# GREAT-WHU/DBA-Fusion

Measured on AMD Instinct MI355X. Metric: DBA iterations/sec (25-KF, 96-edge, 512x512) [dba_update/s], higher is better.
Workload: dtype f32 (BA, f64 reduced system) / f16 (correlation)

## Files before the change

dba-fusion_amd/csrc/ba_host.hip:

```cpp
#include <hip/hip_runtime.h>

#include <algorithm>
#include <atomic>
#include <cstdio>
#include <cstdlib>
#include <cstring>
#include <mutex>
#include <unordered_map>
#include <vector>

#include "ba_kernels.h"

#ifndef GRAM_F32_DEFAULT
#define GRAM_F32_DEFAULT true
#endif

namespace dba {

static thread_local char g_last_error[512] = "";

void set_last_error(const char *what, hipError_t e) {
  snprintf(g_last_error, sizeof(g_last_error), "%s -> %s", what, hipGetErrorString(e));
}

struct BaEnv {
  static int num(const char *name) { const char *e = getenv(name); return e ? atoi(e) : 0; }
  static bool is(const char *name, const char *prefix) { const char *e = getenv(name); return e && !strncmp(e, prefix, strlen(prefix)); }
  int deterministic = is("DBA_DETERMINISTIC", "1");
  int solve_check = is("DBA_SOLVE_CHECK", "1");
  int schur_form = is("DBA_SCHUR_KERNEL", "r") ? 1 : (is("DBA_SCHUR_KERNEL", "f") || is("DBA_SCHUR_KERNEL", "g")) ? 2 : 0;
  int lin_ppl = num("DBA_LINEARIZE_PPL");
  bool lin_no_mfma = is("DBA_LINEARIZE_MFMA", "0");
  int lin_ew = num("DBA_LIN_EW");
  bool h_full = is("DBA_H_FULL", "1");
  int schur_nch = num("DBA_SCHUR_NCH");
  int gram_threads = num("DBA_SCHUR_WAVES") == 4 ? 256 : 512;
  bool gram_f32 = getenv("DBA_SCHUR_MFMA") ? is("DBA_SCHUR_MFMA", "f3") : GRAM_F32_DEFAULT;
  bool fuse_update = !is("DBA_BA_FUSE_UPDATE", "0");
};
static const BaEnv &ba_env() { static const BaEnv env; return env; }

static std::atomic<int> g_schur_form{ba_env().schur_form};
static std::atomic<int> g_deterministic{ba_env().deterministic};
static std::atomic<int> g_solve_check{ba_env().solve_check};

__global__ __launch_bounds__(256) void ba_solve_check_kernel(const double *__restrict__ H, const double *__restrict__ b, int n, double lm,
                                                             double ep, float *__restrict__ dx, int *__restrict__ meta) {
  __shared__ double s_res[256], s_mag[256];
  __shared__ int s_bad;
  if (meta[1] != 0) return;
  double res = 0.0, mag = 0.0;
  for (int i = threadIdx.x; i < n; i += blockDim.x) {
    double acc = -b[i], m = fabs(b[i]);
    for (int j = 0; j < n; j++) {
      double h = H[(size_t)max(i, j) * n + min(i, j)];
      if (i == j) h = fma(lm, h, h) + ep;
      const double t = h * (double)dx[j];
      acc += t, m += fabs(t);
    }
    res = fmax(res, fabs(acc)), mag = fmax(mag, m);
  }
  s_res[threadIdx.x] = res, s_mag[threadIdx.x] = mag;
  __syncthreads();
  if (threadIdx.x == 0) {
    double r = 0.0, m = 0.0;
    for (int k = 0; k < (int)blockDim.x; k++) r = fmax(r, s_res[k]), m = fmax(m, s_mag[k]);
    s_bad = !(r <= 1e-5 * m) ? 1 : 0;
    if (s_bad) meta[1] = 1;
  }
  __syncthreads();
  if (s_bad)
    for (int i = threadIdx.x; i < n; i += blockDim.x) dx[i] = 0.f;
}

static bool schur_auto_frame_form(int N, int P) {
  const int frames = P + 1;
  const int rows_est = 1 + (N + frames - 1) / frames;
  return rows_est > 6;
}

static std::atomic<int> g_schur_generation{0};
static thread_local int t_schur_form = 0;

bool ba_schur_frame_form(int N, int P) {
  const int forced = g_schur_form.load(std::memory_order_relaxed);
  if (N + 1 > GRAM_LIST_CAP) return false;
  if (forced) return forced == 2;
  if (t_schur_form) return t_schur_form == 2;
  return schur_auto_frame_form(N, P);
}

int ba_plan(int N, int B, int ht, int wd, int t0, int t1, void *ws, size_t ws_bytes, BaPlan *plan) {
  if (N < 0 || B <= 0 || ht <= 0 || wd <= 0 || t1 < t0 || t0 < 0 || t1 > B) return DBA_ERR_ARG;
  const int P = t1 - t0;
  const int HW = ht * wd;
  const int Mmax = (P + N < B) ? (P + N) : B;
  int ppl = 1;
  {
    const int env_ppl = ba_env().lin_ppl;
    const long waves1 = (long)Mmax * ((HW + 63) / 64);
    if (env_ppl == 1 || env_ppl == 2 || env_ppl == 4) ppl = env_ppl;
    else if (waves1 >= 16 * 1024) ppl = 4;
    else if (waves1 >= 8 * 1024) ppl = 2;
  }
  const int nchunks = (HW + 256 * ppl - 1) / (256 * ppl);
  const int nparts_max = ((HW + 255) / 256) * 4;
  const int nparts = nchunks * 4;
  const int n6 = 6 * P;
  size_t off = 0;
  auto take = [&](size_t bytes) {
    const size_t o = off;
    off = align_up(off + bytes, 256);
    return o;
  };
  dba_ba_layout L;
  memset(&L, 0, sizeof(L));
  L.meta = take(sizeof(int) * 32);
  const size_t o_gkey = take(sizeof(int) * (8 + 2 * (size_t)N));
  L.kx = take(sizeof(int) * (size_t)(Mmax > 0 ? Mmax : 1));
  const size_t o_fslot = take(sizeof(int) * (size_t)B);
  const size_t o_eoff = take(sizeof(int) * (size_t)(Mmax + 1));
  const size_t o_elist = take(sizeof(int) * (size_t)(N > 0 ? N : 1));
  const size_t o_erank = take(sizeof(int) * (size_t)(N > 0 ? N : 1));
  const size_t o_fpose = take(sizeof(int) * (size_t)(P > 0 ? P : 1));
  const size_t o_einfo = take(sizeof(int) * 2 * (size_t)(N > 0 ? N : 1));
  const size_t o_rowinfo = take(sizeof(int) * 8 * (size_t)(P + N > 0 ? P + N : 1));
  const size_t o_fhead = take(sizeof(int) * 4 * (size_t)(Mmax > 0 ? Mmax : 1));
  const size_t o_frow = take(sizeof(int) * 2 * (size_t)(P + N > 0 ? P + N : 1));
  L.E = take(sizeof(float) * (size_t)(P + N) * 6 * HW);
  L.Q = take(sizeof(float) * (size_t)Mmax * HW);
  L.w = take(sizeof(float) * (size_t)Mmax * HW);
  const size_t o_hparte = take(sizeof(float) * (size_t)(N > 0 ? N : 1) * nparts_max * HPE_STRIDE);
  const size_t o_aedge = take(sizeof(double) * 36 * (size_t)(N > 0 ? N : 1));
  L.dx = take(sizeof(float) * (size_t)(n6 > 0 ? n6 : 1));
  const size_t o_ptmp = take(sizeof(float) * 2 * 7 * (size_t)B);
  L.H = take(sizeof(double) * (size_t)(n6 > 0 ? n6 * (size_t)n6 : 1));
  L.b = take(sizeof(double) * (size_t)(n6 > 0 ? n6 : 1));
  size_t o_lscratch = 0;
  const bool lds_fits = ba_solve_fits_lds(n6);
  const bool want_scratch = !lds_fits || (ba_solve_band_supported(n6) && n6 >= 96);
  if (want_scratch) o_lscratch = take(sizeof(double) * ba_solve_scratch_doubles(n6));
  L.P = P;
  L.Mmax = Mmax;
  L.nchunks = nchunks;
  plan->layout = L;
  plan->bytes = off;
  plan->P = P;
  plan->N = N;
  plan->B = B;
  plan->HW = HW;
  plan->nchunks = nchunks;
  plan->ht = ht, plan->wd = wd, plan->t0 = t0, plan->t1 = t1;
  if (ws) {
    if (ws_bytes < off) return DBA_ERR_WORKSPACE;
    char *base = static_cast<char *>(ws);
    plan->T.meta = reinterpret_cast<int *>(base + L.meta);
    plan->T.kx = reinterpret_cast<int *>(base + L.kx);
    plan->T.frame_slot = reinterpret_cast<int *>(base + o_fslot);
    plan->T.eoff = reinterpret_cast<int *>(base + o_eoff);
    plan->T.elist = reinterpret_cast<int *>(base + o_elist);
    plan->T.elist_rank = reinterpret_cast<int *>(base + o_erank);
    plan->T.fpose = reinterpret_cast<int *>(base + o_fpose);
    plan->T.einfo = reinterpret_cast<int *>(base + o_einfo);
    plan->T.rowinfo = reinterpret_cast<int *>(base + o_rowinfo);
    plan->T.fhead = reinterpret_cast<int *>(base + o_fhead);
    plan->T.frow = reinterpret_cast<int *>(base + o_frow);
    plan->T.gkey = reinterpret_cast<int *>(base + o_gkey);
    plan->T.Mmax = Mmax;
    plan->T.B = B;
    plan->W.E = reinterpret_cast<float *>(base + L.E);
    plan->W.Q = reinterpret_cast<float *>(base + L.Q);
    plan->W.w = reinterpret_cast<float *>(base + L.w);
    plan->W.HpartE = reinterpret_cast<float *>(base + o_hparte);
    plan->W.Aedge = reinterpret_cast<double *>(base + o_aedge);
    plan->W.dx = reinterpret_cast<float *>(base + L.dx);
    plan->W.poses_tmp = reinterpret_cast<float *>(base + o_ptmp);
    plan->W.H = reinterpret_cast<double *>(base + L.H);
    plan->W.b = reinterpret_cast<double *>(base + L.b);
    plan->W.Lscratch = want_scratch ? reinterpret_cast<double *>(base + o_lscratch) : nullptr;
    plan->W.nparts = nparts;
    plan->W.ppl = ppl;
  }
  return DBA_OK;
}

static int ba_prepare_stage(const BaPlan &plan, const int64_t *ii, const int64_t *jj, int eta_rows, int check, bool judge_band,
                            hipStream_t stream) {
  const int N = plan.N, B = plan.B, P = plan.P;
  if (N > 0 && (!ii || !jj)) return DBA_ERR_ARG;
  const int want = std::max(std::max(N, B), P);
  const int threads = std::min(1024, std::max(64, (want + 63) / 64 * 64));
  const size_t scan_ints = std::max<size_t>(std::max(threads, P), N > threads ? 1024 : 0) + 32;
  const size_t lds = sizeof(int) * ((size_t)B + 2 * (size_t)plan.T.Mmax + 1 + scan_ints + plan.T.Mmax + 1);
  if (lds > 160 * 1024 || P > 16384) return DBA_ERR_UNSUPPORTED;
  if (lds > 64 * 1024) {
    DBA_HIP_CHECK(hipFuncSetAttribute(reinterpret_cast<const void *>(&ba_prepare_kernel),
                                      hipFuncAttributeMaxDynamicSharedMemorySize, 160 * 1024));
  }
  const int max_nt = judge_band ? ba_solve_wave_max_nt(6 * P) : 0;
  int *band_verdict = max_nt ? solver_verdict_slot(plan.T.meta) : nullptr;
  hipLaunchKernelGGL(ba_prepare_kernel, dim3(1), dim3(threads), lds, stream, ii, jj, N, B, plan.t0, plan.t1,
                     (int)scan_ints, ba_schur_frame_form(N, P) ? 1 : 0, check ? 1 : 0, eta_rows,
                     eta_rows > 1 ? ws_eta_status(plan.T.meta) : nullptr, plan.T, band_verdict, max_nt);
  DBA_LAUNCH_CHECK();
  return DBA_OK;
}

static int ba_linearize_stage(const BaPlan &plan, const BaProblem &g, const float *poses, const float *disps, float alpha,
                              int upd, float *poses_out, float *disps_w, hipStream_t stream) {
  if (!poses || !disps || !g.intrinsics || !g.disps_sens || !g.eta || g.eta_rows < 1) return DBA_ERR_ARG;
  if (g.eta_rows > 1 && g.eta_rows > plan.T.Mmax) return DBA_ERR_ARG;
  if (plan.N > 0 && (!g.targets || !g.weights || !g.jj)) return DBA_ERR_ARG;
#define LAUNCH_LIN(PPL, MF, EW)                                                                                          \
  hipLaunchKernelGGL((ba_linearize_kernel<PPL, MF, EW>), dim3(plan.nchunks * EW, plan.T.Mmax + 1), dim3(256), 0, stream, \
                     poses, disps, g.intrinsics, g.disps_sens, g.targets, g.weights, g.eta, g.eta_rows, g.jj,            \
                     g.frame_owned, plan.N, plan.HW, plan.wd, plan.t0, plan.P, alpha, upd, poses_out, disps_w, plan.T, plan.W)
  if (plan.W.ppl == 4) LAUNCH_LIN(4, false, 1);
  else if (plan.W.ppl == 2) LAUNCH_LIN(2, false, 1);
  else if (ba_env().lin_no_mfma) LAUNCH_LIN(1, false, 1);
  else {
    const int env_ew = ba_env().lin_ew;
    const long waves2 = (long)plan.nchunks * 2 * 4 * plan.T.Mmax;
    const bool one = env_ew ? env_ew == 1 : waves2 > 4096;
    if (one) LAUNCH_LIN(1, true, 1);
    else LAUNCH_LIN(1, true, 2);
  }
#undef LAUNCH_LIN
  DBA_LAUNCH_CHECK();
  return DBA_OK;
}

static int ba_reduce_stage(const BaPlan &plan, const int64_t *ii, const int64_t *jj, const uint8_t *frame_owned, int motion_only,
                           int lower, hipStream_t stream) {
  const int N = plan.N;
  const int ablocks = (N + 3) / 4;
  if (plan.P <= 0) return DBA_OK;
  if (ba_env().h_full) lower = 0;
  const bool fixed = g_deterministic.load(std::memory_order_relaxed) != 0;
  if (fixed) lower |= 2;
  if (!motion_only) {
    if (!ba_schur_frame_form(N, plan.P)) {
      hipLaunchKernelGGL(ba_schur_kernel, dim3(plan.P + N + ablocks, SCHUR_KP, SCHUR_CH), dim3(256), 0, stream, ii, jj,
                         frame_owned, N, plan.HW, plan.t0, plan.P, lower, plan.T, plan.W);
    } else {
      const int px = 1024;
      int nch = ba_env().schur_nch > 0 ? ba_env().schur_nch : (plan.HW + px - 1) / px;
      nch = std::max(1, std::min(nch, (plan.HW + 15) / 16));
      const dim3 grid((unsigned)(plan.T.Mmax * nch + ablocks));
      const int gram_threads = ba_env().gram_threads;
      const bool f32 = ba_env().gram_f32;
#define GRAM_LAUNCH(V, F)                                                                                     \
  hipLaunchKernelGGL((ba_schur_gram_kernel<V, F>), grid, dim3(gram_threads), 0, stream, ii, jj, frame_owned, \
                     N, plan.HW, plan.t0, plan.P, nch, lower, plan.T, plan.W)
      if (plan.HW % 4 == 0) { if (f32) GRAM_LAUNCH(true, true); else GRAM_LAUNCH(true, false); }
      else { if (f32) GRAM_LAUNCH(false, true); else GRAM_LAUNCH(false, false); }
#undef GRAM_LAUNCH
    }
    DBA_LAUNCH_CHECK();
  } else if (ablocks > 0) {
    hipLaunchKernelGGL(ba_assemble_kernel, dim3(ablocks), dim3(256), 0, stream, ii, jj, frame_owned, N, plan.t0, plan.P,
                       lower, plan.T, plan.W);
    DBA_LAUNCH_CHECK();
  }
  if (fixed) {
    const int n = 6 * plan.P;
    hipLaunchKernelGGL(ba_fixed_to_f64_kernel, dim3((n * n + n + 255) / 256), dim3(256), 0, stream, plan.W.H, plan.W.b, n);
    DBA_LAUNCH_CHECK();
  }
  return DBA_OK;
}

static int ba_symmetrize_launch(const BaPlan &plan, hipStream_t stream) {
  const int n = 6 * plan.P;
  if (n <= 0) return DBA_OK;
  hipLaunchKernelGGL(ba_symmetrize_kernel, dim3((n * n + 255) / 256), dim3(256), 0, stream, plan.W.H, n);
  DBA_LAUNCH_CHECK();
  return DBA_OK;
}

static int ba_solve_check_launch(const BaPlan &plan, float lm, float ep, hipStream_t stream) {
  if (plan.P <= 0) return DBA_OK;
  hipLaunchKernelGGL(ba_solve_check_kernel, dim3(1), dim3(256), 0, stream, plan.W.H, plan.W.b, 6 * plan.P, (double)lm, (double)ep,
                     plan.W.dx, plan.T.meta);
  DBA_LAUNCH_CHECK();
  return DBA_OK;
}

static int ba_solve_stage(const BaPlan &plan, float lm, float ep, const int *fpose, int hint, hipStream_t stream) {
  const int rc = launch_ba_solve(plan.W.H, plan.W.b, fpose, 6 * plan.P, (double)lm, (double)ep, plan.W.dx, plan.T.meta,
                                 plan.W.Lscratch, stream, nullptr, hint, (fpose && fpose == plan.T.fpose) ? plan.T.meta + 16 : nullptr);
  if (rc != DBA_OK) return rc;
  if (g_solve_check.load(std::memory_order_relaxed)) return ba_solve_check_launch(plan, lm, ep, stream);
  return DBA_OK;
}

static int ba_update_launch(const BaPlan &plan, float *poses, float *disps, const int64_t *jj, const uint8_t *frame_owned,
                            int update_poses, int update_disps, float *dz_out, float *dx_out, hipStream_t stream,
                            const float *poses_src = nullptr, float disp_floor = 0.f) {
  dim3 grid((plan.HW + 255) / 256, plan.T.Mmax + 1 + (disp_floor > 0.f ? plan.B : 0));
  hipLaunchKernelGGL(ba_update_kernel, grid, dim3(256), 0, stream, poses, poses_src, disps, jj, frame_owned, plan.HW, plan.t0,
                     plan.P, update_poses, update_disps, dz_out, dx_out, plan.T, plan.W, disp_floor);
  DBA_LAUNCH_CHECK();
  return DBA_OK;
}

int ba_run_loop(const BaPlan &plan, const BaProblem &g, float *poses, float *disps, const BaRun &run, hipStream_t stream) {
  const int *fpose = run.window_fpose ? run.window_fpose : plan.T.fpose;
  int rc;
  if (run.prepared != 1) {
    rc = ba_prepare_stage(plan, g.ii, g.jj, g.eta_rows, run.prepared == 2, run.window_fpose == nullptr, stream);
    if (rc != DBA_OK) return rc;
  }
  const bool fuse = ba_env().fuse_update;
  const float *pose_src = poses;
  bool pending = false;
  for (int itr = 0; itr < run.iterations; itr++) {
    float *pose_dst = plan.W.poses_tmp + (size_t)(itr & 1) * 7 * plan.B;
    const int upd = pending ? (run.motion_only ? 1 : 3) : 0;
    rc = ba_linearize_stage(plan, g, pose_src, disps, run.alpha, upd, pending ? pose_dst : nullptr, disps, stream);
    if (rc != DBA_OK) return rc;
    if (pending) pose_src = pose_dst;
    rc = ba_reduce_stage(plan, g.ii, g.jj, g.frame_owned, run.motion_only, 1, stream);
    if (rc != DBA_OK) return rc;
    if (run.exchange && run.exchange->fn && plan.P > 0) {
      const size_t n6 = (size_t)6 * plan.P;
      rc = run.exchange->fn(run.exchange->ctx, plan.W.H, (size_t)(plan.W.b - plan.W.H) + n6, stream);
      if (rc != DBA_OK) return rc;
    }
    rc = ba_solve_stage(plan, run.lm, run.ep, fpose, run.solver_hint, stream);
    if (rc != DBA_OK) return rc;
    const bool last = (itr == run.iterations - 1);
    if (fuse && !last) {
      pending = true;
      continue;
    }
    rc = ba_update_launch(plan, poses, disps, g.jj, g.frame_owned, 1, run.motion_only ? 0 : 1, last ? run.dz_out : nullptr,
                          last ? run.dx_out : nullptr, stream, pose_src == poses ? nullptr : pose_src,
                          last ? run.disp_floor : 0.f);
    if (rc != DBA_OK) return rc;
    pose_src = poses;
    pending = false;
  }
  return DBA_OK;
}

namespace {
struct BacoreStage {
  double *host = nullptr;
  size_t doubles = 0;
  unsigned *counter = nullptr;
  int seq = 0;
};
std::mutex g_stage_mu;
typedef std::unordered_map<const void *, BacoreStage> BacoreStageMap;
BacoreStageMap *stage_map_ptr() {
  static BacoreStageMap *m = new BacoreStageMap;
  return m;
}
#define stage_map() (*stage_map_ptr())
int *stage_flag(const BacoreStage &st) { return reinterpret_cast<int *>(st.host + st.doubles + 8); }
}

static int bacore_stage_for(const int *meta, size_t need, hipStream_t stream, BacoreStage **out) {
  std::lock_guard<std::mutex> lock(g_stage_mu);
  BacoreStage &st = stage_map()[meta];
  if (st.doubles < need) {
    if (st.host) {
      DBA_HIP_CHECK(hipStreamSynchronize(stream));
      (void)hipHostFree(st.host);
      st.host = nullptr, st.doubles = 0;
    }
    void *p = nullptr;
    DBA_HIP_CHECK(hipHostMalloc(&p, sizeof(double) * (need + 16), hipHostMallocCoherent | hipHostMallocMapped));
    st.host = static_cast<double *>(p), st.doubles = need;
    memset(p, 0, sizeof(double) * (need + 16));
    if (!st.counter) {
      DBA_HIP_CHECK(hipMalloc(reinterpret_cast<void **>(&st.counter), 64));
      DBA_HIP_CHECK(hipMemset(st.counter, 0, 64));
    }
  }
  *out = &st;
  return DBA_OK;
}

static int bacore_wait(int *flag, int seq, hipStream_t stream) {
  for (unsigned long spins = 1;; spins++) {
    if (__atomic_load_n(flag, __ATOMIC_ACQUIRE) == seq) return DBA_OK;
    if ((spins & 0x3fff) == 0) {
      const hipError_t q = hipStreamQuery(stream);
      if (q == hipSuccess) {
        if (__atomic_load_n(flag, __ATOMIC_ACQUIRE) == seq) return DBA_OK;
        set_last_error("BACore.hessian: the stream drained without the export kernel's completion word", hipErrorUnknown);
        return DBA_ERR_HIP;
      }
      if (q != hipErrorNotReady) {
        set_last_error("hipStreamQuery", q);
        return DBA_ERR_HIP;
      }
    }
    __builtin_ia32_pause();
  }
}

static int bacore_export(const BaPlan &plan, int layout, const double *A36, double stabilizer, double **out_host,
                         hipStream_t stream) {
  const int n = 6 * plan.P;
  BacoreStage *st = nullptr;
  const int rc = bacore_stage_for(plan.T.meta, (size_t)n * (n + 1), stream, &st);
  if (rc != DBA_OK) return rc;
  *out_host = st->host;
  if (n == 0) return DBA_OK;
  ExportArg arg;
  for (int i = 0; i < 36; i++) arg.A[i] = (layout == 1) ? A36[i] : 0.0;
  const int seq = ++st->seq;
  const int total = n * (n + 1);
  hipLaunchKernelGGL(ba_export_kernel, dim3((total + 255) / 256), dim3(256), 0, stream, plan.W.H, plan.W.b, n, st->host, layout,
                     arg, stabilizer, st->counter, stage_flag(*st), seq);
  DBA_LAUNCH_CHECK();
  return bacore_wait(stage_flag(*st), seq, stream);
}

}

using namespace dba;

extern "C" {

const char *dba_version(void) { return "dba_hip 0.1 (gfx950)"; }
const char *dba_last_error(void) { return g_last_error; }

size_t dba_ba_workspace_bytes(int N, int B, int ht, int wd, int t0, int t1) {
  BaPlan plan;
  if (ba_plan(N, B, ht, wd, t0, t1, nullptr, 0, &plan) != DBA_OK) return 0;
  return plan.bytes;
}

int dba_ba_get_layout(int N, int B, int ht, int wd, int t0, int t1, dba_ba_layout *out) {
  BaPlan plan;
  const int rc = ba_plan(N, B, ht, wd, t0, t1, nullptr, 0, &plan);
  if (rc != DBA_OK) return rc;
  *out = plan.layout;
  return DBA_OK;
}

int dba_ba_poll_eta_error(int *eta_rows, int *num_kx) { return ws_poll_eta(nullptr, eta_rows, num_kx); }

int dba_ba_poll_eta_error_ws(int N, int B, int ht, int wd, int t0, int t1, void *ws, size_t ws_bytes, int *eta_rows, int *num_kx) {
  DBA_PLAN_OR_RETURN(plan);
  return ws_poll_eta(plan.T.meta, eta_rows, num_kx);
}

int dba_ba_gather_edges(const float *target_inac, const float *weight_inac, const int64_t *ii_inac, const int64_t *jj_inac,
                        int n_inac, const int64_t *sel, int n_sel, const float *target_act, const float *weight_act,
                        const int64_t *ii_act, const int64_t *jj_act, int n_act, int ht, int wd, float *targets_out,
                        float *weights_out, int64_t *ii_out, int64_t *jj_out, dba_stream_t stream) {
  if (n_sel < 0 || n_act < 0 || n_inac < 0 || ht <= 0 || wd <= 0) return DBA_ERR_ARG;
  if (!sel && n_sel > n_inac) return DBA_ERR_ARG;
  const int n = n_sel + n_act;
  if (n == 0) return DBA_OK;
  if (!targets_out || !weights_out || !ii_out || !jj_out) return DBA_ERR_ARG;
  if (n_sel > 0 && (!target_inac || !weight_inac || !ii_inac || !jj_inac || n_inac == 0)) return DBA_ERR_ARG;
  if (n_act > 0 && (!target_act || !weight_act || !ii_act || !jj_act)) return DBA_ERR_ARG;
  const int HW = ht * wd;
  hipLaunchKernelGGL(ba_gather_edges_kernel, dim3((HW + 255) / 256, n, 2), dim3(256), 0, (hipStream_t)stream,
                     reinterpret_cast<const float2 *>(target_inac), reinterpret_cast<const float2 *>(weight_inac), ii_inac, jj_inac,
                     sel, n_sel, n_inac, reinterpret_cast<const float2 *>(target_act), reinterpret_cast<const float2 *>(weight_act),
                     ii_act, jj_act, HW, targets_out, weights_out, ii_out, jj_out);
  DBA_LAUNCH_CHECK();
  return DBA_OK;
}

int dba_ba_solver_verdict(int N, int B, int ht, int wd, int t0, int t1, void *ws, size_t ws_bytes) {
  DBA_PLAN_OR_RETURN(plan);
  if (!ba_solve_wave_supported(6 * plan.P)) return 2;
  const int *slot = solver_verdict_slot(plan.T.meta);
  return slot ? __atomic_load_n(slot, __ATOMIC_RELAXED) : 0;
}

int dba_ba_workspace_init(int N, int B, int ht, int wd, int t0, int t1, void *ws, size_t ws_bytes, dba_stream_t stream) {
  DBA_PLAN_OR_RETURN(plan);
  DBA_HIP_CHECK(hipMemsetAsync(plan.T.meta, 0, (size_t)((char *)(plan.T.gkey + 8) - (char *)plan.T.meta), (hipStream_t)stream));
  ws_words_reset(plan.T.meta);
  return DBA_OK;
}

int dba_ba_prepare(const int64_t *ii, const int64_t *jj, int N, int B, int ht, int wd, int t0, int t1,
                   void *ws, size_t ws_bytes, dba_stream_t stream) {
  return dba_ba_prepare_keyed(ii, jj, N, B, ht, wd, t0, t1, 0, 0, ws, ws_bytes, stream);
}

int dba_ba_prepare_keyed(const int64_t *ii, const int64_t *jj, int N, int B, int ht, int wd, int t0, int t1, int eta_rows,
                         int check, void *ws, size_t ws_bytes, dba_stream_t stream) {
  DBA_PLAN_OR_RETURN(plan);
  return ba_prepare_stage(plan, ii, jj, eta_rows, check, false, (hipStream_t)stream);
}

int dba_ba_linearize(const float *poses, const float *disps, const float *intrinsics,
                     const float *disps_sens, const float *targets, const float *weights,
                     const float *eta, int eta_rows, const int64_t *ii, const int64_t *jj,
                     const uint8_t *frame_owned, int N, int B, int ht, int wd, int t0, int t1,
                     float alpha, void *ws, size_t ws_bytes, dba_stream_t stream) {
  DBA_PLAN_OR_RETURN(plan);
  BaProblem g;
  g.intrinsics = intrinsics, g.disps_sens = disps_sens, g.targets = targets, g.weights = weights;
  g.eta = eta, g.eta_rows = eta_rows, g.ii = ii, g.jj = jj, g.frame_owned = frame_owned;
  return ba_linearize_stage(plan, g, poses, disps, alpha, 0, nullptr, nullptr, (hipStream_t)stream);
}

int dba_ba_reduce(const int64_t *ii, const int64_t *jj, const uint8_t *frame_owned, int N, int B, int ht,
                  int wd, int t0, int t1, int motion_only, void *ws, size_t ws_bytes, dba_stream_t stream) {
  DBA_PLAN_OR_RETURN(plan);
  const int rc = ba_reduce_stage(plan, ii, jj, frame_owned, motion_only, 1, (hipStream_t)stream);
  if (rc != DBA_OK) return rc;
  return ba_symmetrize_launch(plan, (hipStream_t)stream);
}

int dba_ba_schur_select(int form) {
  if (form < 0 || form > 2) return DBA_ERR_ARG;
  g_schur_form.store(form, std::memory_order_relaxed);
  g_schur_generation.fetch_add(1, std::memory_order_relaxed);
  return DBA_OK;
}

int dba_ba_schur_select_thread(int form) {
  if (form < 0 || form > 2) return DBA_ERR_ARG;
  t_schur_form = form;
  return DBA_OK;
}

int dba_ba_schur_thread_form(void) { return t_schur_form; }

int dba_ba_schur_auto_form(int N, int P) { return schur_auto_frame_form(N, P) ? 2 : 1; }

int dba_ba_schur_generation(void) { return g_schur_generation.load(std::memory_order_relaxed); }

int dba_ba_set_deterministic(int on) {
  g_deterministic.store(on ? 1 : 0, std::memory_order_relaxed);
  return DBA_OK;
}

int dba_ba_set_solve_check(int on) {
  g_solve_check.store(on ? 1 : 0, std::memory_order_relaxed);
  return DBA_OK;
}

int dba_ba_solve_check(int N, int B, int ht, int wd, int t0, int t1, float lm, float ep, void *ws, size_t ws_bytes,
                       dba_stream_t stream) {
  DBA_PLAN_OR_RETURN(plan);
  return ba_solve_check_launch(plan, lm, ep, (hipStream_t)stream);
}

int dba_ba_symmetrize(int N, int B, int ht, int wd, int t0, int t1, void *ws, size_t ws_bytes, dba_stream_t stream) {
  DBA_PLAN_OR_RETURN(plan);
  return ba_symmetrize_launch(plan, (hipStream_t)stream);
}

int dba_ba_solve(int N, int B, int ht, int wd, int t0, int t1, float lm, float ep, void *ws, size_t ws_bytes,
                 dba_stream_t stream) {
  return dba_ba_solve_skyline(N, B, ht, wd, t0, t1, lm, ep, nullptr, ws, ws_bytes, stream);
}

int dba_ba_solve_skyline(int N, int B, int ht, int wd, int t0, int t1, float lm, float ep, const int32_t *fpose, void *ws,
                         size_t ws_bytes, dba_stream_t stream) {
  DBA_PLAN_OR_RETURN(plan);
  return ba_solve_stage(plan, lm, ep, fpose, 0, (hipStream_t)stream);
}

int dba_ba_update(float *poses, float *disps, const int64_t *ii, const int64_t *jj,
                  const uint8_t *frame_owned, int N, int B, int ht, int wd, int t0, int t1, int update_poses,
                  int update_disps, float *dz_out, void *ws, size_t ws_bytes, dba_stream_t stream) {
  (void)ii;
  DBA_PLAN_OR_RETURN(plan);
  return ba_update_launch(plan, poses, disps, jj, frame_owned, update_poses, update_disps, dz_out, nullptr, (hipStream_t)stream);
}

int dba_ba_shard_front(const float *poses, const float *disps, const float *intrinsics, const float *disps_sens,
                       const float *targets, const float *weights, const float *eta, int eta_rows, const int64_t *ii,
                       const int64_t *jj, const uint8_t *frame_owned, int N, int B, int ht, int wd, int t0, int t1,
                       float alpha, int motion_only, void *ws, size_t ws_bytes, dba_stream_t stream) {
  DBA_PLAN_OR_RETURN(plan);
  BaProblem g;
  g.intrinsics = intrinsics, g.disps_sens = disps_sens, g.targets = targets, g.weights = weights;
  g.eta = eta, g.eta_rows = eta_rows, g.ii = ii, g.jj = jj, g.frame_owned = frame_owned;
  const int rc = ba_linearize_stage(plan, g, poses, disps, alpha, 0, nullptr, nullptr, (hipStream_t)stream);
  if (rc != DBA_OK) return rc;
  return ba_reduce_stage(plan, ii, jj, frame_owned, motion_only, 1, (hipStream_t)stream);
}

int dba_ba_shard_back(float *poses, float *disps, const int64_t *ii, const int64_t *jj, const uint8_t *frame_owned,
                      int N, int B, int ht, int wd, int t0, int t1, float lm, float ep, int update_disps,
                      const int32_t *window_fpose, int solver_hint, void *ws, size_t ws_bytes, dba_stream_t stream) {
  DBA_PLAN_OR_RETURN(plan);
  const int rc = ba_solve_stage(plan, lm, ep, window_fpose, solver_hint, (hipStream_t)stream);
  if (rc != DBA_OK) return rc;
  return ba_update_launch(plan, poses, disps, jj, frame_owned, 1, update_disps, nullptr, nullptr, (hipStream_t)stream);
}

int dba_ba(float *poses, float *disps, const float *intrinsics, const float *disps_sens,
           const float *targets, const float *weights, const float *eta, int eta_rows, const int64_t *ii,
           const int64_t *jj, int N, int B, int ht, int wd, int t0, int t1, int iterations, float lm,
           float ep, int motion_only, float *dx_out, float *dz_out, void *ws, size_t ws_bytes,
           dba_stream_t stream) {
  return dba_ba_run(poses, disps, intrinsics, disps_sens, targets, weights, eta, eta_rows, ii, jj, N, B, ht, wd, t0, t1,
                    iterations, lm, ep, motion_only, dx_out, dz_out, ws, ws_bytes, stream, 0, 0, 0.f);
}

int dba_ba_prepared(float *poses, float *disps, const float *intrinsics, const float *disps_sens,
                    const float *targets, const float *weights, const float *eta, int eta_rows, const int64_t *ii,
                    const int64_t *jj, int N, int B, int ht, int wd, int t0, int t1, int iterations, float lm,
                    float ep, int motion_only, float *dx_out, float *dz_out, void *ws, size_t ws_bytes,
                    dba_stream_t stream, int solver_hint) {
  return dba_ba_run(poses, disps, intrinsics, disps_sens, targets, weights, eta, eta_rows, ii, jj, N, B, ht, wd, t0, t1,
                    iterations, lm, ep, motion_only, dx_out, dz_out, ws, ws_bytes, stream, 1, solver_hint, 0.f);
}

int dba_ba_run(float *poses, float *disps, const float *intrinsics, const float *disps_sens, const float *targets,
               const float *weights, const float *eta, int eta_rows, const int64_t *ii, const int64_t *jj, int N, int B,
               int ht, int wd, int t0, int t1, int iterations, float lm, float ep, int motion_only, float *dx_out,
               float *dz_out, void *ws, size_t ws_bytes, dba_stream_t stream, int prepared, int solver_hint,
               float disp_floor) {
  if (!(disp_floor >= 0.f)) return DBA_ERR_ARG;
  DBA_PLAN_OR_RETURN(plan);
  BaProblem g;
  g.intrinsics = intrinsics, g.disps_sens = disps_sens, g.targets = targets, g.weights = weights;
  g.eta = eta, g.eta_rows = eta_rows, g.ii = ii, g.jj = jj, g.frame_owned = nullptr;
  BaRun run = {};
  run.iterations = iterations, run.lm = lm, run.ep = ep, run.alpha = 0.05f ;
  run.motion_only = motion_only, run.prepared = prepared, run.solver_hint = prepared == 1 ? solver_hint : 0;
  run.disp_floor = disp_floor, run.dx_out = dx_out, run.dz_out = dz_out;
  return ba_run_loop(plan, g, poses, disps, run, (hipStream_t)stream);
}

int dba_bacore_hessian(const float *poses, const float *disps, const float *intrinsics,
                       const float *disps_sens, const float *targets, const float *weights,
                       const float *eta, int eta_rows, const int64_t *ii, const int64_t *jj, int N, int B,
                       int ht, int wd, int t0, int t1, double *H_host, double *v_host, void *ws,
                       size_t ws_bytes, dba_stream_t stream) {
  return dba_bacore_hessian_run(poses, disps, intrinsics, disps_sens, targets, weights, eta, eta_rows, ii, jj, N, B, ht, wd,
                                t0, t1, H_host, v_host, ws, ws_bytes, stream, 0);
}

int dba_bacore_hessian_host(const float *poses, const float *disps, const float *intrinsics,
                            const float *disps_sens, const float *targets, const float *weights,
                            const float *eta, int eta_rows, const int64_t *ii, const int64_t *jj, int N, int B,
                            int ht, int wd, int t0, int t1, void *ws, size_t ws_bytes, dba_stream_t stream, int prepared,
                            int layout, const double *A36, double stabilizer, double **out_host) {
  DBA_PLAN_OR_RETURN(plan);
  int rc;
  if (!out_host || (layout != 0 && layout != 1) || (layout == 1 && !A36)) return DBA_ERR_ARG;
  hipStream_t s = (hipStream_t)stream;
  if (prepared != 1) {
    rc = ba_prepare_stage(plan, ii, jj, eta_rows, prepared == 2, false, s);
    if (rc != DBA_OK) return rc;
  }
  BaProblem g;
  g.intrinsics = intrinsics, g.disps_sens = disps_sens, g.targets = targets, g.weights = weights;
  g.eta = eta, g.eta_rows = eta_rows, g.ii = ii, g.jj = jj, g.frame_owned = nullptr;
  rc = ba_linearize_stage(plan, g, poses, disps, 0.001f , 0, nullptr, nullptr, s);
  if (rc != DBA_OK) return rc;
  rc = ba_reduce_stage(plan, ii, jj, nullptr, 0, 1, s);
  if (rc != DBA_OK) return rc;
  return bacore_export(plan, layout, A36, stabilizer, out_host, s);
}

int dba_bacore_export_host(int N, int B, int ht, int wd, int t0, int t1, void *ws, size_t ws_bytes, dba_stream_t stream, int layout,
                           const double *A36, double stabilizer, double **out_host) {
  DBA_PLAN_OR_RETURN(plan);
  if (!out_host || (layout != 0 && layout != 1) || (layout == 1 && !A36)) return DBA_ERR_ARG;
  return bacore_export(plan, layout, A36, stabilizer, out_host, (hipStream_t)stream);
}

int dba_bacore_staging(int N, int B, int ht, int wd, int t0, int t1, void *ws, size_t ws_bytes, double **out_host) {
  DBA_PLAN_OR_RETURN(plan);
  if (!out_host) return DBA_ERR_ARG;
  std::lock_guard<std::mutex> lock(g_stage_mu);
  auto it = stage_map().find(plan.T.meta);
  *out_host = (it == stage_map().end()) ? nullptr : it->second.host;
  return *out_host ? DBA_OK : DBA_ERR_ARG;
}

int dba_bacore_hessian_run(const float *poses, const float *disps, const float *intrinsics,
                           const float *disps_sens, const float *targets, const float *weights,
                           const float *eta, int eta_rows, const int64_t *ii, const int64_t *jj, int N, int B,
                           int ht, int wd, int t0, int t1, double *H_host, double *v_host, void *ws,
                           size_t ws_bytes, dba_stream_t stream, int prepared) {
  double *stage = nullptr;
  const int rc = dba_bacore_hessian_host(poses, disps, intrinsics, disps_sens, targets, weights, eta, eta_rows, ii, jj, N, B, ht, wd,
                                         t0, t1, ws, ws_bytes, stream, prepared, 0, nullptr, 0.0, &stage);
  if (rc != DBA_OK) return rc;
  const size_t n = (size_t)6 * std::max(t1 - t0, 0);
  if (n && H_host && H_host != stage) memcpy(H_host, stage, sizeof(double) * n * n);
  if (n && v_host && v_host != stage + n * n) memcpy(v_host, stage + n * n, sizeof(double) * n);
  return DBA_OK;
}

struct DxArg {
  float v[384];
};
__global__ void ba_dx_from_arg_kernel(DxArg a, float *__restrict__ dx, float *__restrict__ dx_out, int n) {
  const int i = blockIdx.x * blockDim.x + threadIdx.x;
  if (i < n) {
    dx[i] = a.v[i];
    if (dx_out) dx_out[i] = a.v[i];
  }
}

int dba_bacore_retract(float *poses, float *disps, const int64_t *ii, const int64_t *jj, int N, int B, int ht,
                       int wd, int t0, int t1, const double *dx_host, float *dx_out, float *dz_out, void *ws,
                       size_t ws_bytes, dba_stream_t stream) {
  (void)ii;
  DBA_PLAN_OR_RETURN(plan);
  const int n = 6 * plan.P;
  if (n > 0 && n <= 384) {
    if (!dx_host) return DBA_ERR_ARG;
    DxArg a;
    for (int i = 0; i < n; i++) a.v[i] = (float)dx_host[i];
    hipLaunchKernelGGL(ba_dx_from_arg_kernel, dim3((n + 127) / 128), dim3(128), 0, (hipStream_t)stream, a, plan.W.dx, dx_out, n);
    DBA_LAUNCH_CHECK();
  } else if (n > 0) {
    if (!dx_host) return DBA_ERR_ARG;
    std::vector<float> dxf((size_t)n);
    for (int i = 0; i < n; i++) dxf[i] = (float)dx_host[i];
    DBA_HIP_CHECK(hipMemcpyAsync(plan.W.dx, dxf.data(), sizeof(float) * n, hipMemcpyHostToDevice,
                                 (hipStream_t)stream));
    DBA_HIP_CHECK(hipStreamSynchronize((hipStream_t)stream));
  }
  const int rc = ba_update_launch(plan, poses, disps, jj, nullptr, 1, 1, dz_out, nullptr, (hipStream_t)stream);
  if (rc != DBA_OK) return rc;
  if (dx_out && n > 384) {
    hipLaunchKernelGGL(ba_copy_f32_kernel, dim3((n + 255) / 256), dim3(256), 0, (hipStream_t)stream, plan.W.dx,
                       dx_out, n);
    DBA_LAUNCH_CHECK();
  }
  return DBA_OK;
}

int dba_bacore_optimize(const double *H_host, const double *v_host, int N, int B, int ht, int wd, int t0,
                        int t1, float lm, float ep, float *dx_out, void *ws, size_t ws_bytes,
                        dba_stream_t stream) {
  DBA_PLAN_OR_RETURN(plan);
  const size_t n = (size_t)6 * plan.P;
  if (n == 0) return DBA_OK;
  if (!H_host || !v_host) return DBA_ERR_ARG;
  DBA_HIP_CHECK(hipMemcpyAsync(plan.W.H, H_host, sizeof(double) * n * n, hipMemcpyHostToDevice,
                               (hipStream_t)stream));
  DBA_HIP_CHECK(hipMemcpyAsync(plan.W.b, v_host, sizeof(double) * n, hipMemcpyHostToDevice,
                               (hipStream_t)stream));
  const int rc = ba_solve_stage(plan, lm, ep, nullptr, 0, (hipStream_t)stream);
  if (rc != DBA_OK) return rc;
  if (dx_out) {
    hipLaunchKernelGGL(ba_copy_f32_kernel, dim3(((int)n + 255) / 256), dim3(256), 0, (hipStream_t)stream,
                       plan.W.dx, dx_out, (int)n);
    DBA_LAUNCH_CHECK();
  }
  DBA_HIP_CHECK(hipStreamSynchronize((hipStream_t)stream));
  return DBA_OK;
}

}
```

dba-fusion_amd/csrc/ba_kernels.h:

```cpp
#pragma once
#include "common.h"

namespace dba {

constexpr int HPE_STRIDE = 32;
#ifndef SCHUR_KP_CFG
#define SCHUR_KP_CFG 8
#endif
#ifndef SCHUR_CH_CFG
#define SCHUR_CH_CFG 2
#endif
constexpr int SCHUR_KP = SCHUR_KP_CFG;
constexpr int SCHUR_CH = SCHUR_CH_CFG;

struct BaTables {
  int *meta;
  int *kx;
  int *frame_slot;
  int *eoff;
  int *elist;
  int *elist_rank;
  int *fpose;
  int *einfo;
  int *rowinfo;
  int *fhead;
  int *frow;
  int *gkey;
  int Mmax, B;
};

struct BaBuffers {
  float *E;
  float *Q;
  float *w;
  float *HpartE;
  double *Aedge;
  double *H;
  double *b;
  float *dx;
  double *Lscratch;
  float *poses_tmp;
  int nparts;
  int ppl;
};

struct BaPlan {
  BaTables T;
  BaBuffers W;
  dba_ba_layout layout;
  size_t bytes;
  int P, N, B, HW, nchunks;
  int ht, wd, t0, t1;
};

int ba_plan(int N, int B, int ht, int wd, int t0, int t1, void *ws, size_t ws_bytes, BaPlan *plan);
#define DBA_PLAN_OR_RETURN(plan) \
  BaPlan plan;                   \
  if (const int plan_rc_ = ::dba::ba_plan(N, B, ht, wd, t0, t1, ws, ws_bytes, &plan)) return plan_rc_

constexpr int GKEY_MAGIC = 0x6b657935;
__global__ void ba_prepare_kernel(const int64_t *ii, const int64_t *jj, int N, int B, int t0, int t1, int scan_ints,
                                  int ftable, int check, int eta_rows, int *status, BaTables T, int *band_verdict, int max_nt);
bool ba_schur_frame_form(int N, int P);
template <int PPL, bool MF, int EW>
__global__ void ba_linearize_kernel(const float *poses, const float *disps, const float *intrinsics,
                                    const float *disps_sens, const float *targets, const float *weights,
                                    const float *eta, int eta_rows, const int64_t *jj,
                                    const uint8_t *frame_owned, int N, int HW, int wd, int t0, int P,
                                    float alpha, int upd, float *poses_out, float *disps_w, BaTables T, BaBuffers W);
__global__ void ba_assemble_kernel(const int64_t *ii, const int64_t *jj, const uint8_t *frame_owned, int N,
                                   int t0, int P, int lower, BaTables T, BaBuffers W);
__global__ void ba_schur_kernel(const int64_t *ii, const int64_t *jj, const uint8_t *frame_owned, int N, int HW,
                                int t0, int P, int lower, BaTables T, BaBuffers W);
__global__ void ba_symmetrize_kernel(double *H, int n);
struct ExportArg {
  double A[36];
};
__global__ void ba_export_kernel(const double *H, const double *b, int n, double *out, int gtsam, ExportArg arg, double stab,
                                 unsigned *counter, int *host_flag, int seq);
__global__ void ba_fixed_to_f64_kernel(double *H, double *b, int n);
constexpr int GRAM_LIST_CAP = 1024;
template <bool VEC, bool F32>
__global__ void ba_schur_gram_kernel(const int64_t *ii, const int64_t *jj, const uint8_t *frame_owned, int N, int HW,
                                     int t0, int P, int nch, int lower, BaTables T, BaBuffers W);
__global__ void ba_update_kernel(float *poses, const float *poses_src, float *disps, const int64_t *jj, const uint8_t *frame_owned,
                                 int HW, int t0, int P, int update_poses, int update_disps, float *dz_out,
                                 float *dx_out, BaTables T, BaBuffers W, float disp_floor);
__global__ void ba_copy_f32_kernel(const float *src, float *dst, int n);
__global__ void ba_gather_edges_kernel(const float2 *tgt_inac, const float2 *wgt_inac, const int64_t *ii_inac, const int64_t *jj_inac,
                                       const int64_t *sel, int n_sel, int n_inac, const float2 *tgt_act, const float2 *wgt_act,
                                       const int64_t *ii_act, const int64_t *jj_act, int HW, float *tgt_out, float *wgt_out,
                                       int64_t *ii_out, int64_t *jj_out);

struct BaProblem {
  const float *intrinsics, *disps_sens, *targets, *weights, *eta;
  int eta_rows;
  const int64_t *ii, *jj;
  const uint8_t *frame_owned;
};
struct BaExchange {
  int (*fn)(void *ctx, double *hb, size_t hb_len, hipStream_t stream);
  void *ctx;
};
struct BaRun {
  int iterations;
  float lm, ep, alpha;
  int motion_only;
  int prepared, solver_hint;
  float disp_floor;
  const int32_t *window_fpose;
  const BaExchange *exchange;
  float *dx_out, *dz_out;
};
int ba_run_loop(const BaPlan &plan, const BaProblem &g, float *poses, float *disps, const BaRun &run, hipStream_t stream);

int launch_ba_solve(const double *H, const double *b, const int *fpose, int n, double lm, double ep, float *dx, int *meta,
                    double *Lscratch, hipStream_t stream, long long *prof = nullptr, int hint = 0, int *splan = nullptr);
bool ba_solve_fits_lds(int n);
bool ba_solve_tile_supported(int n);
bool ba_solve_band_supported(int n);
int launch_ba_solve_band(const double *H, const double *b, const int *fpose, int n, double lm, double ep, float *dx,
                         int *meta, double *scratch, size_t scratch_doubles, bool big, hipStream_t stream,
                         bool last = false);
int launch_ba_solve_tile(const double *H, const double *b, int n, double lm, double ep, float *dx, int *meta,
                         hipStream_t stream);
bool ba_solve_wave_supported(int n);
int ba_solve_wave_max_nt(int n);
int *solver_verdict_slot(const int *meta);
void ws_words_reset(const int *meta);
int *ws_eta_status(const int *meta);
int ws_poll_eta(const int *meta, int *eta_rows, int *num_kx);
int launch_ba_solve_wave(const double *H, const double *b, const int *fpose, int n, double lm, double ep, float *dx, int *meta,
                         double *Lscratch, int *verdict, hipStream_t stream, long long *prof = nullptr, int *splan = nullptr);
size_t ba_solve_scratch_doubles(int n);
constexpr int SOLVE_MAX_LDS_BYTES = 160 * 1024;

}
```

dba-fusion_amd/csrc/ba_kernels.hip:

```cpp
#include "ba_kernels.h"
#include "ba_solve_admit.h"

#include <cstdio>
#include <cstring>

namespace dba {

__device__ __forceinline__ int wave_incl_scan(int v, int lane) {
#pragma unroll
  for (int off = 1; off < 64; off <<= 1) {
    const int o = __shfl_up(v, off, 64);
    if (lane >= off) v += o;
  }
  return v;
}

__global__ __launch_bounds__(1024) void ba_prepare_kernel(const int64_t *__restrict__ ii,
                                                          const int64_t *__restrict__ jj, int N, int B,
                                                          int t0, int t1, int scan_ints, int ftable, int check,
                                                          int eta_rows, int *__restrict__ status, BaTables T,
                                                          int *__restrict__ band_verdict, int max_nt) {
  extern __shared__ int sm[];
  int *flag = sm;
  int *cnt = sm + B;
  int *kxs = cnt + T.Mmax + 1;
  int *scan = kxs + T.Mmax;
  int *vcnt = scan + scan_ints;
  const int tid = threadIdx.x, nt = blockDim.x, lane = tid & 63, wave = tid >> 6, nw = nt >> 6;
  const int P = t1 - t0;
  const int my_i = (tid < N) ? (int)ii[tid] : -1, my_j = (tid < N) ? (int)jj[tid] : -1;
  auto src = [&](int n) { return (n == tid) ? my_i : (int)ii[n]; };
  auto dst = [&](int n) { return (n == tid) ? my_j : (int)jj[n]; };
  auto check_eta = [&](int nk) {
    if (tid == 0) {
      const bool bad = eta_rows > 1 && eta_rows != nk;
      T.gkey[7] = bad ? 1 : 0;
      if (bad && status) {
        status[1] = eta_rows, status[2] = nk;
        __hip_atomic_store(status, 1, __ATOMIC_RELEASE, __HIP_MEMORY_SCOPE_SYSTEM);
      }
    }
  };

  {
    const int *key = T.gkey;
    bool same = check && key[0] == GKEY_MAGIC && key[1] == N && key[2] == B && key[3] == t0 && key[4] == t1 &&
                key[5] == ftable && key[6] == T.Mmax;
    if (same) {
      for (int n = tid; n < N; n += nt) {
        const long long a = (long long)ii[n], b = (long long)jj[n];
        same = same && (long long)key[8 + n] == a && (long long)key[8 + N + n] == b;
      }
    }
    if (__syncthreads_and(same)) {
      check_eta(T.meta[0]);
      return;
    }
  }

  for (int f = tid; f < B; f += nt) flag[f] = 0;
  for (int m = tid; m <= T.Mmax; m += nt) cnt[m] = 0;
  __syncthreads();
  for (int p = tid; p < P; p += nt) {
    const int f = t0 + p;
    if (f >= 0 && f < B) flag[f] = 1;
  }
  for (int n = tid; n < N; n += nt) {
    const int f = src(n);
    if (f >= 0 && f < B) flag[f] = 1;
  }
  __syncthreads();

  const int per = (B + nt - 1) / nt;
  const int lo = min(tid * per, B), hi = min(lo + per, B);
  int c = 0;
  for (int f = lo; f < hi; f++) c += flag[f];
  const int incl = wave_incl_scan(c, lane);
  if (lane == 63) scan[wave] = incl;
  __syncthreads();
  if (wave == 0) {
    const int v = (lane < nw) ? scan[lane] : 0;
    const int w = wave_incl_scan(v, lane);
    if (lane < nw) scan[16 + lane] = w;
  }
  __syncthreads();
  int slot = incl - c + (wave > 0 ? scan[16 + wave - 1] : 0);
  const int M = scan[16 + nw - 1];
  for (int f = lo; f < hi; f++) {
    if (flag[f]) {
      if (slot < T.Mmax) T.kx[slot] = f, kxs[slot] = f;
      T.frame_slot[f] = (slot < T.Mmax) ? slot : -1;
      flag[f] = slot + 1;
      slot++;
    } else {
      T.frame_slot[f] = -1;
    }
  }
  if (tid == 0) {
    T.meta[0] = min(M, T.Mmax);
    T.meta[1] = 0;
    T.meta[2] = (M > T.Mmax) ? 1 : 0;
    T.meta[7] = 0;
    T.meta[16] = 0;
  }
  check_eta(min(M, T.Mmax));
  __syncthreads();
  auto slot_of = [&](int f) { return (f >= 0 && f < B && flag[f] > 0 && flag[f] <= T.Mmax) ? flag[f] - 1 : -1; };
  auto emit_edge = [&](int n, int m, int pos, int jx) {
    const int tg = jx - t0;
    int *ri = T.rowinfo + 8 * (P + n);
    const bool ok = m >= 0 && tg >= 0 && tg < P;
    ri[0] = ok ? m : -1, ri[1] = tg, ri[2] = pos + 1, ri[3] = (m >= 0) ? cnt[m + 1] : 0, ri[4] = (m >= 0) ? kxs[m] : -1;
    if (pos >= 0) T.einfo[2 * pos] = n, T.einfo[2 * pos + 1] = jx;
  };

  for (int n = tid; n < N; n += nt) {
    const int m = slot_of(src(n));
    if (m >= 0) atomicAdd(&cnt[m], 1);
  }
  __syncthreads();
  if (wave == 0) {
    int carry = 0;
    for (int base = 0; base <= T.Mmax; base += 64) {
      const int m = base + lane;
      const int v = (m < T.Mmax) ? cnt[m] : 0;
      const int w = wave_incl_scan(v, lane);
      if (m <= T.Mmax) {
        cnt[m] = carry + w - v;
        T.eoff[m] = carry + w - v;
      }
      carry += __shfl(w, 63, 64);
    }
  }
  __syncthreads();
  int *sii = scan;
  const int Mv0 = min(M, T.Mmax);
  if (N <= nt) {
    const bool myvalid = (tid < N) && (slot_of(my_i) >= 0) && (my_j - t0 >= 0) && (my_j - t0 < P);
    constexpr int VBIT = 1 << 30;
    if (tid < N) sii[tid] = (my_i & (VBIT - 1)) | (myvalid ? VBIT : 0);
    if (ftable)
      for (int m = tid; m <= T.Mmax; m += nt) {
        const int pp = (m < Mv0) ? kxs[m] - t0 : -1;
        vcnt[m] = (pp >= 0 && pp < P) ? 1 : 0;
      }
    __syncthreads();
    int vrank = 0;
    if (tid < N) {
      const int f = my_i & (VBIT - 1), m = slot_of(my_i);
      int pos = -1;
      if (m >= 0) {
        int rank = 0;
        for (int q = 0; q < tid; q++) {
          const int x = sii[q];
          const bool same = ((x & (VBIT - 1)) == f);
          rank += same;
          vrank += same ? (x >> 30) : 0;
        }
        pos = cnt[m] + rank;
        T.elist[pos] = tid;
        if (myvalid && ftable) atomicAdd(&vcnt[m], 1);
      }
      emit_edge(tid, m, pos, my_j);
    }
    if (!ftable) {
      for (int m = tid; m < T.Mmax; m += nt) T.fhead[4 * m] = -1, T.fhead[4 * m + 2] = 0;
    } else {
    __syncthreads();
    if (wave == 0) {
      int carry = 0;
      for (int base = 0; base < T.Mmax; base += 64) {
        const int m = base + lane;
        const int v = (m < T.Mmax) ? vcnt[m] : 0;
        const int w = wave_incl_scan(v, lane);
        if (m < T.Mmax) {
          const int pp = (m < Mv0) ? kxs[m] - t0 : -1;
          const bool own = (pp >= 0 && pp < P);
          const int off = carry + w - v;
          int *fh = T.fhead + 4 * m;
          fh[0] = (m < Mv0) ? kxs[m] : -1, fh[1] = off, fh[2] = v, fh[3] = 0;
          if (own) T.frow[2 * off] = pp, T.frow[2 * off + 1] = pp;
          vcnt[m] = off + (own ? 1 : 0);
        }
        carry += __shfl(w, 63, 64);
      }
    }
    __syncthreads();
    if (myvalid) {
      const int o = vcnt[slot_of(my_i)] + vrank;
      T.frow[2 * o] = P + tid, T.frow[2 * o + 1] = my_j - t0;
    }
    }
  } else {
    for (int m = tid; m < T.Mmax; m += nt) T.fhead[4 * m] = -1, T.fhead[4 * m + 2] = 0;
    for (int n = tid; n < N; n += nt) T.elist_rank[n] = 0;
    for (int base = 0; base < N; base += 1024) {
      __syncthreads();
      for (int q = tid; q < 1024 && base + q < N; q += nt) sii[q] = (int)ii[base + q];
      __syncthreads();
      const int lim = min(1024, N - base);
      for (int n = tid; n < N; n += nt) {
        if (n <= base) continue;
        const int f = (int)ii[n];
        if (slot_of(f) < 0) continue;
        int rank = 0;
        const int qend = min(lim, n - base);
        for (int q = 0; q < qend; q++) rank += (sii[q] == f);
        T.elist_rank[n] += rank;
      }
    }
    __syncthreads();
    for (int n = tid; n < N; n += nt) {
      const int m = slot_of((int)ii[n]);
      const int pos = (m >= 0) ? cnt[m] + T.elist_rank[n] : -1;
      if (m >= 0) T.elist[pos] = n;
      emit_edge(n, m, pos, (int)jj[n]);
    }
  }
  for (int p = tid; p < P; p += nt) {
    const int m = slot_of(t0 + p);
    int *ri = T.rowinfo + 8 * p;
    ri[0] = m, ri[1] = p, ri[2] = (m >= 0) ? cnt[m] : 0, ri[3] = (m >= 0) ? cnt[m + 1] : 0, ri[4] = t0 + p;
  }
  __syncthreads();
  const int Mv = min(M, T.Mmax);
  int *minS = cnt;
  int *fps = scan;
  for (int m = tid; m < Mv; m += nt) {
    const int pp = kxs[m] - t0;
    minS[m] = (pp >= 0 && pp < P) ? pp : 0x7fffffff;
  }
  for (int pp = tid; pp < P; pp += nt) fps[pp] = pp;
  __syncthreads();
  for (int n = tid; n < N; n += nt) {
    const int m = slot_of(src(n)), tg = dst(n) - t0;
    if (m >= 0 && tg >= 0 && tg < P) atomicMin(&minS[m], tg);
  }
  __syncthreads();
  for (int n = tid; n < N; n += nt) {
    const int m = slot_of(src(n)), tg = dst(n) - t0;
    if (m >= 0 && tg >= 0 && tg < P) atomicMin(&fps[tg], minS[m]);
  }
  for (int m = tid; m < Mv; m += nt) {
    const int pp = kxs[m] - t0;
    if (pp >= 0 && pp < P) atomicMin(&fps[pp], minS[m]);
  }
  __syncthreads();
  for (int pp = tid; pp < P; pp += nt) T.fpose[pp] = fps[pp];
  if (band_verdict && wave == 0) {
    const int admitted = ba_solve_wave_admits(fps, 6 * P, lane, max_nt);
    if (lane == 0) __hip_atomic_store(band_verdict, admitted ? 1 : 2, __ATOMIC_RELAXED, __HIP_MEMORY_SCOPE_SYSTEM);
  }
  for (int n = tid; n < N; n += nt) T.gkey[8 + n] = (int)ii[n], T.gkey[8 + N + n] = (int)jj[n];
  if (tid == 0) {
    int *key = T.gkey;
    key[0] = GKEY_MAGIC, key[1] = N, key[2] = B, key[3] = t0, key[4] = t1, key[5] = ftable, key[6] = T.Mmax;
  }
}

__device__ void retract_pose(float *pose, const float *xi) {
  const float *tau = xi, *phi = xi + 3;
  const float th2 = phi[0] * phi[0] + phi[1] * phi[1] + phi[2] * phi[2];
  const float th4 = th2 * th2;
  const float th = sqrtf(th2);
  float imag, real;
  if (th2 < 1e-8f) {
    imag = 0.5f - (1.0f / 48.0f) * th2 + (1.0f / 3840.0f) * th4;
    real = 1.0f - (1.0f / 8.0f) * th2 + (1.0f / 384.0f) * th4;
  } else {
    imag = sinf(0.5f * th) / th;
    real = cosf(0.5f * th);
  }
  const float dq[4] = {imag * phi[0], imag * phi[1], imag * phi[2], real};
  float dt[3] = {tau[0], tau[1], tau[2]};
  if (th > 1e-4f) {
    const float a = (1.f - cosf(th)) / th2;
    const float b = (th - sinf(th)) / (th * th2);
    const float c1[3] = {phi[1] * tau[2] - phi[2] * tau[1], phi[2] * tau[0] - phi[0] * tau[2],
                         phi[0] * tau[1] - phi[1] * tau[0]};
    const float c2[3] = {phi[1] * c1[2] - phi[2] * c1[1], phi[2] * c1[0] - phi[0] * c1[2],
                         phi[0] * c1[1] - phi[1] * c1[0]};
#pragma unroll
    for (int c = 0; c < 3; c++) dt[c] += a * c1[c] + b * c2[c];
  }
  const float t[3] = {pose[0], pose[1], pose[2]};
  const float q[4] = {pose[3], pose[4], pose[5], pose[6]};
  float q1[4], t1[3];
  q1[0] = dq[3] * q[0] + dq[0] * q[3] + dq[1] * q[2] - dq[2] * q[1];
  q1[1] = dq[3] * q[1] + dq[1] * q[3] + dq[2] * q[0] - dq[0] * q[2];
  q1[2] = dq[3] * q[2] + dq[2] * q[3] + dq[0] * q[1] - dq[1] * q[0];
  q1[3] = dq[3] * q[3] - dq[0] * q[0] - dq[1] * q[1] - dq[2] * q[2];
  quat_rotate(dq, t, t1);
  pose[0] = t1[0] + dt[0];
  pose[1] = t1[1] + dt[1];
  pose[2] = t1[2] + dt[2];
  pose[3] = q1[0];
  pose[4] = q1[1];
  pose[5] = q1[2];
  pose[6] = q1[3];
}


__device__ __forceinline__ void load_pose(const float *__restrict__ poses, const float *__restrict__ dx, int f, int t0, int P,
                                          bool upd, float *out) {
#pragma unroll
  for (int c = 0; c < 7; c++) out[c] = poses[7 * f + c];
  const int p = f - t0;
  if (upd && p >= 0 && p < P) retract_pose(out, dx + 6 * p);
}

__device__ __forceinline__ void edge_pose64(const float *__restrict__ poses, const float *__restrict__ dx, int ix, int jx,
                                            int t0, int P, bool upd, double *t, double *R) {
  double q[4];
  if (ix == jx) {
    t[0] = -0.1; t[1] = 0.0; t[2] = 0.0;
    q[0] = 0.0; q[1] = 0.0; q[2] = 0.0; q[3] = 1.0;
  } else {
    float Pi[7], Pj[7];
    load_pose(poses, dx, ix, t0, P, upd, Pi);
    load_pose(poses, dx, jx, t0, P, upd, Pj);
    const double ti[3] = {Pi[0], Pi[1], Pi[2]}, qi[4] = {Pi[3], Pi[4], Pi[5], Pi[6]};
    const double tj[3] = {Pj[0], Pj[1], Pj[2]}, qj[4] = {Pj[3], Pj[4], Pj[5], Pj[6]};
    q[0] = -qj[3] * qi[0] + qj[0] * qi[3] - qj[1] * qi[2] + qj[2] * qi[1];
    q[1] = -qj[3] * qi[1] + qj[1] * qi[3] - qj[2] * qi[0] + qj[0] * qi[2];
    q[2] = -qj[3] * qi[2] + qj[2] * qi[3] - qj[0] * qi[1] + qj[1] * qi[0];
    q[3] = qj[3] * qi[3] + qj[0] * qi[0] + qj[1] * qi[1] + qj[2] * qi[2];
    const double uv0 = 2.0 * (q[1] * ti[2] - q[2] * ti[1]);
    const double uv1 = 2.0 * (q[2] * ti[0] - q[0] * ti[2]);
    const double uv2 = 2.0 * (q[0] * ti[1] - q[1] * ti[0]);
    t[0] = tj[0] - (ti[0] + q[3] * uv0 + (q[1] * uv2 - q[2] * uv1));
    t[1] = tj[1] - (ti[1] + q[3] * uv1 + (q[2] * uv0 - q[0] * uv2));
    t[2] = tj[2] - (ti[2] + q[3] * uv2 + (q[0] * uv1 - q[1] * uv0));
  }
  const double x = q[0], y = q[1], z = q[2], w = q[3];
  R[0] = 1.0 - 2.0 * (y * y + z * z);
  R[1] = 2.0 * (x * y - w * z);
  R[2] = 2.0 * (x * z + w * y);
  R[3] = 2.0 * (x * y + w * z);
  R[4] = 1.0 - 2.0 * (x * x + z * z);
  R[5] = 2.0 * (y * z - w * x);
  R[6] = 2.0 * (x * z - w * y);
  R[7] = 2.0 * (y * z + w * x);
  R[8] = 1.0 - 2.0 * (x * x + y * y);
}

__device__ __forceinline__ float backsub_pixel(const BaTables &T, const BaBuffers &W, int m, int frame, int k, int HW, int t0,
                                               int P) {
  float acc = 0.f;
  const int p = frame - t0;
  if (p > 0 && p < P) {
    const float *Er = W.E + ((size_t)p * 6) * HW + k;
    const float *x = W.dx + 6 * p;
    float dw = 0.f;
#pragma unroll
    for (int c = 0; c < 6; c++) dw += Er[(size_t)c * HW] * x[c];
    acc += dw;
  }
  const int e0 = T.eoff[m], e1 = T.eoff[m + 1];
  for (int e = e0; e < e1; e++) {
    const int2 ei = *reinterpret_cast<const int2 *>(T.einfo + 2 * e);
    const int n = ei.x;
    const int tgt = ei.y - t0;
    if (tgt <= 0 || tgt >= P) continue;
    const float *Er = W.E + ((size_t)(P + n) * 6) * HW + k;
    const float *x = W.dx + 6 * tgt;
    float dw = 0.f;
#pragma unroll
    for (int c = 0; c < 6; c++) dw += Er[(size_t)c * HW] * x[c];
    acc += dw;
  }
  const size_t mk = (size_t)m * HW + k;
  return W.Q[mk] * (W.w[mk] - acc);
}


struct PixelLin {
  float Ju[6], Jv[6];
  float Jzu, Jzv;
  float ru, rv, wu, wv;
};

template <typename T>
__device__ __forceinline__ void edge_adjoint(const T *t, const T *R, T *A) {
#pragma unroll
  for (int k = 0; k < 3; k++)
#pragma unroll
    for (int c = 0; c < 3; c++) {
      A[6 * k + c] = -R[3 * k + c];
      A[6 * (3 + k) + 3 + c] = -R[3 * k + c];
      A[6 * (3 + k) + c] = (T)0;
    }
#pragma unroll
  for (int c = 0; c < 3; c++) {
    A[6 * 0 + 3 + c] = t[2] * R[3 + c] - t[1] * R[6 + c];
    A[6 * 1 + 3 + c] = t[0] * R[6 + c] - t[2] * R[c];
    A[6 * 2 + 3 + c] = t[1] * R[c] - t[0] * R[3 + c];
  }
}

__device__ __forceinline__ void linearize_pixel(float u, float v, float disp, float tu, float tv,
                                                float wgt_u, float wgt_v, const float *intr,
                                                const float *tij, const Rot3 &R, bool stereo,
                                                PixelLin &L, float &Cii, float &bz) {
  const float fx = intr[0], fy = intr[1], cx = intr[2], cy = intr[3];
  const float X0 = (u - cx) / fx, X1 = (v - cy) / fy;
  const float x = fmaf(disp, tij[0], fmaf(R.r[0], X0, fmaf(R.r[1], X1, R.r[2])));
  const float y = fmaf(disp, tij[1], fmaf(R.r[3], X0, fmaf(R.r[4], X1, R.r[5])));
  const float z = fmaf(disp, tij[2], fmaf(R.r[6], X0, fmaf(R.r[7], X1, R.r[8])));
  const float h = disp;
  const bool close = z < 0.25f;
  const float d = close ? 0.f : 1.f / z;
  const float d2 = d * d;
  float wu = close ? 0.f : 0.001f * wgt_u;
  float wv = close ? 0.f : 0.001f * wgt_v;
  L.ru = tu - fmaf(fx * d, x, cx);
  L.rv = tv - fmaf(fy * d, y, cy);

  float *Jju = L.Ju, *Jjv = L.Jv;
  Jju[0] = fx * (h * d);
  Jju[1] = 0.f;
  Jju[2] = fx * (-x * h * d2);
  Jju[3] = fx * (-x * y * d2);
  Jju[4] = fx * fmaf(x * x, d2, 1.f);
  Jju[5] = fx * (-y * d);
  Jjv[0] = 0.f;
  Jjv[1] = fy * (h * d);
  Jjv[2] = fy * (-y * h * d2);
  Jjv[3] = fy * (-fmaf(y * y, d2, 1.f));
  Jjv[4] = fy * (x * y * d2);
  Jjv[5] = fy * (x * d);
  L.Jzu = fx * (tij[0] * d - tij[2] * (x * d2));
  L.Jzv = fy * (tij[1] * d - tij[2] * (y * d2));

  Cii = wu * L.Jzu * L.Jzu + wv * L.Jzv * L.Jzv;
  bz = wu * L.ru * L.Jzu + wv * L.rv * L.Jzv;
  if (stereo) { wu = 0.f; wv = 0.f; }
  L.wu = wu;
  L.wv = wv;
}


constexpr int RED_PITCH = 68;

template <int L>
__device__ __forceinline__ void reduce_deposit(float val, float *red_lane) {
  red_lane[L * RED_PITCH] = val;
}

__device__ __forceinline__ float reduce_row(const float *red_wave, int lane) {
  const float4 *row = reinterpret_cast<const float4 *>(red_wave + lane * RED_PITCH);
  float4 s = row[0];
#pragma unroll
  for (int q = 1; q < 16; q++) {
    const float4 v = row[q];
    s.x += v.x;
    s.y += v.y;
    s.z += v.z;
    s.w += v.w;
  }
  return (s.x + s.y) + (s.z + s.w);
}

__device__ __forceinline__ void wave_lds_fence() {
  __builtin_amdgcn_wave_barrier();
  __builtin_amdgcn_s_waitcnt(0xc07f);
  __builtin_amdgcn_wave_barrier();
}

template <int PPL, int A, int B_>
struct HjjLoop {
  __device__ __forceinline__ static void run(const PixelLin (&L)[PPL], float *acc) {
    float val = 0.f;
#pragma unroll
    for (int q = 0; q < PPL; q++)
      val += L[q].wu * L[q].Ju[A] * L[q].Ju[B_] + L[q].wv * L[q].Jv[A] * L[q].Jv[B_];
    reduce_deposit<A * (A + 1) / 2 + B_>(val, acc);
    if constexpr (B_ < A)
      HjjLoop<PPL, A, B_ + 1>::run(L, acc);
    else if constexpr (A < 5)
      HjjLoop<PPL, A + 1, 0>::run(L, acc);
  }
};

template <int PPL, int A>
struct VjLoop {
  __device__ __forceinline__ static void run(const PixelLin (&L)[PPL], float *acc) {
    float val = 0.f;
#pragma unroll
    for (int q = 0; q < PPL; q++) val += L[q].wu * L[q].ru * L[q].Ju[A] + L[q].wv * L[q].rv * L[q].Jv[A];
    reduce_deposit<21 + A>(val, acc);
    if constexpr (A < 5) VjLoop<PPL, A + 1>::run(L, acc);
  }
};

typedef float lin_f4 __attribute__((ext_vector_type(4)));
constexpr int MFS_T = 16;
constexpr int MFS_P = 20;
constexpr int MFS_VALS = 4 * 16 * MFS_P;
constexpr int MFS_WTS = 4 * 2 * MFS_P;
constexpr int MFS_FLOATS = (MFS_VALS + MFS_WTS) > (64 + 8 * 64) ? (MFS_VALS + MFS_WTS) : (64 + 8 * 64);

#ifdef LIN_PROF
__device__ unsigned long long g_lin_prof[16];
__device__ unsigned long long g_lin_span[2 * 8192];
#define LP(k) do { if (threadIdx.x == 0 && blockIdx.x == 3) { const unsigned long long t_ = wall_clock64(); atomicAdd(&g_lin_prof[k], t_ - lp_); lp_ = t_; } } while (0)
#else
#define LP(k) (void)0
#endif
template <int PPL, bool MF, int EW>
__global__ __launch_bounds__(256, (PPL == 1 ? (MF ? 4 : 2) : 1)) void ba_linearize_kernel(
    const float *__restrict__ poses, const float *__restrict__ disps, const float *__restrict__ intrinsics,
    const float *__restrict__ disps_sens, const float *__restrict__ targets,
    const float *__restrict__ weights, const float *__restrict__ eta, int eta_rows,
    const int64_t *__restrict__ jj, const uint8_t *__restrict__ frame_owned, int N, int HW, int wd,
    int t0, int P, float alpha, int upd_arg, float *__restrict__ poses_out, float *__restrict__ disps_w, BaTables T,
    BaBuffers W) {
  const int upd = T.gkey[7] ? 0 : upd_arg;
#ifdef LIN_PROF
  unsigned long long lp_ = wall_clock64();
  const unsigned long long lp_start_ = lp_;
#endif
  const int m = blockIdx.y;
  if (m == T.Mmax) {
    const int n6 = 6 * P;
    const size_t total = (size_t)n6 * n6;
    for (size_t i = (size_t)blockIdx.x * blockDim.x + threadIdx.x; i < total; i += (size_t)gridDim.x * blockDim.x)
      W.H[i] = 0.0;
    if (blockIdx.x == 0) {
      for (int i = threadIdx.x; i < n6; i += blockDim.x) W.b[i] = 0.0;
      if (upd && poses_out)
        for (int f = threadIdx.x; f < T.B; f += blockDim.x) {
          float pr[7];
          load_pose(poses, W.dx, f, t0, P, true, pr);
#pragma unroll
          for (int c = 0; c < 7; c++) poses_out[7 * f + c] = pr[c];
        }
    }
    return;
  }
  const int M = T.meta[0];
  if (m >= M) return;
  const int frame = T.kx[m];
  if (frame_owned && !frame_owned[frame]) return;

  const int lane = lane_id();
  const int wv = threadIdx.x >> 6, ew = wv % EW;
  const int wave_global = blockIdx.x * (4 / EW) + wv / EW;
  const int kbase = wave_global * (WAVE * PPL) + lane;
  const int nparts = W.nparts;

  float intr[4] = {intrinsics[0], intrinsics[1], intrinsics[2], intrinsics[3]};
  int kc[PPL];
  bool active[PPL];
  float u[PPL], v[PPL], disp[PPL];
#pragma unroll
  for (int q = 0; q < PPL; q++) {
    const int k = kbase + WAVE * q;
    active[q] = k < HW;
    kc[q] = active[q] ? k : 0;
    u[q] = (float)(kc[q] % wd);
    v[q] = (float)(kc[q] / wd);
    disp[q] = disps[(size_t)frame * HW + kc[q]];
    if ((upd & 2) && active[q])
      disp[q] = disp[q] + backsub_pixel(T, W, m, frame, kc[q], HW, t0, P);
  }
  if (upd & 2) {
    __syncthreads();
    if ((threadIdx.x >> 6) % EW == 0) {
#pragma unroll
      for (int q = 0; q < PPL; q++)
        if (active[q]) disps_w[(size_t)frame * HW + kc[q]] = disp[q];
    }
  }

  float Csum[PPL], wsum[PPL], Ei[PPL][6];
#pragma unroll
  for (int q = 0; q < PPL; q++) {
    Csum[q] = 0.f;
    wsum[q] = 0.f;
#pragma unroll
    for (int c = 0; c < 6; c++) Ei[q][c] = 0.f;
  }
  constexpr int EB = 16;
  __shared__ float s_pose[EB][12];
  __shared__ __attribute__((aligned(16))) float s_adj[EB][28];
  __shared__ int s_edge[EB][2];
  constexpr int RED_FLOATS = MF ? MFS_FLOATS : 64 * RED_PITCH;
  __shared__ __attribute__((aligned(16))) float s_red[4][RED_FLOATS];
  float *red_wave = s_red[wv];
  float *red_lane = red_wave + lane;
  const int e0 = T.eoff[m], e1 = T.eoff[m + 1];
  LP(0);
  for (int batch = e0; batch < e1; batch += EB) {
    const int cnt = min(EB, e1 - batch);
    __syncthreads();
    LP(1);
    if ((int)threadIdx.x < cnt) {
      const int2 ei = *reinterpret_cast<const int2 *>(T.einfo + 2 * (batch + threadIdx.x));
      const int n = ei.x, jx = ei.y;
      double t64[3], R64[9];
      edge_pose64(poses, W.dx, frame, jx, t0, P, upd != 0, t64, R64);
      s_edge[threadIdx.x][0] = n;
      s_edge[threadIdx.x][1] = jx;
#pragma unroll
      for (int c = 0; c < 3; c++) s_pose[threadIdx.x][c] = (float)t64[c];
#pragma unroll
      for (int c = 0; c < 9; c++) s_pose[threadIdx.x][3 + c] = (float)R64[c];
      double *Aw = (blockIdx.x == 0) ? W.Aedge + (size_t)n * 36 : nullptr;
      float *As = s_adj[threadIdx.x];
#pragma unroll
      for (int k = 0; k < 3; k++) {
#pragma unroll
        for (int c = 0; c < 3; c++) {
          const double rkc = -R64[3 * k + c];
          const int k1 = (k + 1) % 3, k2 = (k + 2) % 3;
          const double x = t64[k2] * R64[3 * k1 + c] - t64[k1] * R64[3 * k2 + c];
          As[6 * k + c] = (float)rkc, As[6 * k + 3 + c] = (float)x, As[18 + 3 * k + c] = (float)rkc;
          if (Aw) Aw[6 * k + c] = rkc, Aw[6 * k + 3 + c] = x, Aw[6 * (3 + k) + c] = 0.0, Aw[6 * (3 + k) + 3 + c] = rkc;
        }
      }
    }
    __syncthreads();
    LP(2);
    float nx_t[PPL][2], nx_w[PPL][2];
    {
      const int n = s_edge[min(ew, cnt - 1)][0];
#pragma unroll
      for (int q = 0; q < PPL; q++) {
        const size_t tb = (size_t)n * 2 * HW + kc[q];
        nx_t[q][0] = targets[tb];
        nx_t[q][1] = targets[tb + HW];
        nx_w[q][0] = weights[tb];
        nx_w[q][1] = weights[tb + HW];
      }
    }
    for (int i = ew; i < cnt; i += EW) {
      const int n = s_edge[i][0];
      const int jx = s_edge[i][1];
      float tij[3];
      Rot3 R;
#pragma unroll
      for (int c = 0; c < 3; c++) tij[c] = s_pose[i][c];
#pragma unroll
      for (int c = 0; c < 9; c++) R.r[c] = s_pose[i][3 + c];
      float cu_t[PPL][2], cu_w[PPL][2];
#pragma unroll
      for (int q = 0; q < PPL; q++) {
        cu_t[q][0] = nx_t[q][0]; cu_t[q][1] = nx_t[q][1];
        cu_w[q][0] = nx_w[q][0]; cu_w[q][1] = nx_w[q][1];
      }
      if (i + EW < cnt) {
        const int nn = s_edge[i + EW][0];
#pragma unroll
        for (int q = 0; q < PPL; q++) {
          const size_t tb = (size_t)nn * 2 * HW + kc[q];
          nx_t[q][0] = targets[tb];
          nx_t[q][1] = targets[tb + HW];
          nx_w[q][0] = weights[tb];
          nx_w[q][1] = weights[tb + HW];
        }
      }

      PixelLin L[PPL];
#pragma unroll
      for (int q = 0; q < PPL; q++) {
        const float wgu = active[q] ? cu_w[q][0] : 0.f, wgv = active[q] ? cu_w[q][1] : 0.f;
        float Cii, bz;
        linearize_pixel(u[q], v[q], disp[q], cu_t[q][0], cu_t[q][1], wgu, wgv, intr, tij, R, frame == jx, L[q],
                        Cii, bz);
        Csum[q] += Cii;
        wsum[q] += bz;
        float *Eij = W.E + ((size_t)(P + n) * 6) * HW + kc[q];
        const float wJzu = L[q].wu * L[q].Jzu, wJzv = L[q].wv * L[q].Jzv;
        float ej[6];
#pragma unroll
        for (int c = 0; c < 6; c++) {
          ej[c] = wJzu * L[q].Ju[c] + wJzv * L[q].Jv[c];
#ifndef LIN_ABLATE_ESTORE
          if (active[q]) Eij[(size_t)c * HW] = ej[c];
#endif
        }
        const float *Ae = s_adj[i];
#pragma unroll
        for (int c = 0; c < 3; c++)
          Ei[q][c] += fmaf(ej[2], Ae[12 + c], fmaf(ej[1], Ae[6 + c], ej[0] * Ae[c]));
#pragma unroll
        for (int c = 0; c < 3; c++)
          Ei[q][3 + c] += fmaf(ej[5], Ae[24 + c], fmaf(ej[4], Ae[21 + c], fmaf(ej[3], Ae[18 + c],
                          fmaf(ej[2], Ae[15 + c], fmaf(ej[1], Ae[9 + c], ej[0] * Ae[3 + c])))));
      }
      float acc;
      if constexpr (MF) {
        static_assert(!MF || PPL == 1, "the matrix-core reduction is written for one pixel per lane");
        {
          const int t_ = lane >> 2, k0 = lane & 3;
          float *su = red_wave + (k0 * 16) * MFS_P + t_, *sv = su + 8 * MFS_P;
#pragma unroll
          for (int i = 0; i < 6; i++) {
            su[i * MFS_P] = L[0].Ju[i];
            sv[i * MFS_P] = L[0].Jv[i];
          }
          su[6 * MFS_P] = L[0].ru;
          sv[6 * MFS_P] = L[0].rv;
          su[7 * MFS_P] = 0.f;
          sv[7 * MFS_P] = 0.f;
          red_wave[MFS_VALS + (k0 * 2) * MFS_P + t_] = L[0].wu;
          red_wave[MFS_VALS + (k0 * 2 + 1) * MFS_P + t_] = L[0].wv;
        }
        wave_lds_fence();
        lin_f4 c4 = {0.f, 0.f, 0.f, 0.f};
        {
          const lin_f4 *xs = reinterpret_cast<const lin_f4 *>(red_wave + ((lane >> 4) * 16 + (lane & 15)) * MFS_P);
          const lin_f4 *ws = reinterpret_cast<const lin_f4 *>(red_wave + MFS_VALS + ((lane >> 4) * 2 + ((lane >> 3) & 1)) * MFS_P);
          lin_f4 c4b = {0.f, 0.f, 0.f, 0.f};
#pragma unroll
          for (int t4 = 0; t4 < MFS_T / 4; t4 += 2) {
            const lin_f4 x = xs[t4], w4 = ws[t4], y = xs[t4 + 1], v4 = ws[t4 + 1];
#pragma unroll
            for (int e = 0; e < 4; e++) {
              c4 = __builtin_amdgcn_mfma_f32_16x16x4f32(x[e] * w4[e], x[e], c4, 0, 0, 0);
              c4b = __builtin_amdgcn_mfma_f32_16x16x4f32(y[e] * v4[e], y[e], c4b, 0, 0, 0);
            }
          }
#pragma unroll
          for (int r = 0; r < 4; r++) c4[r] += c4b[r];
        }
        wave_lds_fence();
        {
          const int g = lane >> 4, col = lane & 15;
#pragma unroll
          for (int r = 0; r < 4; r++) {
            const int row = 4 * g + r;
            const int a = row & 7, b = col & 7;
            int slot = -1;
            if (((row >> 3) == (col >> 3)) && a < 6) {
              if (b <= a) slot = a * (a + 1) / 2 + b;
              else if (b == 6) slot = 21 + a;
            }
            if (slot >= 0) red_wave[32 * (row >> 3) + slot] = c4[r];
          }
        }
        wave_lds_fence();
        acc = red_wave[lane & 31] + red_wave[32 + (lane & 31)];
        wave_lds_fence();
      } else {
#ifndef LIN_ABLATE_REDUCE
      HjjLoop<PPL, 0, 0>::run(L, red_lane);
      VjLoop<PPL, 0>::run(L, red_lane);
      wave_lds_fence();
      acc = reduce_row(red_wave, lane);
      wave_lds_fence();
#else
      acc = L[0].Ju[0] + L[0].Jv[7];
#endif
      }
      if (lane < HPE_STRIDE) W.HpartE[((size_t)n * nparts + wave_global) * HPE_STRIDE + lane] = acc;
      LP(3);
    }
  }
  LP(4);
  if constexpr (EW > 1) {
    constexpr int NV = 8 * PPL;
    __syncthreads();
    if (ew != 0) {
#pragma unroll
      for (int q = 0; q < PPL; q++) {
        red_lane[(8 * q + 0) * 64] = Csum[q];
        red_lane[(8 * q + 1) * 64] = wsum[q];
#pragma unroll
        for (int c = 0; c < 6; c++) red_lane[(8 * q + 2 + c) * 64] = Ei[q][c];
      }
    }
    __syncthreads();
    if (ew != 0) return;
    static_assert(NV * 64 <= RED_FLOATS, "hand-over does not fit the staging tile");
#pragma unroll
    for (int o = 1; o < EW; o++) {
      const float *src = s_red[wv + o] + lane;
#pragma unroll
      for (int q = 0; q < PPL; q++) {
        Csum[q] += src[(8 * q + 0) * 64];
        wsum[q] += src[(8 * q + 1) * 64];
#pragma unroll
        for (int c = 0; c < 6; c++) Ei[q][c] += src[(8 * q + 2 + c) * 64];
      }
    }
  }
#pragma unroll
  for (int q = 0; q < PPL; q++) {
    if (!active[q]) continue;
    const int k = kc[q];
    const size_t fk = (size_t)frame * HW + k;
    const float ds = disps_sens[fk];
    const float mm = (ds > 0.f) ? 1.f : 0.f;
    const float et = eta[(size_t)min(m, eta_rows - 1) * HW + k];
    const float C = (Csum[q] + mm * alpha) + (1.f - mm) * et;
    const float w = wsum[q] - (mm * alpha) * (disp[q] - ds);
    W.Q[(size_t)m * HW + k] = 1.f / C;
    W.w[(size_t)m * HW + k] = w;
    const int p = frame - t0;
    if (p >= 0 && p < P) {
      float *Er = W.E + ((size_t)p * 6) * HW + k;
#pragma unroll
      for (int c = 0; c < 6; c++) Er[(size_t)c * HW] = Ei[q][c];
    }
  }
  LP(5);
#ifdef LIN_PROF
  if ((threadIdx.x & 63) == 0) {
    const int slot = ((blockIdx.y * gridDim.x + blockIdx.x) * 4 + (threadIdx.x >> 6)) & 8191;
    g_lin_span[2 * slot] = lp_start_;
    g_lin_span[2 * slot + 1] = wall_clock64();
  }
#endif
}

#ifdef LIN_PROF
extern "C" void dba_lin_prof_dump() {
  unsigned long long h[16];
  (void)hipDeviceSynchronize();
  (void)hipMemcpyFromSymbol(h, HIP_SYMBOL(g_lin_prof), sizeof(h));
  static unsigned long long sp[2 * 8192];
  (void)hipMemcpyFromSymbol(sp, HIP_SYMBOL(g_lin_span), sizeof(sp));
  unsigned long long lo = ~0ull, hi = 0, sum = 0, cnt = 0, maxlife = 0, laststart = 0;
  for (int i = 0; i < 8192; i++)
    if (sp[2 * i]) {
      lo = sp[2 * i] < lo ? sp[2 * i] : lo, hi = sp[2 * i + 1] > hi ? sp[2 * i + 1] : hi;
      laststart = sp[2 * i] > laststart ? sp[2 * i] : laststart;
      const unsigned long long life = sp[2 * i + 1] - sp[2 * i];
      sum += life, cnt++, maxlife = life > maxlife ? life : maxlife;
    }
  fprintf(stderr, "LIN_PROF (10 ns ticks, wave 0 of slice-block 3, summed over frames): prologue %llu, sync %llu, resolve %llu, edges %llu, tail-of-loop %llu, epilogue %llu | last launch: %llu waves, first start -> last end %llu ticks, last start at +%llu, mean life %.1f, longest %llu\n",
          h[0], h[1], h[2], h[3], h[4], h[5], cnt, hi - lo, laststart - lo, cnt ? (double)sum / cnt : 0.0, maxlife);
  {
    fprintf(stderr, "LIN_PROF residency (t in ticks: alive / started):");
    for (int d = 0; d <= 10; d++) {
      const unsigned long long t = lo + (hi - lo) * d / 10;
      int alive = 0, started = 0;
      for (int i = 0; i < 8192; i++)
        if (sp[2 * i]) started += sp[2 * i] <= t, alive += (sp[2 * i] <= t && sp[2 * i + 1] > t);
      fprintf(stderr, " %llu: %d / %d;", t - lo, alive, started);
    }
    fprintf(stderr, "\n");
  }
  memset(h, 0, sizeof(h));
  memset(sp, 0, sizeof(sp));
  (void)hipMemcpyToSymbol(HIP_SYMBOL(g_lin_span), sp, sizeof(sp));
  (void)hipMemcpyToSymbol(HIP_SYMBOL(g_lin_prof), h, sizeof(h));
}
#endif

template __global__ void ba_linearize_kernel<1, true, 2>(const float *, const float *, const float *, const float *,
                                                const float *, const float *, const float *, int, const int64_t *,
                                                const uint8_t *, int, int, int, int, int, float, int, float *, float *,
                                                BaTables, BaBuffers);
template __global__ void ba_linearize_kernel<1, true, 1>(const float *, const float *, const float *, const float *,
                                                const float *, const float *, const float *, int, const int64_t *,
                                                const uint8_t *, int, int, int, int, int, float, int, float *, float *,
                                                BaTables, BaBuffers);
template __global__ void ba_linearize_kernel<1, false, 1>(const float *, const float *, const float *, const float *,
                                                const float *, const float *, const float *, int, const int64_t *,
                                                const uint8_t *, int, int, int, int, int, float, int, float *, float *,
                                                BaTables, BaBuffers);
template __global__ void ba_linearize_kernel<2, false, 1>(const float *, const float *, const float *, const float *,
                                                const float *, const float *, const float *, int, const int64_t *,
                                                const uint8_t *, int, int, int, int, int, float, int, float *, float *,
                                                BaTables, BaBuffers);
template __global__ void ba_linearize_kernel<4, false, 1>(const float *, const float *, const float *, const float *,
                                                const float *, const float *, const float *, int, const int64_t *,
                                                const uint8_t *, int, int, int, int, int, float, int, float *, float *,
                                                BaTables, BaBuffers);

__device__ __forceinline__ void atomic_add_f64(double *p, double v) {
  __hip_atomic_fetch_add(p, v, __ATOMIC_RELAXED, __HIP_MEMORY_SCOPE_AGENT);
}

constexpr double ACC_FIX_SCALE = 1073741824.0;
__device__ __forceinline__ void acc_add(double *p, double v, bool fixed) {
  if (fixed)
    atomicAdd(reinterpret_cast<unsigned long long *>(p), (unsigned long long)__double2ll_rn(v * ACC_FIX_SCALE));
  else
    atomic_add_f64(p, v);
}

__device__ __forceinline__ void h_add_pair(const BaBuffers &W, int n6, int hr, int hc, double s, bool lower, bool fixed) {
  if (lower) {
    if (hr == hc) acc_add(&W.H[(size_t)hr * n6 + hc], 2.0 * s, fixed);
    else acc_add(&W.H[(size_t)max(hr, hc) * n6 + min(hr, hc)], s, fixed);
  } else {
    acc_add(&W.H[(size_t)hr * n6 + hc], s, fixed);
    acc_add(&W.H[(size_t)hc * n6 + hr], s, fixed);
  }
}


__device__ __forceinline__ void ba_assemble_block(int block, const int64_t *__restrict__ ii,
                                                  const int64_t *__restrict__ jj,
                                                  const uint8_t *__restrict__ frame_owned, int N, int t0, int P,
                                                  int hflags, const BaTables &T, const BaBuffers &W) {
  const bool lower = (hflags & 1) != 0, fixed = (hflags & 2) != 0;
  const int tid = threadIdx.x;
  const int n6 = 6 * P;
  const int edge_blocks = (N + 3) / 4;
  if (block < edge_blocks) {
    const int n = 4 * block + (tid >> 6);
    const int l = tid & 63;
    if (n >= N) return;
    const int src = (int)ii[n];
    if (frame_owned && !frame_owned[src]) return;
    int ta = 0;
    while ((ta + 1) * (ta + 2) / 2 <= min(l, 20)) ta++;
    const int tb = min(l, 20) - ta * (ta + 1) / 2;
    const int ja = min(l, 35) / 6, jb = min(l, 35) % 6;
    const int va = (l >= 21 && l < 27) ? l - 21 : 0;
    double Ajb[6], Atb[6], Ata[6], Ava[6];
    {
      const double *A = W.Aedge + (size_t)n * 36;
#pragma unroll
      for (int k = 0; k < 6; k++) Ajb[k] = A[6 * k + jb], Atb[k] = A[6 * k + tb], Ata[k] = A[6 * k + ta], Ava[k] = A[6 * k + va];
    }
    double s = 0.0;
    if (l < 27) {
      const float *hp = W.HpartE + (size_t)n * W.nparts * HPE_STRIDE + l;
      int part = 0;
      for (; part + 32 <= W.nparts; part += 32) {
        float v[32];
#pragma unroll
        for (int q = 0; q < 32; q++) v[q] = hp[(size_t)(part + q) * HPE_STRIDE];
#pragma unroll
        for (int q = 0; q < 32; q++) s += (double)v[q];
      }
      for (; part + 8 <= W.nparts; part += 8) {
        float v[8];
#pragma unroll
        for (int q = 0; q < 8; q++) v[q] = hp[(size_t)(part + q) * HPE_STRIDE];
#pragma unroll
        for (int q = 0; q < 8; q++) s += (double)v[q];
      }
      for (; part < W.nparts; part++) s += (double)hp[(size_t)part * HPE_STRIDE];
    }
    const int i = src - t0, j = (int)jj[n] - t0;
    const bool iv = (i >= 0 && i < P), jv = (j >= 0 && j < P);
    if (!iv && !jv) return;
    auto tri = [](int a, int b) { return a >= b ? a * (a + 1) / 2 + b : b * (b + 1) / 2 + a; };
    if (jv) {
      if (l < 21) {
        acc_add(&W.H[(size_t)(6 * j + ta) * n6 + 6 * j + tb], s, fixed);
        if (ta != tb && !lower) acc_add(&W.H[(size_t)(6 * j + tb) * n6 + 6 * j + ta], s, fixed);
      } else if (l < 27) {
        acc_add(&W.b[6 * j + (l - 21)], s, fixed);
      }
    }
    if (!iv) return;
    double hji = 0.0;
#pragma unroll
    for (int k = 0; k < 6; k++) hji = fma(__shfl(s, tri(ja, k), 64), Ajb[k], hji);
    double hii = 0.0, vi = 0.0;
#pragma unroll
    for (int k = 0; k < 6; k++) {
      double u = 0.0;
#pragma unroll
      for (int m = 0; m < 6; m++) u = fma(__shfl(s, k >= m ? k * (k + 1) / 2 + m : m * (m + 1) / 2 + k, 64), Atb[m], u);
      hii = fma(Ata[k], u, hii);
      vi = fma(Ava[k], __shfl(s, 21 + k, 64), vi);
    }
    if (jv && l < 36) h_add_pair(W, n6, 6 * j + ja, 6 * i + jb, hji, lower, fixed);
    if (l < 21) {
      acc_add(&W.H[(size_t)(6 * i + ta) * n6 + 6 * i + tb], hii, fixed);
      if (ta != tb && !lower) acc_add(&W.H[(size_t)(6 * i + tb) * n6 + 6 * i + ta], hii, fixed);
    } else if (l < 27) {
      acc_add(&W.b[6 * i + va], vi, fixed);
    }
    return;
  }
}

__global__ __launch_bounds__(256) void ba_assemble_kernel(const int64_t *__restrict__ ii,
                                                          const int64_t *__restrict__ jj,
                                                          const uint8_t *__restrict__ frame_owned, int N,
                                                          int t0, int P, int lower, BaTables T, BaBuffers W) {
  ba_assemble_block((int)blockIdx.x, ii, jj, frame_owned, N, t0, P, lower, T, W);
}

__global__ __launch_bounds__(256) void ba_schur_kernel(const int64_t *__restrict__ ii,
                                                       const int64_t *__restrict__ jj,
                                                       const uint8_t *__restrict__ frame_owned, int N, int HW,
                                                       int t0, int P, int lower, BaTables T, BaBuffers W) {
  __shared__ float red[4][44];
  const int tid = threadIdx.x, lane = tid & 63, wv = tid >> 6;
  const int n6 = 6 * P;
  const int ablk = (N + 3) / 4;
  if ((int)blockIdx.x < ablk) {
    if (blockIdx.y == 0 && blockIdx.z == 0)
      ba_assemble_block((int)blockIdx.x, ii, jj, frame_owned, N, t0, P, lower, T, W);
    return;
  }
  const int r1 = (int)blockIdx.x - ablk;
  const int4 ri = *reinterpret_cast<const int4 *>(T.rowinfo + 8 * r1);
  const int m = ri.x, tgt1 = ri.y, first_partner = ri.z, e1 = ri.w;
  if (m < 0) return;
  if (frame_owned && !frame_owned[T.rowinfo[8 * r1 + 4]]) return;
  const int chunk = (HW + gridDim.z - 1) / gridDim.z;
  const int k0 = blockIdx.z * chunk, k1 = min(HW, k0 + chunk);

  const float *E1 = W.E + (size_t)r1 * 6 * HW;
  const float *Qm = W.Q + (size_t)m * HW;
  const float *wm = W.w + (size_t)m * HW;

  for (int pe = first_partner - 1 + (int)blockIdx.y; pe < e1; pe += gridDim.y) {
    const bool self = (pe == first_partner - 1);
    const int2 ei = self ? make_int2(0, 0) : *reinterpret_cast<const int2 *>(T.einfo + 2 * pe);
    const int r2 = self ? r1 : P + ei.x;
    const int tgt2 = self ? tgt1 : ei.y - t0;
    if (tgt2 < 0 || tgt2 >= P) continue;
    const float *E2 = W.E + (size_t)r2 * 6 * HW;

    float acc[36];
    float sv[6];
#pragma unroll
    for (int c = 0; c < 36; c++) acc[c] = 0.f;
#pragma unroll
    for (int c = 0; c < 6; c++) sv[c] = 0.f;
    for (int k = k0 + tid; k < k1; k += 256) {
      const float q = Qm[k];
      float e1v[6], e2v[6];
#pragma unroll
      for (int c = 0; c < 6; c++) {
        e1v[c] = E1[(size_t)c * HW + k] * q;
        e2v[c] = E2[(size_t)c * HW + k];
      }
#pragma unroll
      for (int a = 0; a < 6; a++)
#pragma unroll
        for (int b = 0; b < 6; b++) acc[a * 6 + b] = fmaf(e1v[a], e2v[b], acc[a * 6 + b]);
      if (self) {
        const float wk = wm[k];
#pragma unroll
        for (int c = 0; c < 6; c++) sv[c] = fmaf(e1v[c], wk, sv[c]);
      }
    }
    __syncthreads();
#pragma unroll
    for (int c = 0; c < 36; c++) {
      const float r = wave_sum_to_lane63(acc[c]);
      if (lane == 63) red[wv][c] = r;
    }
    if (self) {
#pragma unroll
      for (int c = 0; c < 6; c++) {
        const float r = wave_sum_to_lane63(sv[c]);
        if (lane == 63) red[wv][36 + c] = r;
      }
    }
    __syncthreads();
    if (tid < 36) {
      const double s = (double)red[0][tid] + (double)red[1][tid] + (double)red[2][tid] + (double)red[3][tid];
      const int a = tid / 6, b = tid % 6;
      if (!self) h_add_pair(W, n6, 6 * tgt1 + a, 6 * tgt2 + b, -s, (lower & 1) != 0, (lower & 2) != 0);
      else if (!(lower & 1) || a >= b) acc_add(&W.H[(size_t)(6 * tgt1 + a) * n6 + 6 * tgt2 + b], -s, (lower & 2) != 0);
    } else if (self && tid < 42) {
      const double s = (double)red[0][tid] + (double)red[1][tid] + (double)red[2][tid] + (double)red[3][tid];
      acc_add(&W.b[6 * tgt1 + (tid - 36)], -s, (lower & 2) != 0);
    }
  }
}

constexpr int GRAM_MAX_T = 5;
constexpr int GRAM_MAX_ROWS = (16 * GRAM_MAX_T - 1) / 6;
constexpr int GRAM_MAX_TILES = GRAM_MAX_T * (GRAM_MAX_T + 1) / 2;
typedef double gram_d4 __attribute__((ext_vector_type(4)));

template <int T>
struct GramStage {
  lin_f4 q;
  lin_f4 e[T];
};

template <int T, bool VEC>
__device__ __forceinline__ void gram_load(GramStage<T> &S, const float *const (&bp)[T], const float *qm, int g, int gend,
                                          int c0, int c1, int lk) {
  const int p4 = c0 + 16 * g + 4 * lk;
  if (g < gend && p4 + 3 < c1) {
    if constexpr (VEC) {
      S.q = *reinterpret_cast<const lin_f4 *>(qm + p4);
#pragma unroll
      for (int t = 0; t < T; t++) S.e[t] = *reinterpret_cast<const lin_f4 *>(bp[t] + p4);
    } else {
#pragma unroll
      for (int s = 0; s < 4; s++) S.q[s] = qm[p4 + s];
#pragma unroll
      for (int t = 0; t < T; t++)
#pragma unroll
        for (int s = 0; s < 4; s++) S.e[t][s] = bp[t][p4 + s];
    }
  } else {
#pragma unroll
    for (int s = 0; s < 4; s++) {
      const bool ok = (g < gend) && (p4 + s < c1);
      const int pi = ok ? p4 + s : c0;
      const float qv = qm[pi];
      S.q[s] = ok ? qv : 0.f;
#pragma unroll
      for (int t = 0; t < T; t++) {
        const float ev = bp[t][pi];
        S.e[t][s] = ok ? ev : 0.f;
      }
    }
  }
}

template <int T>
__device__ __forceinline__ void gram_mac(const GramStage<T> &S, gram_d4 (&acc)[T * (T + 1) / 2]) {
#pragma unroll
  for (int s = 0; s < 4; s++) {
    double a[T], b[T];
    const double qs = (double)S.q[s];
#pragma unroll
    for (int t = 0; t < T; t++) {
      b[t] = (double)S.e[t][s];
      a[t] = b[t] * qs;
    }
#pragma unroll
    for (int ti = 0; ti < T; ti++)
#pragma unroll
      for (int tj = 0; tj <= ti; tj++)
        acc[ti * (ti + 1) / 2 + tj] =
            __builtin_amdgcn_mfma_f64_16x16x4f64(a[ti], b[tj], acc[ti * (ti + 1) / 2 + tj], 0, 0, 0);
  }
}

template <int T>
__device__ __forceinline__ void gram_mac_f32(const GramStage<T> &S, gram_d4 (&acc)[T * (T + 1) / 2]) {
#pragma unroll
  for (int ti = 0; ti < T; ti++) {
    float a[4];
#pragma unroll
    for (int s = 0; s < 4; s++) a[s] = S.e[ti][s] * S.q[s];
#pragma unroll
    for (int tj = 0; tj <= ti; tj++) {
      lin_f4 c = {0.f, 0.f, 0.f, 0.f};
#pragma unroll
      for (int s = 0; s < 4; s++) c = __builtin_amdgcn_mfma_f32_16x16x4f32(a[s], S.e[tj][s], c, 0, 0, 0);
#pragma unroll
      for (int r = 0; r < 4; r++) acc[ti * (ti + 1) / 2 + tj][r] += (double)c[r];
    }
  }
}

template <int T, bool VEC, bool F32>
__device__ __forceinline__ void gram_frame(const BaBuffers &W, const float *wm, const float *qm, int my_row, int nrows,
                                           int c0, int c1, int HW, double *red) {
  constexpr int NT = T * (T + 1) / 2;
  constexpr int UNR = (T <= 2) ? 4 : (T == 3 ? 2 : 1);
  const int lane = threadIdx.x & 63, wv = threadIdx.x >> 6, li = lane & 15, lk = lane >> 4;
  const float *bp[T];
#pragma unroll
  for (int t = 0; t < T; t++) {
    const int c = 16 * t + li;
    const int a = (c > 0) ? (c - 1) / 6 : 0;
    const int comp = (c > 0) ? (c - 1) - 6 * a : 0;
    const int erow = __shfl(my_row, a, 64);
    bp[t] = (c == 0 || a >= nrows) ? wm : W.E + ((size_t)erow * 6 + comp) * HW;
  }
  gram_d4 acc[NT];
#pragma unroll
  for (int i = 0; i < NT; i++) acc[i] = gram_d4{0.0, 0.0, 0.0, 0.0};

  const int ngroups = (c1 - c0 + 15) / 16;
  const int nw = (int)(blockDim.x >> 6);
  const int per = (ngroups + nw - 1) / nw;
  const int gbeg = wv * per, gend = min(ngroups, gbeg + per);
  GramStage<T> A[UNR], B[UNR];
#pragma unroll
  for (int u = 0; u < UNR; u++) gram_load<T, VEC>(A[u], bp, qm, gbeg + u, gend, c0, c1, lk);
  for (int g = gbeg; g < gend; g += 2 * UNR) {
#pragma unroll
    for (int u = 0; u < UNR; u++) gram_load<T, VEC>(B[u], bp, qm, g + UNR + u, gend, c0, c1, lk);
#pragma unroll
    for (int u = 0; u < UNR; u++)
      if (g + u < gend) {
        if constexpr (F32) gram_mac_f32<T>(A[u], acc);
        else gram_mac<T>(A[u], acc);
      }
#pragma unroll
    for (int u = 0; u < UNR; u++) gram_load<T, VEC>(A[u], bp, qm, g + 2 * UNR + u, gend, c0, c1, lk);
#pragma unroll
    for (int u = 0; u < UNR; u++)
      if (g + UNR + u < gend) {
        if constexpr (F32) gram_mac_f32<T>(B[u], acc);
        else gram_mac<T>(B[u], acc);
      }
  }
  for (int w = 0; w < nw; w++) {
    if (wv == w) {
#pragma unroll
      for (int i = 0; i < NT; i++)
#pragma unroll
        for (int r = 0; r < 4; r++) {
          double *p = red + (i * 4 + r) * 64 + lane;
          *p = (w == 0) ? acc[i][r] : *p + acc[i][r];
        }
    }
    __syncthreads();
  }
}

__device__ void gram_frame_pairs(const BaBuffers &W, const float *wm, const float *qm, const int *frow, int nrows, int c0,
                                 int c1, int HW, int n6, bool lower, bool fixed, float *red) {
  const int tid = threadIdx.x, lane = tid & 63, wv = tid >> 6;
  for (int a = 0; a < nrows; a++) {
    const float *E1 = W.E + (size_t)frow[2 * a] * 6 * HW;
    const int tgt1 = frow[2 * a + 1];
    for (int b = a; b < nrows; b++) {
      const bool self = (a == b);
      const float *E2 = W.E + (size_t)frow[2 * b] * 6 * HW;
      const int tgt2 = frow[2 * b + 1];
      float acc[36], sv[6];
#pragma unroll
      for (int c = 0; c < 36; c++) acc[c] = 0.f;
#pragma unroll
      for (int c = 0; c < 6; c++) sv[c] = 0.f;
      for (int k = c0 + tid; k < c1; k += (int)blockDim.x) {
        const float q = qm[k];
        float e1v[6], e2v[6];
#pragma unroll
        for (int c = 0; c < 6; c++) {
          e1v[c] = E1[(size_t)c * HW + k] * q;
          e2v[c] = E2[(size_t)c * HW + k];
        }
#pragma unroll
        for (int x = 0; x < 6; x++)
#pragma unroll
          for (int y = 0; y < 6; y++) acc[x * 6 + y] = fmaf(e1v[x], e2v[y], acc[x * 6 + y]);
        if (self) {
          const float wk = wm[k];
#pragma unroll
          for (int c = 0; c < 6; c++) sv[c] = fmaf(e1v[c], wk, sv[c]);
        }
      }
      __syncthreads();
#pragma unroll
      for (int c = 0; c < 36; c++) {
        const float r = wave_sum_to_lane63(acc[c]);
        if (lane == 63) red[wv * 44 + c] = r;
      }
      if (self) {
#pragma unroll
        for (int c = 0; c < 6; c++) {
          const float r = wave_sum_to_lane63(sv[c]);
          if (lane == 63) red[wv * 44 + 36 + c] = r;
        }
      }
      __syncthreads();
      const int nw = (int)(blockDim.x >> 6);
      if (tid < 36) {
        double s = 0.0;
        for (int w = 0; w < nw; w++) s += (double)red[w * 44 + tid];
        const int x = tid / 6, y = tid % 6;
        if (!self) h_add_pair(W, n6, 6 * tgt1 + x, 6 * tgt2 + y, -s, lower, fixed);
        else if (!lower || x >= y) acc_add(&W.H[(size_t)(6 * tgt1 + x) * n6 + 6 * tgt2 + y], -s, fixed);
      } else if (self && tid < 42) {
        double s = 0.0;
        for (int w = 0; w < nw; w++) s += (double)red[w * 44 + tid];
        acc_add(&W.b[6 * tgt1 + (tid - 36)], -s, fixed);
      }
    }
  }
}

template <bool VEC, bool F32>
__global__ __launch_bounds__(512, 2) void ba_schur_gram_kernel(const int64_t *__restrict__ ii, const int64_t *__restrict__ jj,
                                                               const uint8_t *__restrict__ frame_owned, int N, int HW,
                                                               int t0, int P, int nch, int lower, BaTables T, BaBuffers W) {
  __shared__ double red[GRAM_MAX_TILES * 256];
  __shared__ int s_tgt[64];
  const int tid = threadIdx.x, lane = tid & 63;
  const int ablk = (N + 3) / 4;
  if ((int)blockIdx.x < ablk) {
    if (tid < 256) ba_assemble_block((int)blockIdx.x, ii, jj, frame_owned, N, t0, P, lower, T, W);
    return;
  }
  const int fblk = (int)blockIdx.x - ablk;
  const int m = fblk / nch, ch = fblk - m * nch;
  const int4 fh = *reinterpret_cast<const int4 *>(T.fhead + 4 * m);
  const int frame = fh.x, nrows = fh.z;
  if (frame < 0 || nrows == 0) return;
  if (frame_owned && !frame_owned[frame]) return;
  const int cpx = ((HW + nch - 1) / nch + 15) / 16 * 16;
  const int c0 = ch * cpx, c1 = min(HW, c0 + cpx);
  if (c0 >= c1) return;
  const float *wm = W.w + (size_t)m * HW, *qm = W.Q + (size_t)m * HW;
  const int n6 = 6 * P;
  const int *frow = T.frow + 2 * fh.y;
  if (nrows > GRAM_MAX_ROWS) {
    gram_frame_pairs(W, wm, qm, frow, nrows, c0, c1, HW, n6, (lower & 1) != 0, (lower & 2) != 0, reinterpret_cast<float *>(red));
    return;
  }
  int my_row = 0, my_tgt = 0;
  if (lane < nrows) {
    const int2 rt = *reinterpret_cast<const int2 *>(frow + 2 * lane);
    my_row = rt.x, my_tgt = rt.y;
  }
  if (tid < 64) s_tgt[lane] = my_tgt;
  const int R = 1 + 6 * nrows, Tn = (R + 15) / 16;
  switch (Tn) {
    case 1: gram_frame<1, VEC, F32>(W, wm, qm, my_row, nrows, c0, c1, HW, red); break;
    case 2: gram_frame<2, VEC, F32>(W, wm, qm, my_row, nrows, c0, c1, HW, red); break;
    case 3: gram_frame<3, VEC, F32>(W, wm, qm, my_row, nrows, c0, c1, HW, red); break;
    case 4: gram_frame<4, VEC, F32>(W, wm, qm, my_row, nrows, c0, c1, HW, red); break;
    default: gram_frame<5, VEC, F32>(W, wm, qm, my_row, nrows, c0, c1, HW, red); break;
  }
  const int ntiles = Tn * (Tn + 1) / 2;
  const int r = (tid >> 6) & 3, li = lane & 15, lk = lane >> 4;
  const int tgroups = (int)(blockDim.x >> 8);
  int ti = 0, tj = 0;
  for (int idx = 0; idx < ntiles; idx++) {
    if (idx % tgroups != (tid >> 8)) {
      if (++tj > ti) ti++, tj = 0;
      continue;
    }
    const int i = 16 * ti + (F32 ? 4 * lk + r : lk + 4 * r), j = 16 * tj + li;
    if (i < R && j <= i && i >= 1) {
      const double s = -red[(idx * 4 + r) * 64 + lane];
      const int a = (i - 1) / 6, ca = (i - 1) - 6 * a;
      const int hr = 6 * s_tgt[a] + ca;
      if (j == 0) {
        acc_add(&W.b[hr], s, (lower & 2) != 0);
      } else {
        const int b = (j - 1) / 6, cb = (j - 1) - 6 * b;
        const int hc = 6 * s_tgt[b] + cb;
        if (i == j) acc_add(&W.H[(size_t)hr * n6 + hc], s, (lower & 2) != 0);
        else h_add_pair(W, n6, hr, hc, s, (lower & 1) != 0, (lower & 2) != 0);
      }
    }
    if (++tj > ti) ti++, tj = 0;
  }
}
#define GRAM_INST(V, F)                                                                                                  \
  template __global__ void ba_schur_gram_kernel<V, F>(const int64_t *, const int64_t *, const uint8_t *, int, int, int, int, \
                                                      int, int, BaTables, BaBuffers);
GRAM_INST(true, true)
GRAM_INST(true, false)
GRAM_INST(false, true)
GRAM_INST(false, false)
#undef GRAM_INST

__global__ __launch_bounds__(256) void ba_fixed_to_f64_kernel(double *__restrict__ H, double *__restrict__ b, int n) {
  const int idx = blockIdx.x * blockDim.x + threadIdx.x;
  double *p = (idx < n * n) ? H + idx : ((idx < n * n + n) ? b + (idx - n * n) : nullptr);
  if (!p) return;
  const long long v = *reinterpret_cast<const long long *>(p);
  *p = (double)v * (1.0 / ACC_FIX_SCALE);
}

__global__ __launch_bounds__(256) void ba_symmetrize_kernel(double *__restrict__ H, int n) {
  const int idx = blockIdx.x * blockDim.x + threadIdx.x;
  if (idx >= n * n) return;
  const int i = idx / n, j = idx - i * n;
  if (j > i) H[idx] = H[(size_t)j * n + i];
}

__global__ __launch_bounds__(256) void ba_export_kernel(const double *__restrict__ H, const double *__restrict__ b, int n,
                                                        double *__restrict__ out, int gtsam, ExportArg arg, double stab,
                                                        unsigned *__restrict__ counter, int *__restrict__ host_flag, int seq) {
  const int ld = gtsam ? n + 1 : n;
  const int total = n * ld + (gtsam ? 0 : n);
  const int idx = blockIdx.x * blockDim.x + threadIdx.x;
  auto h = [&](int i, int j) {
    const double x = H[(size_t)max(i, j) * n + min(i, j)];
    return (gtsam && i == j && i < 6) ? x + stab : x;
  };
  if (idx < total) {
    double r;
    if (!gtsam) {
      if (idx < n * n) {
        const int i = idx / n, j = idx - i * n;
        r = H[(size_t)max(i, j) * n + min(i, j)];
      } else {
        r = b[idx - n * n];
      }
    } else {
      const int i = idx / ld, j = idx - i * ld;
      const int p = i / 6, a = i - 6 * p;
      if (j == n) {
        r = 0.0;
#pragma unroll
        for (int k = 0; k < 6; k++) r = fma(arg.A[6 * k + a], b[6 * p + k], r);
      } else {
        const int q = j / 6, c = j - 6 * q;
        r = 0.0;
#pragma unroll
        for (int k = 0; k < 6; k++) {
          double t = 0.0;
#pragma unroll
          for (int l = 0; l < 6; l++) t = fma(h(6 * p + k, 6 * q + l), arg.A[6 * l + c], t);
          r = fma(arg.A[6 * k + a], t, r);
        }
      }
    }
    out[idx] = r;
  }
  __threadfence_system();
  __syncthreads();
  if (threadIdx.x == 0) {
    const unsigned done = atomicAdd(counter, 1u);
    if (done == gridDim.x - 1) {
      *counter = 0;
      __threadfence_system();
      __hip_atomic_store(host_flag, seq, __ATOMIC_RELEASE, __HIP_MEMORY_SCOPE_SYSTEM);
    }
  }
}

__global__ __launch_bounds__(256) void ba_update_kernel(float *__restrict__ poses, const float *__restrict__ poses_src,
                                                        float *__restrict__ disps,
                                                        const int64_t *__restrict__ jj,
                                                        const uint8_t *__restrict__ frame_owned, int HW,
                                                        int t0, int P, int update_poses, int update_disps,
                                                        float *__restrict__ dz_out,
                                                        float *__restrict__ dx_out, BaTables T, BaBuffers W,
                                                        float disp_floor) {
  const int m = blockIdx.y;
  if (T.gkey[7]) {
    if (m == T.Mmax && blockIdx.x == 0 && dx_out)
      for (int i = threadIdx.x; i < 6 * P; i += blockDim.x) dx_out[i] = 0.f;
    const int k = blockIdx.x * blockDim.x + threadIdx.x;
    if (m < T.Mmax && k < HW && dz_out && update_disps) dz_out[(size_t)m * HW + k] = 0.f;
    return;
  }
  if (m > T.Mmax) {
    const int frame = m - T.Mmax - 1;
    const int slot = T.frame_slot[frame];
    if (update_disps && slot >= 0 && slot < T.meta[0] && (!frame_owned || frame_owned[frame])) return;
    const int k = blockIdx.x * blockDim.x + threadIdx.x;
    if (k >= HW) return;
    const size_t fk = (size_t)frame * HW + k;
    if (disps[fk] < disp_floor) disps[fk] = disp_floor;
    return;
  }
  if (m == T.Mmax) {
    if (blockIdx.x != 0) return;
    if (dx_out)
      for (int i = threadIdx.x; i < 6 * P; i += blockDim.x) dx_out[i] = W.dx[i];
    if (!update_poses) return;
    for (int p = threadIdx.x; p < P; p += blockDim.x) {
      float pr[7];
      load_pose(poses_src ? poses_src : poses, W.dx, t0 + p, t0, P, true, pr);
#pragma unroll
      for (int c = 0; c < 7; c++) poses[7 * (t0 + p) + c] = pr[c];
    }
    return;
  }
  if (!update_disps) return;
  const int M = T.meta[0];
  if (m >= M) return;
  const int frame = T.kx[m];
  if (frame_owned && !frame_owned[frame]) return;
  const int k = blockIdx.x * blockDim.x + threadIdx.x;
  if (k >= HW) return;

  const float dz = backsub_pixel(T, W, m, frame, k, HW, t0, P);
  const size_t mk = (size_t)m * HW + k;
  const size_t fk = (size_t)frame * HW + k;
  float d = disps[fk] + dz;
  if (disp_floor > 0.f) d = (d < disp_floor) ? disp_floor : d;
  disps[fk] = d;
  if (dz_out) dz_out[mk] = dz;
}

__global__ __launch_bounds__(256) void ba_gather_edges_kernel(const float2 *__restrict__ tgt_inac, const float2 *__restrict__ wgt_inac,
                                                              const int64_t *__restrict__ ii_inac, const int64_t *__restrict__ jj_inac,
                                                              const int64_t *__restrict__ sel, int n_sel, int n_inac,
                                                              const float2 *__restrict__ tgt_act, const float2 *__restrict__ wgt_act,
                                                              const int64_t *__restrict__ ii_act, const int64_t *__restrict__ jj_act,
                                                              int HW, float *__restrict__ tgt_out, float *__restrict__ wgt_out,
                                                              int64_t *__restrict__ ii_out, int64_t *__restrict__ jj_out) {
  const int o = blockIdx.y, k = blockIdx.x * 256 + threadIdx.x;
  const bool inac = o < n_sel;
  int64_t src = inac ? (sel ? sel[o] : (int64_t)o) : (int64_t)(o - n_sel);
  if (inac) src = (src < 0) ? src + n_inac : src;
  const bool bad = inac && (src < 0 || src >= n_inac);
  if (bad) src = 0;
  if (blockIdx.x == 0 && blockIdx.z == 0 && threadIdx.x == 0) {
    ii_out[o] = inac ? ii_inac[src] : ii_act[src];
    jj_out[o] = inac ? jj_inac[src] : jj_act[src];
  }
  if (k >= HW) return;
  const float2 *in = blockIdx.z ? (inac ? wgt_inac : wgt_act) : (inac ? tgt_inac : tgt_act);
  float *out = blockIdx.z ? wgt_out : tgt_out;
  float2 v = in[(size_t)src * HW + k];
  if (bad) v = make_float2(0.f, 0.f);
  out[((size_t)o * 2 + 0) * HW + k] = v.x;
  out[((size_t)o * 2 + 1) * HW + k] = v.y;
}

__global__ void ba_copy_f32_kernel(const float *__restrict__ src, float *__restrict__ dst, int n) {
  const int i = blockIdx.x * blockDim.x + threadIdx.x;
  if (i < n) dst[i] = src[i];
}

}
```

dba-fusion_amd/dbaf_amd/_lib.py:

```python
import ctypes
import os
import weakref

import torch

_HERE = os.path.dirname(os.path.abspath(__file__))
LIB_PATH = os.environ.get("DBA_HIP_LIB") or os.path.join(os.path.dirname(_HERE), "lib", "libdba_hip.so")

DBA_F32, DBA_F16, DBA_F64 = 0, 1, 2
_ERR = {-1: "DBA_ERR_ARG", -2: "DBA_ERR_WORKSPACE", -3: "DBA_ERR_HIP", -4: "DBA_ERR_UNSUPPORTED"}

c_int, c_float, c_size_t, c_void_p = ctypes.c_int, ctypes.c_float, ctypes.c_size_t, ctypes.c_void_p


class BaLayout(ctypes.Structure):
    _fields_ = [(n, c_size_t) for n in ("H", "b", "dx", "meta", "E", "Q", "w", "kx")] + \
               [("P", c_int), ("Mmax", c_int), ("nchunks", c_int)]


class ShardExchange(ctypes.Structure):
    _fields_ = [("world", c_int), ("rank", c_int), ("comm", c_void_p), ("peer_regions", c_void_p),
                ("peer_epoch", ctypes.POINTER(ctypes.c_uint)), ("peer_max_doubles", c_size_t), ("peer_status", c_void_p),
                ("band_idx", c_void_p), ("band_len", c_size_t), ("band_buf", c_void_p),
                ("my_rows", c_void_p), ("n_mine", c_int), ("kmax", c_int), ("all_rows", c_void_p), ("all_slots", c_void_p),
                ("n_all", c_int), ("send", c_void_p), ("recv", c_void_p)]


class RowJob(ctypes.Structure):
    _fields_ = [("src", c_void_p), ("dst", c_void_p), ("pos", c_void_p), ("row_bytes", ctypes.c_int64),
                ("count", c_int), ("dst_row0", c_int), ("src_rows", c_int), ("dst_rows", c_int)]


class AfJob(ctypes.Structure):
    _fields_ = [("kind", c_int), ("reserved", c_int), ("rows", RowJob)]


class AfGeometry(ctypes.Structure):
    _fields_ = [("poses", c_void_p), ("disps", c_void_p), ("intrinsics_b4", c_void_p), ("ii", c_void_p), ("jj", c_void_p),
                ("n_frames", c_int), ("ht", c_int), ("wd", c_int), ("reserved", c_int)]


_P = c_void_p
SYMBOLS = {
    "dba_version": (ctypes.c_char_p, []),
    "dba_last_error": (ctypes.c_char_p, []),
    "dba_ba_workspace_bytes": (c_size_t, [c_int] * 6),
    "dba_ba_get_layout": (c_int, [c_int] * 6 + [ctypes.POINTER(BaLayout)]),
    "dba_ba_prepare": (c_int, [_P, _P] + [c_int] * 6 + [_P, c_size_t, _P]),
    "dba_ba_prepare_keyed": (c_int, [_P, _P] + [c_int] * 8 + [_P, c_size_t, _P]),
    "dba_ba_workspace_init": (c_int, [c_int] * 6 + [_P, c_size_t, _P]),
    "dba_ba_solver_verdict": (c_int, [c_int] * 6 + [_P, c_size_t]),
    "dba_ba_poll_eta_error": (c_int, [ctypes.POINTER(c_int), ctypes.POINTER(c_int)]),
    "dba_ba_poll_eta_error_ws": (c_int, [c_int] * 6 + [_P, c_size_t, ctypes.POINTER(c_int), ctypes.POINTER(c_int)]),
    "dba_ba_gather_edges": (c_int, [_P] * 4 + [c_int, _P, c_int] + [_P] * 4 + [c_int] * 3 + [_P] * 5),
    "dba_ba_linearize": (c_int, [_P] * 7 + [c_int] + [_P] * 3 + [c_int] * 6 + [c_float, _P, c_size_t, _P]),
    "dba_ba_reduce": (c_int, [_P] * 3 + [c_int] * 7 + [_P, c_size_t, _P]),
    "dba_ba_schur_select": (c_int, [c_int]),
    "dba_ba_schur_select_thread": (c_int, [c_int]),
    "dba_ba_schur_auto_form": (c_int, [c_int, c_int]),
    "dba_ba_schur_thread_form": (c_int, []),
    "dba_ba_schur_generation": (c_int, []),
    "dba_ba_set_deterministic": (c_int, [c_int]),
    "dba_ba_set_solve_check": (c_int, [c_int]),
    "dba_ba_solve_check": (c_int, [c_int] * 6 + [c_float, c_float, _P, c_size_t, _P]),
    "dba_ba_symmetrize": (c_int, [c_int] * 6 + [_P, c_size_t, _P]),
    "dba_ba_solve": (c_int, [c_int] * 6 + [c_float, c_float, _P, c_size_t, _P]),
    "dba_ba_solve_skyline": (c_int, [c_int] * 6 + [c_float, c_float, _P, _P, c_size_t, _P]),
    "dba_ba_update": (c_int, [_P] * 5 + [c_int] * 8 + [_P, _P, c_size_t, _P]),
    "dba_ba_shard_front": (c_int, [_P] * 7 + [c_int] + [_P] * 3 + [c_int] * 6 + [c_float, c_int, _P, c_size_t, _P]),
    "dba_ba_shard_back": (c_int, [_P] * 5 + [c_int] * 6 + [c_float, c_float, c_int, _P, c_int, _P, c_size_t, _P]),
    "dba_comm_unique_id": (c_int, [_P]),
    "dba_comm_create": (c_int, [_P, c_int, c_int, ctypes.POINTER(_P)]),
    "dba_comm_destroy": (c_int, [_P]),
    "dba_comm_info": (c_int, [_P, ctypes.POINTER(c_int), ctypes.POINTER(c_int)]),
    "dba_comm_allreduce_f64": (c_int, [_P, c_size_t, _P]),
    "dba_ba_sharded_run": (c_int, [_P] * 7 + [c_int] + [_P] * 3 + [c_int] * 7 + [c_float, c_float, c_float, c_int, _P, c_int,
                                                                                  c_int, ctypes.POINTER(ShardExchange), _P,
                                                                                  c_size_t, _P]),
    "dba_ba": (c_int, [_P] * 7 + [c_int] + [_P, _P] + [c_int] * 7 + [c_float, c_float, c_int, _P, _P, _P,
                                                                     c_size_t, _P]),
    "dba_ba_prepared": (c_int, [_P] * 7 + [c_int] + [_P, _P] + [c_int] * 7 + [c_float, c_float, c_int, _P, _P, _P,
                                                                              c_size_t, _P, c_int]),
    "dba_ba_run": (c_int, [_P] * 7 + [c_int] + [_P, _P] + [c_int] * 7 + [c_float, c_float, c_int, _P, _P, _P,
                                                                         c_size_t, _P, c_int, c_int, c_float]),
    "dba_bacore_hessian": (c_int, [_P] * 7 + [c_int] + [_P, _P] + [c_int] * 6 + [_P, _P, _P, c_size_t, _P]),
    "dba_bacore_hessian_run": (c_int, [_P] * 7 + [c_int] + [_P, _P] + [c_int] * 6 + [_P, _P, _P, c_size_t, _P, c_int]),
    "dba_bacore_staging": (c_int, [c_int] * 6 + [_P, c_size_t, ctypes.POINTER(ctypes.c_void_p)]),
    "dba_bacore_export_host": (c_int, [c_int] * 6 + [_P, c_size_t, _P, c_int, _P, ctypes.c_double, ctypes.POINTER(ctypes.c_void_p)]),
    "dba_bacore_hessian_host": (c_int, [_P] * 7 + [c_int] + [_P, _P] + [c_int] * 6 + [_P, c_size_t, _P, c_int, c_int, _P,
                                        ctypes.c_double, ctypes.POINTER(ctypes.c_void_p)]),
    "dba_bacore_retract": (c_int, [_P] * 4 + [c_int] * 6 + [_P, _P, _P, _P, c_size_t, _P]),
    "dba_bacore_optimize": (c_int, [_P, _P] + [c_int] * 6 + [c_float, c_float, _P, _P, c_size_t, _P]),
    "dba_corr_index_forward": (c_int, [_P, _P, _P] + [c_int] * 7 + [_P]),
    "dba_corr_lookup_pyramid": (c_int, [_P, _P, _P] + [c_int] * 8 + [_P]),
    "dba_corr_volume_build_sheared_supported": (c_int, [c_int] * 6),
    "dba_corr_volume_build_sheared": (c_int, [_P, _P, _P] + [c_int] * 7 + [_P, c_size_t, _P]),
    "dba_corr_sheared_plane_elems": (c_int, [c_int, c_int]),
    "dba_corr_sheared_tiled": (c_int, [c_int, c_int]),
    "dba_corr_sheared_grid": (c_int, [c_int, c_int, _P, _P]),
    "dba_corr_lookup_select": (c_int, [c_int]),
    "dba_corr_lookup_arm_timing": (c_int, [_P, _P]),
    "dba_corr_shear_level": (c_int, [_P, _P] + [c_int] * 6 + [_P]),
    "dba_corr_lookup_pyramid_sheared": (c_int, [_P, _P, _P] + [c_int] * 7 + [_P]),
    "dba_corr_lookup_level_sheared": (c_int, [_P, _P, _P] + [c_int] * 7 + [_P]),
    "dba_corr_lookup_level_sheared_slots": (c_int, [_P, _P, _P, _P] + [c_int] * 7 + [_P]),
    "dba_corr_shear_level_slots": (c_int, [_P, _P, _P, _P] + [c_int] * 6 + [_P]),
    "dba_corr_volume_build_sheared_slots": (c_int, [_P, _P, _P, _P] + [c_int] * 7 + [_P, c_size_t, _P]),
    "dba_corr_lookup_pyramid_sheared_slots": (c_int, [_P, _P, _P, _P] + [c_int] * 7 + [_P]),
    "dba_corr_lookup_pyramid_slots": (c_int, [_P, _P, _P, _P] + [c_int] * 8 + [_P]),
    "dba_corr_lookup_reproject_sheared": (c_int, [_P] * 10 + [c_int] * 7 + [_P]),
    "dba_corr_lookup_reproject_motion_sheared": (c_int, [_P] * 12 + [c_int] * 7 + [_P]),
    "dba_corr_index_backward": (c_int, [_P, _P, _P] + [c_int] * 6 + [_P]),
    "dba_corr_volume_scratch_bytes": (c_size_t, [c_int] * 6),
    "dba_corr_once_pyramid_bytes": (c_size_t, [c_int] * 6),
    "dba_corr_build_lookup_once_sheared": (c_int, [_P, _P, _P, _P, _P, c_size_t, _P, c_size_t] + [c_int] * 8 + [_P]),
    "dba_corr_volume_build": (c_int, [_P, _P, _P] + [c_int] * 7 + [_P, c_size_t, _P]),
    "dba_altcorr_forward": (c_int, [_P] * 4 + [c_int] * 8 + [_P]),
    "dba_altcorr_forward_t": (c_int, [_P] * 4 + [c_int] * 9 + [_P]),
    "dba_altcorr_pyramid_forward": (c_int, [_P] * 6 + [c_int] * 8 + [_P]),
    "dba_altcorr_pyramid_forward_f16maps": (c_int, [_P] * 6 + [c_int] * 7 + [_P]),
    "dba_altcorr_backward": (c_int, [_P] * 6 + [c_int] * 8 + [_P]),
    "dba_reproject": (c_int, [_P] * 5 + [c_int] * 3 + [_P, _P, _P]),
    "dba_frame_distance": (c_int, [_P] * 5 + [c_int] * 3 + [c_float, _P, _P]),
    "dba_projmap": (c_int, [_P] * 5 + [c_int] * 3 + [_P, _P, _P]),
    "dba_iproj": (c_int, [_P] * 3 + [c_int] * 3 + [_P, _P]),
    "dba_depth_filter": (c_int, [_P] * 5 + [c_int] * 4 + [_P, _P]),
    "dba_peer_exchange_bytes": (c_size_t, [c_size_t]),
    "dba_peer_exchange_create": (c_int, [c_size_t, ctypes.POINTER(_P), _P]),
    "dba_peer_exchange_open": (c_int, [_P, ctypes.POINTER(_P)]),
    "dba_peer_exchange_close": (c_int, [_P, c_int]),
    "dba_peer_allreduce_f64": (c_int, [_P, c_size_t, _P, c_int, c_int, ctypes.c_uint, c_size_t, _P, _P]),
    "dba_cvx_upsample_disp": (c_int, [_P, c_int, _P, _P] + [c_int] * 4 + [_P, c_int, _P, _P]),
    "dba_segment_reduce": (c_int, [_P, c_int, _P, c_int, ctypes.c_int64, ctypes.c_int64, c_int, c_int, _P, _P]),
    "dba_frame_distance_bidir": (c_int, [_P] * 5 + [c_int] * 4 + [c_float, _P, _P]),
    "dba_proximity_edges_capacity": (c_int, [c_int] * 5),
    "dba_proximity_edges": (c_int, [_P] * 3 + [c_int] * 7 + [c_float, ctypes.c_double, c_int, c_int, _P, c_int, c_int]
                            + [_P, _P, c_int, _P, _P, c_int, _P, _P]),
    "dba_filter_repeated_edges": (c_int, [_P, _P, c_int, _P, _P, c_int, _P, _P, _P, _P]),
    "dba_select_edges": (c_int, [_P, _P, _P, c_int, c_int, _P, ctypes.c_int64, ctypes.c_int64, _P, _P, c_int, _P, _P, _P,
                                 _P]),
    "dba_move_rows": (c_int, [ctypes.POINTER(RowJob), c_int, _P]),
    "dba_shift_rows": (c_int, [ctypes.POINTER(_P), ctypes.POINTER(ctypes.c_int64), ctypes.POINTER(ctypes.c_int64), c_int,
                               ctypes.c_int64, _P]),
    "dba_add_factors_plan": (c_int, [_P, _P, _P, c_int, _P, _P, c_int, _P, _P, c_int] + [c_int] * 4 + [_P, _P, _P, _P]),
    "dba_add_factors_payload": (c_int, [ctypes.POINTER(AfJob), c_int, ctypes.POINTER(AfGeometry), _P]),
    "dba_update_inputs_edges": (c_int, [_P, _P, c_int, _P, _P, c_int, _P, c_int, c_int, ctypes.c_int64, ctypes.c_int64,
                                        c_float, c_int] + [_P] * 7),
    "dba_update_inputs_payload": (c_int, [_P, _P, c_int, _P, _P, c_int, _P, _P, c_int, c_int, c_int, c_float, c_int,
                                          c_float] + [_P] * 5 + [c_int] * 3 + [_P] * 4),
    "dba_update_inputs_payload_op": (c_int, [_P, _P, c_int, _P, _P, _P, c_int, c_int, _P, _P, c_int, c_int, c_int, c_float,
                                             c_int, c_float] + [_P] * 5 + [c_int] * 3 + [_P] * 6),
    "dba_update_inputs_poll": (c_int, [ctypes.POINTER(c_int)]),
    "dba_vio_window_plan": (c_int, [_P, _P, c_int] + [ctypes.c_int64] * 3 + [_P, _P, c_int, ctypes.c_int64] + [_P] * 8),
    "dba_vio_window_payload": (c_int, [ctypes.POINTER(RowJob), c_int, _P, ctypes.POINTER(c_int), _P]),
    "dba_vio_window_poll": (c_int, [ctypes.POINTER(c_int)]),
    "dba_keyframe_report_words": (c_int, []),
    "dba_keyframe_report": (c_int, [_P, ctypes.POINTER(_P), ctypes.POINTER(c_int)]),
    "dba_keyframe_check": (c_int, [_P] * 3 + [c_int] * 4 + [c_float, _P, c_int, _P]),
    "dba_keyframe_flow_magnitude": (c_int, [_P, c_int, c_int, _P, c_int, _P]),
    "dba_keyframe_wait": (c_int, [_P, c_int]),
}

_lib = None


def load():
    global _lib
    if _lib is None:
        if not os.path.exists(LIB_PATH):
            raise RuntimeError(
                "dba_hip: %s not found -- build it with `make lib` (hipcc --offload-arch=gfx950); "
                "there is no CPU fallback for the DBA hot path" % LIB_PATH)
        lib = ctypes.CDLL(LIB_PATH)
        for name, (res, args) in SYMBOLS.items():
            fn = getattr(lib, name)
            fn.restype = res
            fn.argtypes = args
        _lib = lib
    return _lib


def schur_generation():
    lib = load()
    return (lib.dba_ba_schur_generation(), lib.dba_ba_schur_thread_form())


def check(rc, what):
    if rc != 0:
        msg = _ERR.get(rc, str(rc))
        detail = load().dba_last_error().decode() if rc == -3 else ""
        raise RuntimeError("dba_hip: %s failed with %s %s" % (what, msg, detail))



def ptr(x):
    return ctypes.c_void_p(x.data_ptr()) if x is not None and x.numel() else None


def require(cond, op, msg):
    if not cond:
        raise ValueError("%s (MI355X): %s" % (op, msg))


def stream(dev):
    return ctypes.c_void_p(torch.cuda.current_stream(dev).cuda_stream)


def check_edge_list(op, dev, x, nm):
    require(isinstance(x, torch.Tensor) and x.is_cuda and (dev is None or x.device == dev), op,
            "%s must be a HIP device tensor%s; no CPU path" % (nm, "" if dev is None else " on %s" % dev))
    require(x.dtype == torch.int64 and x.dim() == 1 and x.is_contiguous(), op,
            "%s must be a contiguous 1-D int64 tensor" % nm)


def dev_tensor(op, x, nm, dev, dtype, aligned=False):
    require(isinstance(x, torch.Tensor) and x.is_cuda and (dev is None or x.device == dev), op,
            "%s must be a HIP device tensor%s; no CPU path" % (nm, "" if dev is None else " on %s" % dev))
    require(x.dtype == dtype, op, "%s must be %s, got %s" % (nm, dtype, x.dtype))
    require(x.is_contiguous(), op, "%s must be contiguous" % nm)
    require(not aligned or x.data_ptr() % 16 == 0, op, "%s must be 16-byte aligned" % nm)


def edge_list(op, x, nm, dev, max_edges, aligned=False):
    dev_tensor(op, x, nm, dev, torch.int64, aligned)
    require(x.dim() == 1, op, "%s must be 1-D, got %s" % (nm, tuple(x.shape)))
    require(x.shape[0] <= max_edges, op, "%s: %d edges exceed the supported %d" % (nm, x.shape[0], max_edges))


class EdgeSetMemo:

    def __init__(self, capacity=8):
        self.capacity = capacity
        self._entries = []

    def __len__(self):
        return len(self._entries)

    def lookup(self, lists, key):
        for refs, k, value in reversed(self._entries):
            if k == key and len(refs) == len(lists) and all(r() is x and v == x._version for (r, v), x in zip(refs, lists)):
                return value
        return None

    def remember(self, lists, key, value):
        live = [e for e in self._entries if all(r() is not None for r, _ in e[0])]
        self._entries = live[max(0, len(live) - (self.capacity - 1)):]
        self._entries.append((tuple((weakref.ref(x), x._version) for x in lists), key, value))

    def clear(self):
        del self._entries[:]
```

include/dba_hip.h:

```cpp
#ifndef DBA_HIP_H
#define DBA_HIP_H

#include <stddef.h>
#include <stdint.h>

#ifdef __cplusplus
extern "C" {
#endif

enum {
  DBA_OK = 0,
  DBA_ERR_ARG = -1,
  DBA_ERR_WORKSPACE = -2,
  DBA_ERR_HIP = -3,
  DBA_ERR_UNSUPPORTED = -4
};

enum { DBA_F32 = 0, DBA_F16 = 1, DBA_F64 = 2 };

typedef void *dba_stream_t;

const char *dba_version(void);
const char *dba_last_error(void);


size_t dba_ba_workspace_bytes(int N, int B, int ht, int wd, int t0, int t1);

typedef struct {
  size_t H, b, dx, meta, E, Q, w, kx;
  int P, Mmax, nchunks;
} dba_ba_layout;
int dba_ba_get_layout(int N, int B, int ht, int wd, int t0, int t1, dba_ba_layout *out);

int dba_ba_prepare(const int64_t *ii, const int64_t *jj, int N, int B, int ht, int wd, int t0, int t1,
                   void *ws, size_t ws_bytes, dba_stream_t stream);
int dba_ba_prepare_keyed(const int64_t *ii, const int64_t *jj, int N, int B, int ht, int wd, int t0, int t1, int eta_rows,
                         int check, void *ws, size_t ws_bytes, dba_stream_t stream);
int dba_ba_solver_verdict(int N, int B, int ht, int wd, int t0, int t1, void *ws, size_t ws_bytes);
int dba_ba_workspace_init(int N, int B, int ht, int wd, int t0, int t1, void *ws, size_t ws_bytes, dba_stream_t stream);
int dba_ba_poll_eta_error(int *eta_rows, int *num_kx);
int dba_ba_poll_eta_error_ws(int N, int B, int ht, int wd, int t0, int t1, void *ws, size_t ws_bytes, int *eta_rows, int *num_kx);

int dba_ba_gather_edges(const float *target_inac, const float *weight_inac, const int64_t *ii_inac, const int64_t *jj_inac,
                        int n_inac, const int64_t *sel, int n_sel, const float *target_act, const float *weight_act,
                        const int64_t *ii_act, const int64_t *jj_act, int n_act, int ht, int wd, float *targets_out,
                        float *weights_out, int64_t *ii_out, int64_t *jj_out, dba_stream_t stream);

int dba_ba_linearize(const float *poses, const float *disps, const float *intrinsics,
                     const float *disps_sens, const float *targets, const float *weights,
                     const float *eta, int eta_rows, const int64_t *ii, const int64_t *jj,
                     const uint8_t *frame_owned, int N, int B, int ht, int wd, int t0, int t1,
                     float alpha, void *ws, size_t ws_bytes, dba_stream_t stream);

int dba_ba_reduce(const int64_t *ii, const int64_t *jj, const uint8_t *frame_owned, int N, int B,
                  int ht, int wd, int t0, int t1, int motion_only, void *ws, size_t ws_bytes,
                  dba_stream_t stream);

int dba_ba_schur_select(int form);
int dba_ba_schur_select_thread(int form);
int dba_ba_schur_thread_form(void);
int dba_ba_schur_auto_form(int N, int P);
int dba_ba_schur_generation(void);

int dba_ba_set_deterministic(int on);

int dba_ba_set_solve_check(int on);
int dba_ba_solve_check(int N, int B, int ht, int wd, int t0, int t1, float lm, float ep, void *ws, size_t ws_bytes,
                       dba_stream_t stream);

int dba_ba_symmetrize(int N, int B, int ht, int wd, int t0, int t1, void *ws, size_t ws_bytes, dba_stream_t stream);

int dba_ba_solve(int N, int B, int ht, int wd, int t0, int t1, float lm, float ep, void *ws,
                 size_t ws_bytes, dba_stream_t stream);
int dba_ba_solve_skyline(int N, int B, int ht, int wd, int t0, int t1, float lm, float ep, const int32_t *fpose, void *ws,
                         size_t ws_bytes, dba_stream_t stream);

int dba_ba_update(float *poses, float *disps, const int64_t *ii, const int64_t *jj,
                  const uint8_t *frame_owned, int N, int B, int ht, int wd, int t0, int t1,
                  int update_poses, int update_disps, float *dz_out, void *ws, size_t ws_bytes,
                  dba_stream_t stream);

int dba_ba_shard_front(const float *poses, const float *disps, const float *intrinsics, const float *disps_sens,
                       const float *targets, const float *weights, const float *eta, int eta_rows, const int64_t *ii,
                       const int64_t *jj, const uint8_t *frame_owned, int N, int B, int ht, int wd, int t0, int t1,
                       float alpha, int motion_only, void *ws, size_t ws_bytes, dba_stream_t stream);
int dba_ba_shard_back(float *poses, float *disps, const int64_t *ii, const int64_t *jj, const uint8_t *frame_owned,
                      int N, int B, int ht, int wd, int t0, int t1, float lm, float ep, int update_disps,
                      const int32_t *window_fpose, int solver_hint, void *ws, size_t ws_bytes, dba_stream_t stream);

typedef struct dba_comm dba_comm;
int dba_comm_unique_id(void *id128);
int dba_comm_create(const void *id128, int world, int rank, dba_comm **out);
int dba_comm_destroy(dba_comm *c);
int dba_comm_info(dba_comm *c, int *world, int *rank);
int dba_comm_allreduce_f64(dba_comm *c, double *buf, size_t count, dba_stream_t stream);

typedef struct {
  int world, rank;
  dba_comm *comm;
  void *const *peer_regions;
  unsigned *peer_epoch;
  size_t peer_max_doubles;
  int *peer_status;
  const int64_t *band_idx;
  size_t band_len;
  double *band_buf;
  const int64_t *my_rows;
  int n_mine, kmax;
  const int64_t *all_rows, *all_slots;
  int n_all;
  float *send, *recv;
} dba_shard_exchange;

int dba_ba_sharded_run(float *poses, float *disps, const float *intrinsics, const float *disps_sens, const float *targets,
                       const float *weights, const float *eta, int eta_rows, const int64_t *ii, const int64_t *jj,
                       const uint8_t *frame_owned, int N, int B, int ht, int wd, int t0, int t1, int iterations, float lm,
                       float ep, float alpha, int motion_only, const int32_t *window_fpose, int solver_hint, int prepared,
                       const dba_shard_exchange *x, void *ws, size_t ws_bytes, dba_stream_t stream);

int dba_ba(float *poses, float *disps, const float *intrinsics, const float *disps_sens,
           const float *targets, const float *weights, const float *eta, int eta_rows,
           const int64_t *ii, const int64_t *jj, int N, int B, int ht, int wd, int t0, int t1,
           int iterations, float lm, float ep, int motion_only, float *dx_out, float *dz_out,
           void *ws, size_t ws_bytes, dba_stream_t stream);

int dba_ba_prepared(float *poses, float *disps, const float *intrinsics, const float *disps_sens,
                    const float *targets, const float *weights, const float *eta, int eta_rows,
                    const int64_t *ii, const int64_t *jj, int N, int B, int ht, int wd, int t0, int t1,
                    int iterations, float lm, float ep, int motion_only, float *dx_out, float *dz_out,
                    void *ws, size_t ws_bytes, dba_stream_t stream, int solver_hint);

int dba_ba_run(float *poses, float *disps, const float *intrinsics, const float *disps_sens,
               const float *targets, const float *weights, const float *eta, int eta_rows,
               const int64_t *ii, const int64_t *jj, int N, int B, int ht, int wd, int t0, int t1,
               int iterations, float lm, float ep, int motion_only, float *dx_out, float *dz_out,
               void *ws, size_t ws_bytes, dba_stream_t stream, int prepared, int solver_hint, float disp_floor);

int dba_bacore_hessian_run(const float *poses, const float *disps, const float *intrinsics,
                           const float *disps_sens, const float *targets, const float *weights,
                           const float *eta, int eta_rows, const int64_t *ii, const int64_t *jj, int N,
                           int B, int ht, int wd, int t0, int t1, double *H_host, double *v_host,
                           void *ws, size_t ws_bytes, dba_stream_t stream, int prepared);

int dba_bacore_hessian_host(const float *poses, const float *disps, const float *intrinsics,
                            const float *disps_sens, const float *targets, const float *weights,
                            const float *eta, int eta_rows, const int64_t *ii, const int64_t *jj, int N,
                            int B, int ht, int wd, int t0, int t1, void *ws, size_t ws_bytes, dba_stream_t stream,
                            int prepared, int layout, const double *A36, double stabilizer, double **out_host);

int dba_bacore_staging(int N, int B, int ht, int wd, int t0, int t1, void *ws, size_t ws_bytes, double **out_host);

int dba_bacore_export_host(int N, int B, int ht, int wd, int t0, int t1, void *ws, size_t ws_bytes, dba_stream_t stream, int layout,
                           const double *A36, double stabilizer, double **out_host);

int dba_bacore_hessian(const float *poses, const float *disps, const float *intrinsics,
                       const float *disps_sens, const float *targets, const float *weights,
                       const float *eta, int eta_rows, const int64_t *ii, const int64_t *jj, int N,
                       int B, int ht, int wd, int t0, int t1, double *H_host, double *v_host, void *ws,
                       size_t ws_bytes, dba_stream_t stream);

int dba_bacore_retract(float *poses, float *disps, const int64_t *ii, const int64_t *jj, int N, int B,
                       int ht, int wd, int t0, int t1, const double *dx_host, float *dx_out,
                       float *dz_out, void *ws, size_t ws_bytes, dba_stream_t stream);

int dba_bacore_optimize(const double *H_host, const double *v_host, int N, int B, int ht, int wd,
                        int t0, int t1, float lm, float ep, float *dx_out, void *ws, size_t ws_bytes,
                        dba_stream_t stream);


int dba_corr_index_forward(const void *volume, const float *coords, void *corr, int n, int h1, int w1,
                           int h2, int w2, int radius, int dtype, dba_stream_t stream);

int dba_corr_lookup_pyramid(const void *const *volumes ,
                            const float *coords_nhw2, void *corr, int n, int h1, int w1, int h2,
                            int w2, int num_levels, int radius, int dtype, dba_stream_t stream);

int dba_corr_sheared_plane_elems(int h1, int w1);
int dba_corr_sheared_tiled(int h1, int w1);
int dba_corr_sheared_grid(int h1, int w1, int *h1g, int *w1g);
int dba_corr_lookup_select(int kernel);
int dba_corr_lookup_arm_timing(void *start_event, void *stop_event);
int dba_corr_volume_build_sheared_supported(int C, int h1, int w1, int h2, int w2, int num_levels);
int dba_corr_volume_build_sheared(const void *fmap1, const void *fmap2, void *const *sheared_levels, int n, int C,
                                  int h1, int w1, int h2, int w2, int num_levels, void *scratch,
                                  size_t scratch_bytes, dba_stream_t stream);
int dba_corr_shear_level(const void *ref_level, void *sheared_level, int n, int h1, int w1, int h2l, int w2l,
                         int lvl, dba_stream_t stream);
int dba_corr_lookup_pyramid_sheared(const void *const *volumes ,
                                    const float *coords_nhw2, void *corr, int n, int h1, int w1, int h2,
                                    int w2, int num_levels, int radius, dba_stream_t stream);

int dba_corr_volume_build_sheared_slots(const void *fmap1, const void *fmap2, void *const *level_stores,
                                        const int *out_slots , int n, int C, int h1, int w1, int h2,
                                        int w2, int num_levels, void *scratch, size_t scratch_bytes, dba_stream_t stream);
int dba_corr_lookup_pyramid_sheared_slots(const void *const *level_stores, const int *slots ,
                                          const float *coords_nhw2, void *corr, int n, int h1, int w1, int h2, int w2,
                                          int num_levels, int radius, dba_stream_t stream);
int dba_corr_lookup_pyramid_slots(const void *const *level_stores, const int *slots, const float *coords_nhw2, void *corr,
                                  int n, int h1, int w1, int h2, int w2, int num_levels, int radius, int dtype,
                                  dba_stream_t stream);

int dba_corr_lookup_reproject_sheared(const void *const *level_stores, const int *slots, const float *poses,
                                      const float *disps, const float *intrinsics_b4, const int64_t *ii, const int64_t *jj,
                                      float *coords_out, float *valid_out, void *corr, int n, int h1, int w1, int h2, int w2,
                                      int num_levels, int radius, dba_stream_t stream);

int dba_corr_lookup_reproject_motion_sheared(const void *const *level_stores, const int *slots, const float *poses,
                                             const float *disps, const float *intrinsics_b4, const int64_t *ii,
                                             const int64_t *jj, float *coords_out, float *valid_out, void *corr,
                                             const float *target, float *motn, int n, int h1, int w1, int h2, int w2,
                                             int num_levels, int radius, dba_stream_t stream);

size_t dba_corr_once_pyramid_bytes(int n, int h1, int w1, int h2, int w2, int num_levels);
int dba_corr_build_lookup_once_sheared(const void *fmap1, const void *fmap2, const float *coords_nhw2, void *corr, void *pyramid,
                                       size_t pyramid_bytes, void *scratch, size_t scratch_bytes, int n, int C, int h1, int w1,
                                       int h2, int w2, int num_levels, int radius, dba_stream_t stream);

int dba_corr_lookup_level_sheared(const void *sheared_level, const float *coords_n2hw_scaled, void *corr, int n, int h1,
                                  int w1, int h2, int w2, int lvl, int radius, dba_stream_t stream);

int dba_corr_lookup_level_sheared_slots(const void *sheared_store, const int *slots, const float *coords_n2hw_scaled,
                                        void *corr, int n, int h1, int w1, int h2, int w2, int lvl, int radius,
                                        dba_stream_t stream);
int dba_corr_shear_level_slots(const void *ref_level, void *sheared_store, const int *src_idx, const int *dst_slots, int n,
                               int h1, int w1, int h2l, int w2l, int lvl, dba_stream_t stream);

int dba_corr_index_backward(const float *coords, const float *corr_grad, float *volume_grad, int n,
                            int h1, int w1, int h2, int w2, int radius, dba_stream_t stream);

size_t dba_corr_volume_scratch_bytes(int n, int C, int h1, int w1, int h2, int w2);
int dba_corr_volume_build(const void *fmap1, const void *fmap2, void *const *levels ,
                          int n, int C, int h1, int w1, int h2, int w2, int num_levels, void *scratch,
                          size_t scratch_bytes, dba_stream_t stream);

int dba_altcorr_forward(const float *fmap1, const float *fmap2, const float *coords, float *corr, int B,
                        int S, int H1, int W1, int H2, int W2, int C, int radius, dba_stream_t stream);
int dba_altcorr_forward_t(const void *fmap1, const void *fmap2, const float *coords, void *corr, int B, int S,
                          int H1, int W1, int H2, int W2, int C, int radius, int dtype, dba_stream_t stream);

int dba_altcorr_pyramid_forward(const void *fmap1, const void *const *fmap2_levels ,
                                const int64_t *ii, const int64_t *jj, const float *coords, void *corr, int B, int S, int H1,
                                int W1, int C, int num_levels, int radius, int dtype, dba_stream_t stream);

int dba_altcorr_pyramid_forward_f16maps(const void *fmap1, const void *const *fmap2_levels ,
                                        const int64_t *ii, const int64_t *jj, const float *coords, float *corr, int B, int S,
                                        int H1, int W1, int C, int num_levels, int radius, dba_stream_t stream);

int dba_altcorr_backward(const float *fmap1, const float *fmap2, const float *coords, const float *corr_grad,
                         float *fmap1_grad, float *fmap2_grad, int B, int S, int H1, int W1, int H2, int W2,
                         int C, int radius, dba_stream_t stream);


int dba_reproject(const float *poses, const float *disps, const float *intrinsics_b4,
                  const int64_t *ii, const int64_t *jj, int N, int ht, int wd, float *coords,
                  float *valid, dba_stream_t stream);

int dba_frame_distance(const float *poses, const float *disps, const float *intrinsics,
                       const int64_t *ii, const int64_t *jj, int N, int ht, int wd, float beta,
                       float *dist, dba_stream_t stream);

int dba_projmap(const float *poses, const float *disps, const float *intrinsics, const int64_t *ii,
                const int64_t *jj, int N, int ht, int wd, float *coords, float *valid,
                dba_stream_t stream);

int dba_iproj(const float *poses, const float *disps, const float *intrinsics, int nm, int ht, int wd,
              float *points, dba_stream_t stream);

int dba_depth_filter(const float *poses, const float *disps, const float *intrinsics,
                     const int64_t *inds, const float *thresh, int num, int nbuf, int ht, int wd,
                     float *counter, dba_stream_t stream);

int dba_cvx_upsample_disp(const float *disps, int n_disps, const int64_t *src_rows, const void *mask, int mask_dtype,
                          int B, int ht, int wd, float *out, int n_out, const int64_t *dst_rows, dba_stream_t stream);
int dba_segment_reduce(const void *src, int dtype, const int64_t *index, int n, int64_t outer, int64_t inner,
                       int dim_size, int mean, void *out, dba_stream_t stream);

int dba_frame_distance_bidir(const float *poses, const float *disps, const float *intrinsics, const int64_t *ii,
                             const int64_t *jj, int N, int n_frames, int ht, int wd, float beta, float *dist,
                             dba_stream_t stream);
int dba_proximity_edges_capacity(int t, int t0, int rad, int stereo, int max_factors);
int dba_proximity_edges(const float *poses, const float *disps, const float *intrinsics, int ht, int wd, int t,
                        int t0, int t1, int rad, int nms, float beta, double thresh, int max_factors, int stereo,
                        const int *skip_edge_host, int n_skip, int frontend_window, const int64_t *ex_ii,
                        const int64_t *ex_jj, int n_ex, float *dist, int64_t *edges, int capacity, int *count,
                        dba_stream_t stream);
int dba_filter_repeated_edges(const int64_t *ii, const int64_t *jj, int n, const int64_t *ex_ii, const int64_t *ex_jj,
                              int n_ex, int64_t *out_ii, int64_t *out_jj, int *count, dba_stream_t stream);

#define DBA_SEL_MASK 0
#define DBA_SEL_RULE_OR 1
#define DBA_SEL_RULE_AND 2
#define DBA_SEL_KEYFRAME 3
#define DBA_SEL_ROLL 4
#define DBA_SEL_SHIFT 5
#define DBA_SEL_MAX_EDGES 8192
#define DBA_MAX_ROW_JOBS 8
#define DBA_MAX_SHIFT_BUFS 12
typedef struct dba_row_job {
  const void *src;
  void *dst;
  const int *pos;
  int64_t row_bytes;
  int count, dst_row0, src_rows, dst_rows;
} dba_row_job;
int dba_select_edges(const int64_t *ii, const int64_t *jj, const int64_t *age, int n, int mode,
                     const unsigned char *mask, int64_t a, int64_t b, const int64_t *pre_ii, const int64_t *pre_jj,
                     int n_pre, int64_t *keep, int64_t *drop, int *sel, dba_stream_t stream);
int dba_move_rows(const dba_row_job *jobs_host, int n_jobs, dba_stream_t stream);
int dba_shift_rows(void *const *bases_host, const int64_t *row_bytes_host, const int64_t *rows_host, int n_bufs,
                   int64_t ix, dba_stream_t stream);

#define DBA_AF_INFO_WORDS 8
#define DBA_AF_BAD_RANGE 1
#define DBA_AF_BAD_STEREO 2
#define DBA_AF_MAX_JOBS 16
#define DBA_AF_COPY 0
#define DBA_AF_GATHER 1
#define DBA_AF_ZERO 2
#define DBA_AF_REPROJECT 3
typedef struct dba_af_job {
  int kind, reserved;
  dba_row_job rows;
} dba_af_job;
typedef struct dba_af_geometry {
  const float *poses;
  const float *disps;
  const float *intrinsics_b4;
  const int64_t *ii, *jj;
  int n_frames, ht, wd, reserved;
} dba_af_geometry;
int dba_add_factors_plan(const int64_t *ii, const int64_t *jj, const int64_t *age, int n, const int64_t *ii_inac,
                         const int64_t *jj_inac, int n_inac, const int64_t *prop_ii, const int64_t *prop_jj, int n_prop,
                         int max_factors, int may_evict, int n_frames, int cams, int64_t *lists, int64_t *inac,
                         int *info, dba_stream_t stream);
int dba_add_factors_payload(const dba_af_job *jobs_host, int n_jobs, const dba_af_geometry *geom_host,
                            dba_stream_t stream);

#define DBA_UI_MAX_FRAMES 1024
#define DBA_UI_RES_WORDS 16
int dba_update_inputs_edges(const int64_t *ii_inac, const int64_t *jj_inac, int n_inac, const int64_t *ii_act,
                            const int64_t *jj_act, int n_act, const float *poses, int n_frames, int has_t0, int64_t t0,
                            int64_t inac_range, float mask_threshold, int baseline_rule, int *sel, int64_t *ii_out,
                            int64_t *jj_out, unsigned char *flags, int64_t *kx, int *res, dba_stream_t stream);
int dba_update_inputs_payload(const float *target_inac, const float *weight_inac, int n_inac, const float *target_act,
                              const float *weight_act, int n_act, const float *disps, const float *damping,
                              int n_frames, int ht, int wd, float far_threshold, int far_rule, float ep, const int *sel,
                              const int64_t *ii_out, const unsigned char *flags, const int64_t *kx, const int *res,
                              int exp_n_sel, int exp_N, int exp_n_kx, float *target_out, float *weight_out,
                              float *damping_out, dba_stream_t stream);
int dba_update_inputs_payload_op(const float *target_inac, const float *weight_inac, int n_inac, const float *coords1,
                                 const void *delta, const void *weight_op, int op_dtype, int n_act, const float *disps,
                                 const float *damping, int n_frames, int ht, int wd, float far_threshold, int far_rule,
                                 float ep, const int *sel, const int64_t *ii_out, const unsigned char *flags,
                                 const int64_t *kx, const int *res, int exp_n_sel, int exp_N, int exp_n_kx,
                                 float *target_out, float *weight_out, float *damping_out, float *target_new,
                                 float *weight_new, dba_stream_t stream);
int dba_update_inputs_poll(int *counts6);

#define DBA_VW_RES_WORDS 4
#define DBA_VW_MAX_JOBS 4
int dba_vio_window_plan(const int64_t *cur_ii, const int64_t *cur_jj, int n_cur, int64_t last_t0, int64_t lo,
                        int64_t last_t1, const int64_t *ii, const int64_t *jj, int n, int64_t t0, int64_t *marg_ii,
                        int64_t *marg_jj, int *marg_pos, int64_t *act_ii, int64_t *act_jj, int *act_pos, int *res,
                        dba_stream_t stream);
int dba_vio_window_payload(const dba_row_job *jobs_host, int n_jobs, const int *res, const int *expect4_host,
                           dba_stream_t stream);
int dba_vio_window_poll(int *words8);

#define DBA_KF_D 0
#define DBA_KF_WIN 1
#define DBA_KF_CAM 2
#define DBA_KF_MAT 9
#define DBA_KF_SEQ 25
#define DBA_KF_WORDS 26
int dba_keyframe_report_words(void);
int dba_keyframe_report(dba_stream_t stream, void **report, int *seq);
int dba_keyframe_check(const float *poses, const float *disps, const float *intrinsics, int n_frames, int ht, int wd,
                       int t1, float beta, void *report, int seq, dba_stream_t stream);
int dba_keyframe_flow_magnitude(const void *delta, int dtype, int n_pixels, void *report, int seq, dba_stream_t stream);
int dba_keyframe_wait(const void *report, int seq);

#define DBA_PEER_TIMEOUT 1
size_t dba_peer_exchange_bytes(size_t max_doubles);
int dba_peer_exchange_create(size_t bytes, void **region, unsigned char *handle64);
int dba_peer_exchange_open(const unsigned char *handle64, void **region);
int dba_peer_exchange_close(void *region, int opened);
int dba_peer_allreduce_f64(double *buf, size_t n, void *const *regions, int rank, int world, unsigned epoch,
                           size_t max_doubles, int *status, dba_stream_t stream);

#ifdef __cplusplus
}
#endif
#endif
```

Before: 4055.

## Precompute per-edge pose/adjoint table in prepare kernel for first linearize

```diff
diff --git a/dba-fusion_amd/csrc/ba_host.hip b/dba-fusion_amd/csrc/ba_host.hip
--- a/dba-fusion_amd/csrc/ba_host.hip
+++ b/dba-fusion_amd/csrc/ba_host.hip
@@ -37,12 +37,14 @@
   int gram_threads = num("DBA_SCHUR_WAVES") == 4 ? 256 : 512;
   bool gram_f32 = getenv("DBA_SCHUR_MFMA") ? is("DBA_SCHUR_MFMA", "f3") : GRAM_F32_DEFAULT;
   bool fuse_update = !is("DBA_BA_FUSE_UPDATE", "0");
+  int edge_table = !is("DBA_LIN_EDGE_TABLE", "0");
 };
 static const BaEnv &ba_env() { static const BaEnv env; return env; }
 
 static std::atomic<int> g_schur_form{ba_env().schur_form};
 static std::atomic<int> g_deterministic{ba_env().deterministic};
 static std::atomic<int> g_solve_check{ba_env().solve_check};
+static std::atomic<int> g_edge_table{ba_env().edge_table};
 
 __global__ __launch_bounds__(256) void ba_solve_check_kernel(const double *__restrict__ H, const double *__restrict__ b, int n, double lm,
                                                              double ep, float *__restrict__ dx, int *__restrict__ meta) {
@@ -127,11 +129,13 @@
   const size_t o_rowinfo = take(sizeof(int) * 8 * (size_t)(P + N > 0 ? P + N : 1));
   const size_t o_fhead = take(sizeof(int) * 4 * (size_t)(Mmax > 0 ? Mmax : 1));
   const size_t o_frow = take(sizeof(int) * 2 * (size_t)(P + N > 0 ? P + N : 1));
+  const size_t o_slotinfo = take(sizeof(int) * 4 * (size_t)(Mmax + 1));
   L.E = take(sizeof(float) * (size_t)(P + N) * 6 * HW);
   L.Q = take(sizeof(float) * (size_t)Mmax * HW);
   L.w = take(sizeof(float) * (size_t)Mmax * HW);
   const size_t o_hparte = take(sizeof(float) * (size_t)(N > 0 ? N : 1) * nparts_max * HPE_STRIDE);
   const size_t o_aedge = take(sizeof(double) * 36 * (size_t)(N > 0 ? N : 1));
+  const size_t o_etab = take(sizeof(float) * ETAB_WORDS * (size_t)(N > 0 ? N : 1));
   L.dx = take(sizeof(float) * (size_t)(n6 > 0 ? n6 : 1));
   const size_t o_ptmp = take(sizeof(float) * 2 * 7 * (size_t)B);
   L.H = take(sizeof(double) * (size_t)(n6 > 0 ? n6 * (size_t)n6 : 1));
@@ -166,6 +170,7 @@
     plan->T.fhead = reinterpret_cast<int *>(base + o_fhead);
     plan->T.frow = reinterpret_cast<int *>(base + o_frow);
     plan->T.gkey = reinterpret_cast<int *>(base + o_gkey);
+    plan->T.slotinfo = reinterpret_cast<int *>(base + o_slotinfo);
     plan->T.Mmax = Mmax;
     plan->T.B = B;
     plan->W.E = reinterpret_cast<float *>(base + L.E);
@@ -173,6 +178,7 @@
     plan->W.w = reinterpret_cast<float *>(base + L.w);
     plan->W.HpartE = reinterpret_cast<float *>(base + o_hparte);
     plan->W.Aedge = reinterpret_cast<double *>(base + o_aedge);
+    plan->W.etab = reinterpret_cast<float *>(base + o_etab);
     plan->W.dx = reinterpret_cast<float *>(base + L.dx);
     plan->W.poses_tmp = reinterpret_cast<float *>(base + o_ptmp);
     plan->W.H = reinterpret_cast<double *>(base + L.H);
@@ -185,7 +191,7 @@
 }
 
 static int ba_prepare_stage(const BaPlan &plan, const int64_t *ii, const int64_t *jj, int eta_rows, int check, bool judge_band,
-                            hipStream_t stream) {
+                            hipStream_t stream, const float *poses = nullptr) {
   const int N = plan.N, B = plan.B, P = plan.P;
   if (N > 0 && (!ii || !jj)) return DBA_ERR_ARG;
   const int want = std::max(std::max(N, B), P);
@@ -201,7 +207,8 @@
   int *band_verdict = max_nt ? solver_verdict_slot(plan.T.meta) : nullptr;
   hipLaunchKernelGGL(ba_prepare_kernel, dim3(1), dim3(threads), lds, stream, ii, jj, N, B, plan.t0, plan.t1,
                      (int)scan_ints, ba_schur_frame_form(N, P) ? 1 : 0, check ? 1 : 0, eta_rows,
-                     eta_rows > 1 ? ws_eta_status(plan.T.meta) : nullptr, plan.T, band_verdict, max_nt);
+                     eta_rows > 1 ? ws_eta_status(plan.T.meta) : nullptr, plan.T, band_verdict, max_nt, poses, plan.W.Aedge,
+                     plan.W.etab);
   DBA_LAUNCH_CHECK();
   return DBA_OK;
 }
@@ -307,8 +314,11 @@
 int ba_run_loop(const BaPlan &plan, const BaProblem &g, float *poses, float *disps, const BaRun &run, hipStream_t stream) {
   const int *fpose = run.window_fpose ? run.window_fpose : plan.T.fpose;
   int rc;
+  bool table_filled = false;
   if (run.prepared != 1) {
-    rc = ba_prepare_stage(plan, g.ii, g.jj, g.eta_rows, run.prepared == 2, run.window_fpose == nullptr, stream);
+    table_filled = g_edge_table.load(std::memory_order_relaxed) != 0 && !g.frame_owned && !run.exchange && plan.N > 0;
+    rc = ba_prepare_stage(plan, g.ii, g.jj, g.eta_rows, run.prepared == 2, run.window_fpose == nullptr, stream,
+                          table_filled ? poses : nullptr);
     if (rc != DBA_OK) return rc;
   }
   const bool fuse = ba_env().fuse_update;
@@ -316,7 +326,7 @@
   bool pending = false;
   for (int itr = 0; itr < run.iterations; itr++) {
     float *pose_dst = plan.W.poses_tmp + (size_t)(itr & 1) * 7 * plan.B;
-    const int upd = pending ? (run.motion_only ? 1 : 3) : 0;
+    const int upd = (pending ? (run.motion_only ? 1 : 3) : 0) | (table_filled && itr == 0 ? LIN_EDGE_TABLE : 0);
     rc = ba_linearize_stage(plan, g, pose_src, disps, run.alpha, upd, pending ? pose_dst : nullptr, disps, stream);
     if (rc != DBA_OK) return rc;
     if (pending) pose_src = pose_dst;
@@ -539,6 +549,11 @@
   return DBA_OK;
 }
 
+int dba_ba_set_edge_table(int on) {
+  g_edge_table.store(on ? 1 : 0, std::memory_order_relaxed);
+  return DBA_OK;
+}
+
 int dba_ba_set_solve_check(int on) {
   g_solve_check.store(on ? 1 : 0, std::memory_order_relaxed);
   return DBA_OK;
diff --git a/dba-fusion_amd/csrc/ba_kernels.h b/dba-fusion_amd/csrc/ba_kernels.h
--- a/dba-fusion_amd/csrc/ba_kernels.h
+++ b/dba-fusion_amd/csrc/ba_kernels.h
@@ -26,8 +26,14 @@
   int *fhead;
   int *frow;
   int *gkey;
+  int *slotinfo;
   int Mmax, B;
 };
+constexpr int SLOT_REFUSED = 1, SLOT_UNUSED = 2;
+
+constexpr int ETAB_WORDS = 44;
+constexpr int ETAB_POSE = 4, ETAB_ADJ = 16;
+constexpr int LIN_EDGE_TABLE = 4;
 
 struct BaBuffers {
   float *E;
@@ -35,6 +41,7 @@
   float *w;
   float *HpartE;
   double *Aedge;
+  float *etab;
   double *H;
   double *b;
   float *dx;
@@ -60,7 +67,8 @@
 
 constexpr int GKEY_MAGIC = 0x6b657935;
 __global__ void ba_prepare_kernel(const int64_t *ii, const int64_t *jj, int N, int B, int t0, int t1, int scan_ints,
-                                  int ftable, int check, int eta_rows, int *status, BaTables T, int *band_verdict, int max_nt);
+                                  int ftable, int check, int eta_rows, int *status, BaTables T, int *band_verdict, int max_nt,
+                                  const float *poses, double *Aedge, float *etab);
 bool ba_schur_frame_form(int N, int P);
 template <int PPL, bool MF, int EW>
 __global__ void ba_linearize_kernel(const float *poses, const float *disps, const float *intrinsics,
diff --git a/dba-fusion_amd/csrc/ba_kernels.hip b/dba-fusion_amd/csrc/ba_kernels.hip
--- a/dba-fusion_amd/csrc/ba_kernels.hip
+++ b/dba-fusion_amd/csrc/ba_kernels.hip
@@ -5,258 +5,6 @@
 #include <cstring>
 
 namespace dba {
-
-__device__ __forceinline__ int wave_incl_scan(int v, int lane) {
-#pragma unroll
-  for (int off = 1; off < 64; off <<= 1) {
-    const int o = __shfl_up(v, off, 64);
-    if (lane >= off) v += o;
-  }
-  return v;
-}
-
-__global__ __launch_bounds__(1024) void ba_prepare_kernel(const int64_t *__restrict__ ii,
-                                                          const int64_t *__restrict__ jj, int N, int B,
-                                                          int t0, int t1, int scan_ints, int ftable, int check,
-                                                          int eta_rows, int *__restrict__ status, BaTables T,
-                                                          int *__restrict__ band_verdict, int max_nt) {
-  extern __shared__ int sm[];
-  int *flag = sm;
-  int *cnt = sm + B;
-  int *kxs = cnt + T.Mmax + 1;
-  int *scan = kxs + T.Mmax;
-  int *vcnt = scan + scan_ints;
-  const int tid = threadIdx.x, nt = blockDim.x, lane = tid & 63, wave = tid >> 6, nw = nt >> 6;
-  const int P = t1 - t0;
-  const int my_i = (tid < N) ? (int)ii[tid] : -1, my_j = (tid < N) ? (int)jj[tid] : -1;
-  auto src = [&](int n) { return (n == tid) ? my_i : (int)ii[n]; };
-  auto dst = [&](int n) { return (n == tid) ? my_j : (int)jj[n]; };
-  auto check_eta = [&](int nk) {
-    if (tid == 0) {
-      const bool bad = eta_rows > 1 && eta_rows != nk;
-      T.gkey[7] = bad ? 1 : 0;
-      if (bad && status) {
-        status[1] = eta_rows, status[2] = nk;
-        __hip_atomic_store(status, 1, __ATOMIC_RELEASE, __HIP_MEMORY_SCOPE_SYSTEM);
-      }
-    }
-  };
-
-  {
-    const int *key = T.gkey;
-    bool same = check && key[0] == GKEY_MAGIC && key[1] == N && key[2] == B && key[3] == t0 && key[4] == t1 &&
-                key[5] == ftable && key[6] == T.Mmax;
-    if (same) {
-      for (int n = tid; n < N; n += nt) {
-        const long long a = (long long)ii[n], b = (long long)jj[n];
-        same = same && (long long)key[8 + n] == a && (long long)key[8 + N + n] == b;
-      }
-    }
-    if (__syncthreads_and(same)) {
-      check_eta(T.meta[0]);
-      return;
-    }
-  }
-
-  for (int f = tid; f < B; f += nt) flag[f] = 0;
-  for (int m = tid; m <= T.Mmax; m += nt) cnt[m] = 0;
-  __syncthreads();
-  for (int p = tid; p < P; p += nt) {
-    const int f = t0 + p;
-    if (f >= 0 && f < B) flag[f] = 1;
-  }
-  for (int n = tid; n < N; n += nt) {
-    const int f = src(n);
-    if (f >= 0 && f < B) flag[f] = 1;
-  }
-  __syncthreads();
-
-  const int per = (B + nt - 1) / nt;
-  const int lo = min(tid * per, B), hi = min(lo + per, B);
-  int c = 0;
-  for (int f = lo; f < hi; f++) c += flag[f];
-  const int incl = wave_incl_scan(c, lane);
-  if (lane == 63) scan[wave] = incl;
-  __syncthreads();
-  if (wave == 0) {
-    const int v = (lane < nw) ? scan[lane] : 0;
-    const int w = wave_incl_scan(v, lane);
-    if (lane < nw) scan[16 + lane] = w;
-  }
-  __syncthreads();
-  int slot = incl - c + (wave > 0 ? scan[16 + wave - 1] : 0);
-  const int M = scan[16 + nw - 1];
-  for (int f = lo; f < hi; f++) {
-    if (flag[f]) {
-      if (slot < T.Mmax) T.kx[slot] = f, kxs[slot] = f;
-      T.frame_slot[f] = (slot < T.Mmax) ? slot : -1;
-      flag[f] = slot + 1;
-      slot++;
-    } else {
-      T.frame_slot[f] = -1;
-    }
-  }
-  if (tid == 0) {
-    T.meta[0] = min(M, T.Mmax);
-    T.meta[1] = 0;
-    T.meta[2] = (M > T.Mmax) ? 1 : 0;
-    T.meta[7] = 0;
-    T.meta[16] = 0;
-  }
-  check_eta(min(M, T.Mmax));
-  __syncthreads();
-  auto slot_of = [&](int f) { return (f >= 0 && f < B && flag[f] > 0 && flag[f] <= T.Mmax) ? flag[f] - 1 : -1; };
-  auto emit_edge = [&](int n, int m, int pos, int jx) {
-    const int tg = jx - t0;
-    int *ri = T.rowinfo + 8 * (P + n);
-    const bool ok = m >= 0 && tg >= 0 && tg < P;
-    ri[0] = ok ? m : -1, ri[1] = tg, ri[2] = pos + 1, ri[3] = (m >= 0) ? cnt[m + 1] : 0, ri[4] = (m >= 0) ? kxs[m] : -1;
-    if (pos >= 0) T.einfo[2 * pos] = n, T.einfo[2 * pos + 1] = jx;
-  };
-
-  for (int n = tid; n < N; n += nt) {
-    const int m = slot_of(src(n));
-    if (m >= 0) atomicAdd(&cnt[m], 1);
-  }
-  __syncthreads();
-  if (wave == 0) {
-    int carry = 0;
-    for (int base = 0; base <= T.Mmax; base += 64) {
-      const int m = base + lane;
-      const int v = (m < T.Mmax) ? cnt[m] : 0;
-      const int w = wave_incl_scan(v, lane);
-      if (m <= T.Mmax) {
-        cnt[m] = carry + w - v;
-        T.eoff[m] = carry + w - v;
-      }
-      carry += __shfl(w, 63, 64);
-    }
-  }
-  __syncthreads();
-  int *sii = scan;
-  const int Mv0 = min(M, T.Mmax);
-  if (N <= nt) {
-    const bool myvalid = (tid < N) && (slot_of(my_i) >= 0) && (my_j - t0 >= 0) && (my_j - t0 < P);
-    constexpr int VBIT = 1 << 30;
-    if (tid < N) sii[tid] = (my_i & (VBIT - 1)) | (myvalid ? VBIT : 0);
-    if (ftable)
-      for (int m = tid; m <= T.Mmax; m += nt) {
-        const int pp = (m < Mv0) ? kxs[m] - t0 : -1;
-        vcnt[m] = (pp >= 0 && pp < P) ? 1 : 0;
-      }
-    __syncthreads();
-    int vrank = 0;
-    if (tid < N) {
-      const int f = my_i & (VBIT - 1), m = slot_of(my_i);
-      int pos = -1;
-      if (m >= 0) {
-        int rank = 0;
-        for (int q = 0; q < tid; q++) {
-          const int x = sii[q];
-          const bool same = ((x & (VBIT - 1)) == f);
-          rank += same;
-          vrank += same ? (x >> 30) : 0;
-        }
-        pos = cnt[m] + rank;
-        T.elist[pos] = tid;
-        if (myvalid && ftable) atomicAdd(&vcnt[m], 1);
-      }
-      emit_edge(tid, m, pos, my_j);
-    }
-    if (!ftable) {
-      for (int m = tid; m < T.Mmax; m += nt) T.fhead[4 * m] = -1, T.fhead[4 * m + 2] = 0;
-    } else {
-    __syncthreads();
-    if (wave == 0) {
-      int carry = 0;
-      for (int base = 0; base < T.Mmax; base += 64) {
-        const int m = base + lane;
-        const int v = (m < T.Mmax) ? vcnt[m] : 0;
-        const int w = wave_incl_scan(v, lane);
-        if (m < T.Mmax) {
-          const int pp = (m < Mv0) ? kxs[m] - t0 : -1;
-          const bool own = (pp >= 0 && pp < P);
-          const int off = carry + w - v;
-          int *fh = T.fhead + 4 * m;
-          fh[0] = (m < Mv0) ? kxs[m] : -1, fh[1] = off, fh[2] = v, fh[3] = 0;
-          if (own) T.frow[2 * off] = pp, T.frow[2 * off + 1] = pp;
-          vcnt[m] = off + (own ? 1 : 0);
-        }
-        carry += __shfl(w, 63, 64);
-      }
-    }
-    __syncthreads();
-    if (myvalid) {
-      const int o = vcnt[slot_of(my_i)] + vrank;
-      T.frow[2 * o] = P + tid, T.frow[2 * o + 1] = my_j - t0;
-    }
-    }
-  } else {
-    for (int m = tid; m < T.Mmax; m += nt) T.fhead[4 * m] = -1, T.fhead[4 * m + 2] = 0;
-    for (int n = tid; n < N; n += nt) T.elist_rank[n] = 0;
-    for (int base = 0; base < N; base += 1024) {
-      __syncthreads();
-      for (int q = tid; q < 1024 && base + q < N; q += nt) sii[q] = (int)ii[base + q];
-      __syncthreads();
-      const int lim = min(1024, N - base);
-      for (int n = tid; n < N; n += nt) {
-        if (n <= base) continue;
-        const int f = (int)ii[n];
-        if (slot_of(f) < 0) continue;
-        int rank = 0;
-        const int qend = min(lim, n - base);
-        for (int q = 0; q < qend; q++) rank += (sii[q] == f);
-        T.elist_rank[n] += rank;
-      }
-    }
-    __syncthreads();
-    for (int n = tid; n < N; n += nt) {
-      const int m = slot_of((int)ii[n]);
-      const int pos = (m >= 0) ? cnt[m] + T.elist_rank[n] : -1;
-      if (m >= 0) T.elist[pos] = n;
-      emit_edge(n, m, pos, (int)jj[n]);
-    }
-  }
-  for (int p = tid; p < P; p += nt) {
-    const int m = slot_of(t0 + p);
-    int *ri = T.rowinfo + 8 * p;
-    ri[0] = m, ri[1] = p, ri[2] = (m >= 0) ? cnt[m] : 0, ri[3] = (m >= 0) ? cnt[m + 1] : 0, ri[4] = t0 + p;
-  }
-  __syncthreads();
-  const int Mv = min(M, T.Mmax);
-  int *minS = cnt;
-  int *fps = scan;
-  for (int m = tid; m < Mv; m += nt) {
-    const int pp = kxs[m] - t0;
-    minS[m] = (pp >= 0 && pp < P) ? pp : 0x7fffffff;
-  }
-  for (int pp = tid; pp < P; pp += nt) fps[pp] = pp;
-  __syncthreads();
-  for (int n = tid; n < N; n += nt) {
-    const int m = slot_of(src(n)), tg = dst(n) - t0;
-    if (m >= 0 && tg >= 0 && tg < P) atomicMin(&minS[m], tg);
-  }
-  __syncthreads();
-  for (int n = tid; n < N; n += nt) {
-    const int m = slot_of(src(n)), tg = dst(n) - t0;
-    if (m >= 0 && tg >= 0 && tg < P) atomicMin(&fps[tg], minS[m]);
-  }
-  for (int m = tid; m < Mv; m += nt) {
-    const int pp = kxs[m] - t0;
-    if (pp >= 0 && pp < P) atomicMin(&fps[pp], minS[m]);
-  }
-  __syncthreads();
-  for (int pp = tid; pp < P; pp += nt) T.fpose[pp] = fps[pp];
-  if (band_verdict && wave == 0) {
-    const int admitted = ba_solve_wave_admits(fps, 6 * P, lane, max_nt);
-    if (lane == 0) __hip_atomic_store(band_verdict, admitted ? 1 : 2, __ATOMIC_RELAXED, __HIP_MEMORY_SCOPE_SYSTEM);
-  }
-  for (int n = tid; n < N; n += nt) T.gkey[8 + n] = (int)ii[n], T.gkey[8 + N + n] = (int)jj[n];
-  if (tid == 0) {
-    int *key = T.gkey;
-    key[0] = GKEY_MAGIC, key[1] = N, key[2] = B, key[3] = t0, key[4] = t1, key[5] = ftable, key[6] = T.Mmax;
-  }
-}
 
 __device__ void retract_pose(float *pose, const float *xi) {
   const float *tau = xi, *phi = xi + 3;
@@ -344,8 +92,304 @@
   R[8] = 1.0 - 2.0 * (x * x + y * y);
 }
 
-__device__ __forceinline__ float backsub_pixel(const BaTables &T, const BaBuffers &W, int m, int frame, int k, int HW, int t0,
-                                               int P) {
+__device__ __forceinline__ void edge_resolve(const float *__restrict__ poses, const float *__restrict__ dx, int n, int ix, int jx,
+                                             int t0, int P, bool upd, float *rec, double *Aw) {
+  double t64[3], R64[9];
+  edge_pose64(poses, dx, ix, jx, t0, P, upd, t64, R64);
+  reinterpret_cast<int *>(rec)[0] = n;
+  reinterpret_cast<int *>(rec)[1] = jx;
+#pragma unroll
+  for (int c = 0; c < 3; c++) rec[ETAB_POSE + c] = (float)t64[c];
+#pragma unroll
+  for (int c = 0; c < 9; c++) rec[ETAB_POSE + 3 + c] = (float)R64[c];
+  float *As = rec + ETAB_ADJ;
+#pragma unroll
+  for (int k = 0; k < 3; k++) {
+#pragma unroll
+    for (int c = 0; c < 3; c++) {
+      const double rkc = -R64[3 * k + c];
+      const int k1 = (k + 1) % 3, k2 = (k + 2) % 3;
+      const double x = t64[k2] * R64[3 * k1 + c] - t64[k1] * R64[3 * k2 + c];
+      As[6 * k + c] = (float)rkc, As[6 * k + 3 + c] = (float)x, As[18 + 3 * k + c] = (float)rkc;
+      if (Aw) Aw[6 * k + c] = rkc, Aw[6 * k + 3 + c] = x, Aw[6 * (3 + k) + c] = 0.0, Aw[6 * (3 + k) + 3 + c] = rkc;
+    }
+  }
+}
+
+__device__ __forceinline__ int wave_incl_scan(int v, int lane) {
+#pragma unroll
+  for (int off = 1; off < 64; off <<= 1) {
+    const int o = __shfl_up(v, off, 64);
+    if (lane >= off) v += o;
+  }
+  return v;
+}
+
+__global__ __launch_bounds__(1024) void ba_prepare_kernel(const int64_t *__restrict__ ii,
+                                                          const int64_t *__restrict__ jj, int N, int B,
+                                                          int t0, int t1, int scan_ints, int ftable, int check,
+                                                          int eta_rows, int *__restrict__ status, BaTables T,
+                                                          int *__restrict__ band_verdict, int max_nt,
+                                                          const float *__restrict__ poses, double *__restrict__ Aedge,
+                                                          float *__restrict__ etab) {
+  extern __shared__ int sm[];
+  int *flag = sm;
+  int *cnt = sm + B;
+  int *kxs = cnt + T.Mmax + 1;
+  int *scan = kxs + T.Mmax;
+  int *vcnt = scan + scan_ints;
+  const int tid = threadIdx.x, nt = blockDim.x, lane = tid & 63, wave = tid >> 6, nw = nt >> 6;
+  const int P = t1 - t0;
+  const int my_i = (tid < N) ? (int)ii[tid] : -1, my_j = (tid < N) ? (int)jj[tid] : -1;
+  auto src = [&](int n) { return (n == tid) ? my_i : (int)ii[n]; };
+  auto dst = [&](int n) { return (n == tid) ? my_j : (int)jj[n]; };
+  auto check_eta = [&](int nk) {
+    const bool bad = eta_rows > 1 && eta_rows != nk;
+    if (tid == 0) {
+      T.gkey[7] = bad ? 1 : 0;
+      if (bad && status) {
+        status[1] = eta_rows, status[2] = nk;
+        __hip_atomic_store(status, 1, __ATOMIC_RELEASE, __HIP_MEMORY_SCOPE_SYSTEM);
+      }
+    }
+    return bad ? SLOT_REFUSED : 0;
+  };
+  auto fill_edge_table = [&]() {
+    if (!poses) return;
+    for (int n = tid; n < N; n += nt) {
+      const int pos = T.rowinfo[8 * (P + n) + 2] - 1;
+      if (pos < 0) continue;
+      edge_resolve(poses, nullptr, n, src(n), dst(n), t0, P, false, etab + (size_t)pos * ETAB_WORDS, Aedge + (size_t)n * 36);
+    }
+  };
+
+  {
+    const int *key = T.gkey;
+    bool same = check && key[0] == GKEY_MAGIC && key[1] == N && key[2] == B && key[3] == t0 && key[4] == t1 &&
+                key[5] == ftable && key[6] == T.Mmax;
+    if (same) {
+      for (int n = tid; n < N; n += nt) {
+        const long long a = (long long)ii[n], b = (long long)jj[n];
+        same = same && (long long)key[8 + n] == a && (long long)key[8 + N + n] == b;
+      }
+    }
+    if (__syncthreads_and(same)) {
+      const int nk = T.meta[0];
+      const int refused = check_eta(nk);
+      for (int m = tid; m <= T.Mmax; m += nt) T.slotinfo[4 * m + 3] = refused | (m >= nk ? SLOT_UNUSED : 0);
+      fill_edge_table();
+      return;
+    }
+  }
+
+  for (int f = tid; f < B; f += nt) flag[f] = 0;
+  for (int m = tid; m <= T.Mmax; m += nt) cnt[m] = 0;
+  __syncthreads();
+  for (int p = tid; p < P; p += nt) {
+    const int f = t0 + p;
+    if (f >= 0 && f < B) flag[f] = 1;
+  }
+  for (int n = tid; n < N; n += nt) {
+    const int f = src(n);
+    if (f >= 0 && f < B) flag[f] = 1;
+  }
+  __syncthreads();
+
+  const int per = (B + nt - 1) / nt;
+  const int lo = min(tid * per, B), hi = min(lo + per, B);
+  int c = 0;
+  for (int f = lo; f < hi; f++) c += flag[f];
+  const int incl = wave_incl_scan(c, lane);
+  if (lane == 63) scan[wave] = incl;
+  __syncthreads();
+  if (wave == 0) {
+    const int v = (lane < nw) ? scan[lane] : 0;
+    const int w = wave_incl_scan(v, lane);
+    if (lane < nw) scan[16 + lane] = w;
+  }
+  __syncthreads();
+  int slot = incl - c + (wave > 0 ? scan[16 + wave - 1] : 0);
+  const int M = scan[16 + nw - 1];
+  for (int f = lo; f < hi; f++) {
+    if (flag[f]) {
+      if (slot < T.Mmax) T.kx[slot] = f, kxs[slot] = f;
+      T.frame_slot[f] = (slot < T.Mmax) ? slot : -1;
+      flag[f] = slot + 1;
+      slot++;
+    } else {
+      T.frame_slot[f] = -1;
+    }
+  }
+  if (tid == 0) {
+    T.meta[0] = min(M, T.Mmax);
+    T.meta[1] = 0;
+    T.meta[2] = (M > T.Mmax) ? 1 : 0;
+    T.meta[7] = 0;
+    T.meta[16] = 0;
+  }
+  const int refused = check_eta(min(M, T.Mmax));
+  __syncthreads();
+  auto slot_of = [&](int f) { return (f >= 0 && f < B && flag[f] > 0 && flag[f] <= T.Mmax) ? flag[f] - 1 : -1; };
+  auto emit_edge = [&](int n, int m, int pos, int jx) {
+    const int tg = jx - t0;
+    int *ri = T.rowinfo + 8 * (P + n);
+    const bool ok = m >= 0 && tg >= 0 && tg < P;
+    ri[0] = ok ? m : -1, ri[1] = tg, ri[2] = pos + 1, ri[3] = (m >= 0) ? cnt[m + 1] : 0, ri[4] = (m >= 0) ? kxs[m] : -1;
+    if (pos >= 0) T.einfo[2 * pos] = n, T.einfo[2 * pos + 1] = jx;
+  };
+
+  for (int n = tid; n < N; n += nt) {
+    const int m = slot_of(src(n));
+    if (m >= 0) atomicAdd(&cnt[m], 1);
+  }
+  __syncthreads();
+  if (wave == 0) {
+    int carry = 0;
+    for (int base = 0; base <= T.Mmax; base += 64) {
+      const int m = base + lane;
+      const int v = (m < T.Mmax) ? cnt[m] : 0;
+      const int w = wave_incl_scan(v, lane);
+      if (m <= T.Mmax) {
+        cnt[m] = carry + w - v;
+        T.eoff[m] = carry + w - v;
+      }
+      carry += __shfl(w, 63, 64);
+    }
+  }
+  __syncthreads();
+  for (int m = tid; m <= T.Mmax; m += nt) {
+    const bool used = m < min(M, T.Mmax);
+    *reinterpret_cast<int4 *>(T.slotinfo + 4 * m) =
+        make_int4(used ? kxs[m] : -1, used ? cnt[m] : 0, used ? cnt[m + 1] : 0, refused | (used ? 0 : SLOT_UNUSED));
+  }
+  int *sii = scan;
+  const int Mv0 = min(M, T.Mmax);
+  if (N <= nt) {
+    const bool myvalid = (tid < N) && (slot_of(my_i) >= 0) && (my_j - t0 >= 0) && (my_j - t0 < P);
+    constexpr int VBIT = 1 << 30;
+    if (tid < N) sii[tid] = (my_i & (VBIT - 1)) | (myvalid ? VBIT : 0);
+    if (ftable)
+      for (int m = tid; m <= T.Mmax; m += nt) {
+        const int pp = (m < Mv0) ? kxs[m] - t0 : -1;
+        vcnt[m] = (pp >= 0 && pp < P) ? 1 : 0;
+      }
+    __syncthreads();
+    int vrank = 0;
+    if (tid < N) {
+      const int f = my_i & (VBIT - 1), m = slot_of(my_i);
+      int pos = -1;
+      if (m >= 0) {
+        int rank = 0;
+        for (int q = 0; q < tid; q++) {
+          const int x = sii[q];
+          const bool same = ((x & (VBIT - 1)) == f);
+          rank += same;
+          vrank += same ? (x >> 30) : 0;
+        }
+        pos = cnt[m] + rank;
+        T.elist[pos] = tid;
+        if (myvalid && ftable) atomicAdd(&vcnt[m], 1);
+      }
+      emit_edge(tid, m, pos, my_j);
+    }
+    if (!ftable) {
+      for (int m = tid; m < T.Mmax; m += nt) T.fhead[4 * m] = -1, T.fhead[4 * m + 2] = 0;
+    } else {
+    __syncthreads();
+    if (wave == 0) {
+      int carry = 0;
+      for (int base = 0; base < T.Mmax; base += 64) {
+        const int m = base + lane;
+        const int v = (m < T.Mmax) ? vcnt[m] : 0;
+        const int w = wave_incl_scan(v, lane);
+        if (m < T.Mmax) {
+          const int pp = (m < Mv0) ? kxs[m] - t0 : -1;
+          const bool own = (pp >= 0 && pp < P);
+          const int off = carry + w - v;
+          int *fh = T.fhead + 4 * m;
+          fh[0] = (m < Mv0) ? kxs[m] : -1, fh[1] = off, fh[2] = v, fh[3] = 0;
+          if (own) T.frow[2 * off] = pp, T.frow[2 * off + 1] = pp;
+          vcnt[m] = off + (own ? 1 : 0);
+        }
+        carry += __shfl(w, 63, 64);
+      }
+    }
+    __syncthreads();
+    if (myvalid) {
+      const int o = vcnt[slot_of(my_i)] + vrank;
+      T.frow[2 * o] = P + tid, T.frow[2 * o + 1] = my_j - t0;
+    }
+    }
+  } else {
+    for (int m = tid; m < T.Mmax; m += nt) T.fhead[4 * m] = -1, T.fhead[4 * m + 2] = 0;
+    for (int n = tid; n < N; n += nt) T.elist_rank[n] = 0;
+    for (int base = 0; base < N; base += 1024) {
+      __syncthreads();
+      for (int q = tid; q < 1024 && base + q < N; q += nt) sii[q] = (int)ii[base + q];
+      __syncthreads();
+      const int lim = min(1024, N - base);
+      for (int n = tid; n < N; n += nt) {
+        if (n <= base) continue;
+        const int f = (int)ii[n];
+        if (slot_of(f) < 0) continue;
+        int rank = 0;
+        const int qend = min(lim, n - base);
+        for (int q = 0; q < qend; q++) rank += (sii[q] == f);
+        T.elist_rank[n] += rank;
+      }
+    }
+    __syncthreads();
+    for (int n = tid; n < N; n += nt) {
+      const int m = slot_of((int)ii[n]);
+      const int pos = (m >= 0) ? cnt[m] + T.elist_rank[n] : -1;
+      if (m >= 0) T.elist[pos] = n;
+      emit_edge(n, m, pos, (int)jj[n]);
+    }
+  }
+  for (int p = tid; p < P; p += nt) {
+    const int m = slot_of(t0 + p);
+    int *ri = T.rowinfo + 8 * p;
+    ri[0] = m, ri[1] = p, ri[2] = (m >= 0) ? cnt[m] : 0, ri[3] = (m >= 0) ? cnt[m + 1] : 0, ri[4] = t0 + p;
+  }
+  __syncthreads();
+  const int Mv = min(M, T.Mmax);
+  int *minS = cnt;
+  int *fps = scan;
+  for (int m = tid; m < Mv; m += nt) {
+    const int pp = kxs[m] - t0;
+    minS[m] = (pp >= 0 && pp < P) ? pp : 0x7fffffff;
+  }
+  for (int pp = tid; pp < P; pp += nt) fps[pp] = pp;
+  __syncthreads();
+  for (int n = tid; n < N; n += nt) {
+    const int m = slot_of(src(n)), tg = dst(n) - t0;
+    if (m >= 0 && tg >= 0 && tg < P) atomicMin(&minS[m], tg);
+  }
+  __syncthreads();
+  for (int n = tid; n < N; n += nt) {
+    const int m = slot_of(src(n)), tg = dst(n) - t0;
+    if (m >= 0 && tg >= 0 && tg < P) atomicMin(&fps[tg], minS[m]);
+  }
+  for (int m = tid; m < Mv; m += nt) {
+    const int pp = kxs[m] - t0;
+    if (pp >= 0 && pp < P) atomicMin(&fps[pp], minS[m]);
+  }
+  __syncthreads();
+  for (int pp = tid; pp < P; pp += nt) T.fpose[pp] = fps[pp];
+  if (band_verdict && wave == 0) {
+    const int admitted = ba_solve_wave_admits(fps, 6 * P, lane, max_nt);
+    if (lane == 0) __hip_atomic_store(band_verdict, admitted ? 1 : 2, __ATOMIC_RELAXED, __HIP_MEMORY_SCOPE_SYSTEM);
+  }
+  for (int n = tid; n < N; n += nt) T.gkey[8 + n] = (int)ii[n], T.gkey[8 + N + n] = (int)jj[n];
+  if (tid == 0) {
+    int *key = T.gkey;
+    key[0] = GKEY_MAGIC, key[1] = N, key[2] = B, key[3] = t0, key[4] = t1, key[5] = ftable, key[6] = T.Mmax;
+  }
+  fill_edge_table();
+}
+
+__device__ __forceinline__ float backsub_pixel(const BaTables &T, const BaBuffers &W, int m, int frame, int e0, int e1, int k,
+                                               int HW, int t0, int P) {
   float acc = 0.f;
   const int p = frame - t0;
   if (p > 0 && p < P) {
@@ -356,7 +400,6 @@
     for (int c = 0; c < 6; c++) dw += Er[(size_t)c * HW] * x[c];
     acc += dw;
   }
-  const int e0 = T.eoff[m], e1 = T.eoff[m + 1];
   for (int e = e0; e < e1; e++) {
     const int2 ei = *reinterpret_cast<const int2 *>(T.einfo + 2 * e);
     const int n = ei.x;
@@ -515,7 +558,9 @@
     const int64_t *__restrict__ jj, const uint8_t *__restrict__ frame_owned, int N, int HW, int wd,
     int t0, int P, float alpha, int upd_arg, float *__restrict__ poses_out, float *__restrict__ disps_w, BaTables T,
     BaBuffers W) {
-  const int upd = T.gkey[7] ? 0 : upd_arg;
+  const int4 srec = *reinterpret_cast<const int4 *>(T.slotinfo + 4 * blockIdx.y);
+  const int upd = (srec.w & SLOT_REFUSED) ? 0 : (upd_arg & 3);
+  const bool use_tab = (upd_arg & LIN_EDGE_TABLE) != 0;
 #ifdef LIN_PROF
   unsigned long long lp_ = wall_clock64();
   const unsigned long long lp_start_ = lp_;
@@ -538,9 +583,8 @@
     }
     return;
   }
-  const int M = T.meta[0];
-  if (m >= M) return;
-  const int frame = T.kx[m];
+  if (srec.w & SLOT_UNUSED) return;
+  const int frame = srec.x;
   if (frame_owned && !frame_owned[frame]) return;
 
   const int lane = lane_id();
@@ -562,7 +606,7 @@
     v[q] = (float)(kc[q] / wd);
     disp[q] = disps[(size_t)frame * HW + kc[q]];
     if ((upd & 2) && active[q])
-      disp[q] = disp[q] + backsub_pixel(T, W, m, frame, kc[q], HW, t0, P);
+      disp[q] = disp[q] + backsub_pixel(T, W, m, frame, srec.y, srec.z, kc[q], HW, t0, P);
   }
   if (upd & 2) {
     __syncthreads();
@@ -582,49 +626,19 @@
     for (int c = 0; c < 6; c++) Ei[q][c] = 0.f;
   }
   constexpr int EB = 16;
-  __shared__ float s_pose[EB][12];
-  __shared__ __attribute__((aligned(16))) float s_adj[EB][28];
-  __shared__ int s_edge[EB][2];
+  __shared__ __attribute__((aligned(16))) float s_tab[EB][ETAB_WORDS];
+  static_assert(ETAB_WORDS % 4 == 0 && ETAB_ADJ % 4 == 0 && EB * (ETAB_WORDS / 4) <= 256, "a batch is one 16-byte load per thread");
+  auto s_edge = [&](int i, int c) { return reinterpret_cast<const int *>(s_tab[i])[c]; };
   constexpr int RED_FLOATS = MF ? MFS_FLOATS : 64 * RED_PITCH;
   __shared__ __attribute__((aligned(16))) float s_red[4][RED_FLOATS];
   float *red_wave = s_red[wv];
   float *red_lane = red_wave + lane;
-  const int e0 = T.eoff[m], e1 = T.eoff[m + 1];
+  const int e0 = srec.y, e1 = srec.z;
   LP(0);
   for (int batch = e0; batch < e1; batch += EB) {
     const int cnt = min(EB, e1 - batch);
-    __syncthreads();
-    LP(1);
-    if ((int)threadIdx.x < cnt) {
-      const int2 ei = *reinterpret_cast<const int2 *>(T.einfo + 2 * (batch + threadIdx.x));
-      const int n = ei.x, jx = ei.y;
-      double t64[3], R64[9];
-      edge_pose64(poses, W.dx, frame, jx, t0, P, upd != 0, t64, R64);
-      s_edge[threadIdx.x][0] = n;
-      s_edge[threadIdx.x][1] = jx;
-#pragma unroll
-      for (int c = 0; c < 3; c++) s_pose[threadIdx.x][c] = (float)t64[c];
-#pragma unroll
-      for (int c = 0; c < 9; c++) s_pose[threadIdx.x][3 + c] = (float)R64[c];
-      double *Aw = (blockIdx.x == 0) ? W.Aedge + (size_t)n * 36 : nullptr;
-      float *As = s_adj[threadIdx.x];
-#pragma unroll
-      for (int k = 0; k < 3; k++) {
-#pragma unroll
-        for (int c = 0; c < 3; c++) {
-          const double rkc = -R64[3 * k + c];
-          const int k1 = (k + 1) % 3, k2 = (k + 2) % 3;
-          const double x = t64[k2] * R64[3 * k1 + c] - t64[k1] * R64[3 * k2 + c];
-          As[6 * k + c] = (float)rkc, As[6 * k + 3 + c] = (float)x, As[18 + 3 * k + c] = (float)rkc;
-          if (Aw) Aw[6 * k + c] = rkc, Aw[6 * k + 3 + c] = x, Aw[6 * (3 + k) + c] = 0.0, Aw[6 * (3 + k) + 3 + c] = rkc;
-        }
-      }
-    }
-    __syncthreads();
-    LP(2);
     float nx_t[PPL][2], nx_w[PPL][2];
-    {
-      const int n = s_edge[min(ew, cnt - 1)][0];
+    auto prefetch = [&](int n) {
 #pragma unroll
       for (int q = 0; q < PPL; q++) {
         const size_t tb = (size_t)n * 2 * HW + kc[q];
@@ -633,33 +647,46 @@
         nx_w[q][0] = weights[tb];
         nx_w[q][1] = weights[tb + HW];
       }
+    };
+    if (use_tab) {
+      if (batch != e0) __syncthreads();
+      LP(1);
+      const float *tab = W.etab + (size_t)batch * ETAB_WORDS;
+      const bool mine = (int)threadIdx.x < cnt * (ETAB_WORDS / 4);
+      float4 rec4 = make_float4(0.f, 0.f, 0.f, 0.f);
+      if (mine) rec4 = reinterpret_cast<const float4 *>(tab)[threadIdx.x];
+      prefetch(reinterpret_cast<const int *>(tab)[min(ew, cnt - 1) * ETAB_WORDS]);
+      if (mine) reinterpret_cast<float4 *>(&s_tab[0][0])[threadIdx.x] = rec4;
+      __syncthreads();
+      LP(2);
+    } else {
+      __syncthreads();
+      LP(1);
+      if ((int)threadIdx.x < cnt) {
+        const int2 ei = *reinterpret_cast<const int2 *>(T.einfo + 2 * (batch + threadIdx.x));
+        edge_resolve(poses, W.dx, ei.x, frame, ei.y, t0, P, upd != 0, s_tab[threadIdx.x],
+                     (blockIdx.x == 0) ? W.Aedge + (size_t)ei.x * 36 : nullptr);
+      }
+      __syncthreads();
+      LP(2);
+      prefetch(s_edge(min(ew, cnt - 1), 0));
     }
     for (int i = ew; i < cnt; i += EW) {
-      const int n = s_edge[i][0];
-      const int jx = s_edge[i][1];
+      const int n = s_edge(i, 0);
+      const int jx = s_edge(i, 1);
       float tij[3];
       Rot3 R;
 #pragma unroll
-      for (int c = 0; c < 3; c++) tij[c] = s_pose[i][c];
-#pragma unroll
-      for (int c = 0; c < 9; c++) R.r[c] = s_pose[i][3 + c];
+      for (int c = 0; c < 3; c++) tij[c] = s_tab[i][ETAB_POSE + c];
+#pragma unroll
+      for (int c = 0; c < 9; c++) R.r[c] = s_tab[i][ETAB_POSE + 3 + c];
       float cu_t[PPL][2], cu_w[PPL][2];
 #pragma unroll
       for (int q = 0; q < PPL; q++) {
         cu_t[q][0] = nx_t[q][0]; cu_t[q][1] = nx_t[q][1];
         cu_w[q][0] = nx_w[q][0]; cu_w[q][1] = nx_w[q][1];
       }
-      if (i + EW < cnt) {
-        const int nn = s_edge[i + EW][0];
-#pragma unroll
-        for (int q = 0; q < PPL; q++) {
-          const size_t tb = (size_t)nn * 2 * HW + kc[q];
-          nx_t[q][0] = targets[tb];
-          nx_t[q][1] = targets[tb + HW];
-          nx_w[q][0] = weights[tb];
-          nx_w[q][1] = weights[tb + HW];
-        }
-      }
+      if (i + EW < cnt) prefetch(s_edge(i + EW, 0));
 
       PixelLin L[PPL];
 #pragma unroll
@@ -680,7 +707,7 @@
           if (active[q]) Eij[(size_t)c * HW] = ej[c];
 #endif
         }
-        const float *Ae = s_adj[i];
+        const float *Ae = s_tab[i] + ETAB_ADJ;
 #pragma unroll
         for (int c = 0; c < 3; c++)
           Ei[q][c] += fmaf(ej[2], Ae[12 + c], fmaf(ej[1], Ae[6 + c], ej[0] * Ae[c]));
@@ -1421,7 +1448,8 @@
                                                         float *__restrict__ dx_out, BaTables T, BaBuffers W,
                                                         float disp_floor) {
   const int m = blockIdx.y;
-  if (T.gkey[7]) {
+  const int4 srec = *reinterpret_cast<const int4 *>(T.slotinfo + 4 * min(m, T.Mmax));
+  if (srec.w & SLOT_REFUSED) {
     if (m == T.Mmax && blockIdx.x == 0 && dx_out)
       for (int i = threadIdx.x; i < 6 * P; i += blockDim.x) dx_out[i] = 0.f;
     const int k = blockIdx.x * blockDim.x + threadIdx.x;
@@ -1452,14 +1480,13 @@
     return;
   }
   if (!update_disps) return;
-  const int M = T.meta[0];
-  if (m >= M) return;
-  const int frame = T.kx[m];
+  if (srec.w & SLOT_UNUSED) return;
+  const int frame = srec.x;
   if (frame_owned && !frame_owned[frame]) return;
   const int k = blockIdx.x * blockDim.x + threadIdx.x;
   if (k >= HW) return;
 
-  const float dz = backsub_pixel(T, W, m, frame, k, HW, t0, P);
+  const float dz = backsub_pixel(T, W, m, frame, srec.y, srec.z, k, HW, t0, P);
   const size_t mk = (size_t)m * HW + k;
   const size_t fk = (size_t)frame * HW + k;
   float d = disps[fk] + dz;
diff --git a/dba-fusion_amd/dbaf_amd/_lib.py b/dba-fusion_amd/dbaf_amd/_lib.py
--- a/dba-fusion_amd/dbaf_amd/_lib.py
+++ b/dba-fusion_amd/dbaf_amd/_lib.py
@@ -61,6 +61,7 @@
     "dba_ba_schur_thread_form": (c_int, []),
     "dba_ba_schur_generation": (c_int, []),
     "dba_ba_set_deterministic": (c_int, [c_int]),
+    "dba_ba_set_edge_table": (c_int, [c_int]),
     "dba_ba_set_solve_check": (c_int, [c_int]),
     "dba_ba_solve_check": (c_int, [c_int] * 6 + [c_float, c_float, _P, c_size_t, _P]),
     "dba_ba_symmetrize": (c_int, [c_int] * 6 + [_P, c_size_t, _P]),
diff --git a/include/dba_hip.h b/include/dba_hip.h
--- a/include/dba_hip.h
+++ b/include/dba_hip.h
@@ -63,6 +63,8 @@
 int dba_ba_schur_generation(void);
 
 int dba_ba_set_deterministic(int on);
+
+int dba_ba_set_edge_table(int on);
 
 int dba_ba_set_solve_check(int on);
 int dba_ba_solve_check(int N, int B, int ht, int wd, int t0, int t1, float lm, float ep, void *ws, size_t ws_bytes,
```

After: 4030. No clear change (-0.6%).
